# esq4/nind-denoise

Hardware: AMD Instinct MI355X
Metric: megapixels/sec denoised, UtNet cs=256 on 24 MP frames, 1/2/4/8 MI355X (higher is better)
Workload: dtype f32; 1 GPU; configs[1]: one 6000x4000 (24.0 MP) fp32 frame per step, f32 storage in the conv stack (fp32 accumulate), UtNet(funit=64,PReLU) random-init (seed 123), cs=264 (nearest valid to the named size; the reference rejects 256 / 512) ucs=200 ol=64 -> 1276 tiles/frame, tiles per conv-stack launch 256, crop->infer->stitch device resident (frame and canvas in HBM); every tile's input is the whole cs x cs cro; tiles_per_frame=1276, parallelism=single GPU

## Files before the change

include/nind_hip.h:

```cpp
#ifndef NIND_HIP_H
#define NIND_HIP_H

#include <stddef.h>
#include <stdint.h>

#ifdef __cplusplus
extern "C" {
#endif

typedef enum nd_status {
    ND_OK = 0,
    ND_EINVAL = -1,
    ND_ENOMEM = -2,
    ND_EHIP = -3
} nd_status;

typedef enum nd_act {
    ND_ACT_NONE = 0,
    ND_ACT_PRELU = 1,
    ND_ACT_ELU = 2,
    ND_ACT_HARDSWISH = 3
} nd_act;

typedef enum nd_layer_kind {
    ND_CONV3 = 0,
    ND_CONVT3 = 1,
    ND_CONVT2S2 = 2,
    ND_CONV1 = 3,
    ND_CONV2S2 = 4
} nd_layer_kind;

typedef enum nd_dtype {
    ND_F32 = 0,
    ND_BF16 = 1,
    ND_F16 = 2
} nd_dtype;

typedef enum nd_flags {
    ND_FLAG_NO_SPLITK = 1,
    ND_FLAG_DIRECT_CONV = 2,
    ND_FLAG_W1D_REGS = 4,
    ND_FLAG_UNFUSED_POOL = 16,
    ND_FLAG_TILE_ENCODER = 32,
    ND_FLAG_TILE_LEVEL2 = 64,
    ND_FLAG_FIND_NOISE = 128,
    ND_FLAG_TILE_SKIPS = 256,
    ND_FLAG_TILE_WINO = 512,
    ND_FLAG_FULL_TILES = 8
} nd_flags;

int nd_version(void);
const char *nd_last_error(void);

int nd_tile_grid(int width, int height, int cs, int ucs, int ol, int *cols, int *rows, int *pad);
int nd_tile_geom(int i, int width, int height, int cs, int ucs, int ol,
                 int *x0, int *y0, int usefuldim[4], int usefulstart[2]);

int nd_tile_gather(const float *img_chw, int width, int height, int cs, int ucs, int ol,
                   int tile_begin, int tile_count, float *tiles_nchw, void *stream);
int nd_stitch_add(float *canvas_chw, int width, int height, int cs, int ucs, int ol,
                  const float *tiles_nchw, int tile_begin, int tile_count, void *stream);

int nd_tile_source(int i, int width, int height, int cs, int ucs, int ol, int y, int x, int *Y, int *X);
int nd_stitch_weight(int i, int width, int height, int cs, int ucs, int ol, int y, int x, int *Y, int *X, float *w);
int nd_stitch_grad(const float *gcanvas_chw, int width, int height, int cs, int ucs, int ol, int tile_begin, int tile_count,
                   float *gtiles_nchw, void *stream);
int nd_tile_gather_grad(const float *gtiles_nchw, int width, int height, int cs, int ucs, int ol, int tile_begin, int tile_count,
                        float *gimg_chw, void *stream);

int nd_utnet_num_tensors(void);
const char *nd_utnet_tensor_name(int idx);
size_t nd_utnet_packed_bytes(int funit, int dtype);
int nd_utnet_pack_weights(int funit, int dtype, const float *const *tensors, int n_tensors,
                          void *packed_host, size_t packed_bytes);

int nd_utnet_pack_weights_device(int funit, int dtype, const float *const *dev_tensors, int n_tensors, void *packed_dev,
                                 size_t packed_bytes, void *stream);

size_t nd_utnet_workspace_bytes_hw(int funit, int h, int w, int batch, int dtype);
int nd_utnet_workspace_init_hw(void *workspace, size_t workspace_bytes, int funit, int h, int w, int batch, int dtype,
                               void *stream);
int nd_utnet_forward_hw(int funit, int act, int dtype, int flags, const void *packed_dev,
                        const float *x_nchw, float *y_nchw, int batch, int h, int w,
                        void *workspace, size_t workspace_bytes, void *stream);

int nd_utnet_denoise_tiles(int funit, int act, int dtype, int flags, const void *packed_dev,
                           const float *img_chw, float *canvas_chw, int width, int height,
                           int cs, int ucs, int ol, int tile_begin, int tile_count, int batch,
                           void *workspace, size_t workspace_bytes, void *stream);

typedef void (*nd_progress_fn)(void *ctx, int n, int tile_begin, int tile_count);
size_t nd_utnet_frame_workspace_bytes(int funit, int dtype, int flags, int width, int height, int cs, int ucs, int ol, int batch);
int nd_utnet_denoise_frame(int funit, int act, int dtype, int flags, const void *packed_dev,
                           const float *img_chw, float *canvas_chw, int width, int height,
                           int cs, int ucs, int ol, int tile_begin, int tile_count, int batch,
                           void *workspace, size_t workspace_bytes, void *frame_ws, size_t frame_ws_bytes, void *stream,
                           nd_progress_fn progress, void *progress_ctx);
int nd_utnet_denoise_frame_checked(int funit, int act, int dtype, int flags, const void *packed_dev,
                                   const float *img_chw, float *canvas_chw, int width, int height,
                                   int cs, int ucs, int ol, int tile_begin, int tile_count, int batch,
                                   void *workspace, size_t workspace_bytes, void *frame_ws, size_t frame_ws_bytes, void *stream,
                                   nd_progress_fn progress, void *progress_ctx, unsigned char *tile_ok);
int nd_utnet_frame_plan(int funit, int dtype, int flags, int width, int height, int cs, int ucs, int ol, int *out);
int nd_utnet_frame_levels(int funit, int dtype, int flags, int width, int height, int cs, int ucs, int ol, int *levels);
int nd_utnet_frame_folds(int funit, int dtype, int flags, int width, int height, int cs, int ucs, int ol, int *mask);

typedef struct nd_step_profile {
    float ms;
    float ms_xform_in;
    float ms_gemm;
    float ms_xform_out;
    int form;
    int kind;
    double flops;
    double mfma_flops;
    double bytes;
    double xform_bytes_in;
    double xform_bytes_out;
} nd_step_profile;
int nd_utnet_profile_stack(int funit, int act, int dtype, int flags, const void *packed_dev, int batch, int cs, int crop,
                           void *workspace, size_t workspace_bytes, void *stream, nd_step_profile *steps, int max_steps);
const char *nd_utnet_step_name(int i);
int nd_utnet_useful_region(int funit, int cs, int crop, int step, int *rect);

int nd_unet_num_tensors(void);
const char *nd_unet_tensor_name(int idx);
size_t nd_unet_packed_bytes(int dtype);
int nd_unet_pack_weights(int dtype, const float *const *tensors, int n_tensors, void *packed_host, size_t packed_bytes);
size_t nd_unet_workspace_bytes(int h, int w, int batch, int dtype);
int nd_unet_workspace_init(void *workspace, size_t workspace_bytes, int h, int w, int batch, int dtype, void *stream);
int nd_unet_forward(int dtype, const void *packed_dev, const float *x_nchw, float *y_nchw, int batch, int h, int w,
                    void *workspace, size_t workspace_bytes, void *stream);

int nd_unet_pack_weights_device(int dtype, const float *const *dev_tensors, int n_tensors, void *packed_dev, size_t packed_bytes,
                                void *stream);

int nd_unet_num_steps(void);
const char *nd_unet_step_name(int i);
int nd_unet_useful_region(int cs, int crop, int step, int *rect);

int nd_unet_denoise_frame(int dtype, int flags, const void *packed_dev, const float *img_chw, float *canvas_chw, int width,
                          int height, int cs, int ucs, int ol, int tile_begin, int tile_count, int batch, void *workspace,
                          size_t workspace_bytes, void *stream, nd_progress_fn progress, void *progress_ctx);

size_t nd_unet_param_count(void);
int nd_unet_param_range(int tensor_idx, size_t *offset, size_t *count);
size_t nd_unet_grad_blob_bytes(void);
size_t nd_unet_grad_workspace_bytes(int h, int w, int batch);
int nd_unet_grad_workspace_init(void *workspace, size_t workspace_bytes, int h, int w, int batch, void *stream);
int nd_unet_grad_forward(int flags, const float *params, void *blobs, const float *x_nchw, float *y_nchw, int batch, int h, int w,
                         void *workspace, size_t workspace_bytes, void *stream);
int nd_unet_grad_backward(int flags, const float *params, float *grads, void *blobs, const float *gy_nchw, float *dx_nchw, int batch,
                          int h, int w, void *workspace, size_t workspace_bytes, void *stream);

size_t nd_unet_train_blob_bytes(void);
size_t nd_unet_train_workspace_bytes(int h, int w, int batch);
int nd_unet_train_workspace_init(void *workspace, size_t workspace_bytes, int h, int w, int batch, void *stream);
int nd_unet_train_forward(int flags, float *params, void *blobs, const float *x_nchw, float *y_nchw, int batch, int h, int w,
                          float momentum, void *workspace, size_t workspace_bytes, void *stream);
int nd_unet_train_backward(int flags, const float *params, float *grads, void *blobs, const float *gy_nchw, float *dx_nchw, int batch,
                           int h, int w, void *workspace, size_t workspace_bytes, void *stream);

double nd_utnet_flops(int funit, int cs);

size_t nd_layer_packed_bytes(int kind, int cin, int cout, int dtype);
int nd_layer_pack(int kind, int cin, int cout, int dtype, const float *weight, const float *bias,
                  void *packed_host, size_t packed_bytes);
size_t nd_layer_workspace_bytes(int kind, int batch, int cin, int cout, int h, int w, int dtype);
int nd_layer_forward(int kind, int act, float slope, int dtype, const void *packed_dev,
                     const float *x_nchw, int batch, int cin, int h, int w, int cout, float *y_nchw,
                     void *workspace, size_t workspace_bytes, int variant, int flags, void *stream);
int nd_maxpool2_forward(const float *x_nchw, int batch, int c, int h, int w, float *y_nchw,
                        void *workspace, size_t workspace_bytes, void *stream);

size_t nd_layer_wgrad_workspace_bytes(int kind, int batch, int cin, int cout, int h, int w);
int nd_layer_wgrad(int kind, const float *x_nchw, const float *dy_nchw, int batch, int cin, int h, int w, int cout,
                   float *dw, float *db, void *workspace, size_t workspace_bytes, void *stream);

size_t nd_utnet_param_count(int funit);
int nd_utnet_param_range(int funit, int tensor_idx, size_t *offset, size_t *count);
size_t nd_utnet_train_blob_bytes(int funit);
size_t nd_utnet_train_workspace_bytes_hw(int funit, int h, int w, int batch);
int nd_utnet_train_workspace_init_hw(void *workspace, size_t workspace_bytes, int funit, int h, int w, int batch, void *stream);
int nd_utnet_train_step_act_hw(int funit, int act, int flags, const float *params, float *grads, void *blobs, const float *x_nchw,
                               const float *target_nchw, float *y_out_nchw, float w_l1, float w_mse, float w_ssim, float w_msssim,
                               float *loss_out, int batch, int h, int w, int loss_cs, void *workspace, size_t workspace_bytes,
                               void *stream, void *const *bucket_events, int n_events);
int nd_utnet_train_forward_hw(int funit, int act, int flags, const float *params, void *blobs, const float *x_nchw,
                              float *y_out_nchw, int batch, int h, int w, void *workspace, size_t workspace_bytes, void *stream);
int nd_utnet_train_backward_hw(int funit, int act, int flags, const float *params, float *grads, void *blobs, const float *gy_nchw,
                               float *dx_nchw, int batch, int h, int w, void *workspace, size_t workspace_bytes, void *stream,
                               void *const *bucket_events, int n_events);
int nd_utnet_grad_buckets(int funit, size_t *offsets, size_t *counts, int max);
int nd_adam_step(float *params, const float *grads, float *m, float *v, float *vmax, size_t n, float lr, float beta1,
                 float beta2, float eps, int step, int amsgrad, void *stream);
size_t nd_grad_guard_workspace_bytes(size_t n);
int nd_grad_guard(const float *grads, size_t n, float max_norm, int skip_nonfinite, double *state, void *workspace,
                  size_t workspace_bytes, void *stream);
int nd_adam_step_guarded(float *params, const float *grads, float *m, float *v, float *vmax, size_t n, float lr, float beta1,
                         float beta2, float eps, int step, int amsgrad, const double *state, void *stream);

size_t nd_ssim_workspace_bytes(int n, int c, int h, int w);
int nd_ssim(const float *x, const float *y, int n, int c, int h, int w, float *out, void *workspace, size_t workspace_bytes,
            void *stream);
int nd_ms_ssim(const float *x, const float *y, int n, int c, int h, int w, float *out, void *workspace,
               size_t workspace_bytes, void *stream);
int nd_mse(const float *x, const float *y, size_t count, float *out, void *workspace, size_t workspace_bytes, void *stream);

size_t nd_ssim_loss_workspace_bytes(int n, int c, int h, int w);
int nd_ssim_loss_grad(const float *x, const float *y, int n, int c, int h, int w, int multiscale, float weight,
                      float *loss_acc, float *gx, int accumulate, void *workspace, size_t workspace_bytes, void *stream);

size_t nd_criteria_workspace_bytes(int n, int h, int w, int loss_cs);
int nd_criteria(const float *y_nchw, const float *target_nchw, int n, int h, int w, int loss_cs, float w_l1, float w_mse,
                float w_ssim, float w_msssim, int also, float *out, void *workspace, size_t workspace_bytes, void *stream);
size_t nd_criteria_grad_workspace_bytes(int n, int h, int w, int loss_cs);
int nd_criteria_grad(const float *y_nchw, const float *target_nchw, int n, int h, int w, int loss_cs, float w_l1, float w_mse,
                     float w_ssim, float w_msssim, float *loss_out, float *gy_nchw, void *workspace, size_t workspace_bytes,
                     void *stream);

size_t nd_ssim_padded_workspace_bytes(int n, int c, int h, int w, int window);
int nd_ssim_padded(const float *x, const float *y, int n, int c, int h, int w, int window, float *out, void *workspace,
                   size_t workspace_bytes, void *stream);
int nd_ssim_padded_grad(const float *x, const float *y, int n, int c, int h, int w, int window, const float *gout, float *gx,
                        void *workspace, size_t workspace_bytes, void *stream);

typedef enum nd_sample_type { ND_SAMPLE_U8 = 0, ND_SAMPLE_U16 = 1, ND_SAMPLE_F32 = 2 } nd_sample_type;
int nd_crop_source(int cs, int nrot, int flips, int y, int x, int *a, int *b);
int nd_crop_batch(const void *pool, size_t pool_bytes, const int64_t *images, int n_images, const int32_t *draws, int batch, int cs,
                  float exp_mult_min, float exp_mult_max, const float *mult, float *xmax, float *mult_out, float *clean_nchw,
                  float *noisy_nchw, void *stream);
int nd_pool_fetch(const void *pool, size_t pool_bytes, const int64_t *images, int n_images, const int32_t *index, int n, int h, int w,
                  float *out_nchw, void *stream);
int nd_crop_batch_windows(const void *pool, size_t pool_bytes, const int64_t *windows, int n_windows, const int32_t *draws, int batch,
                          int cs, float exp_mult_min, float exp_mult_max, const float *mult, float *xmax, float *mult_out,
                          float *clean_nchw, float *noisy_nchw, void *stream);
int nd_pool_fetch_windows(const void *pool, size_t pool_bytes, const int64_t *windows, int n_windows, const int32_t *index, int n,
                          int h, int w, float *out_nchw, void *stream);

int nd_wino_mosaic(int p, int B, int *bx, int *by, long *tiles, long *tiles_per_image);

size_t nd_winograd_packed_bytes(int tile, int cin, int cout);
int nd_winograd_pack(int tile, int kind, int cin, int cout, const float *w, const float *bias, void *packed,
                     size_t packed_bytes);
size_t nd_layer_winograd_workspace_bytes(int tile, int kind, int batch, int cin, int cout, int h, int w);
int nd_layer_forward_winograd(int tile, int kind, int act, float slope, const void *packed, const float *x, int batch,
                              int cin, int h, int w, int cout, float *y, void *workspace, size_t workspace_bytes, int flags,
                              void *stream);

int nd_conv_bench(int kind, int dtype, int batch, int cin, int cout, int h, int w, int variant, int iters,
                  void *workspace, size_t workspace_bytes, void *stream, float *mean_ms);

int nd_winograd_bench(int tile, int kind, int batch, int cin, int cout, int h, int w, int iters, void *workspace,
                      size_t workspace_bytes, void *stream, float *mean_ms);
int nd_winograd_bench_flags(int tile, int kind, int batch, int cin, int cout, int h, int w, int iters, int flags, void *workspace,
                            size_t workspace_bytes, void *stream, float *mean_ms);

int nd_num_conv_variants(void);
const char *nd_conv_variant_name(int variant);

#ifdef __cplusplus
}
#endif
#endif
```

nind_denoise_amd/_lib.py:

```python
import ctypes
import os
from ctypes import POINTER, c_char_p, c_double, c_float, c_int, c_long, c_size_t, c_void_p

_HERE = os.path.dirname(os.path.abspath(__file__))
LIB_PATH = os.path.join(_HERE, "libnind_hip.so")

ND_F32, ND_BF16, ND_F16 = 0, 1, 2
DTYPE = {"f32": 0, "fp32": 0, "float32": 0, "bf16": 1, "bfloat16": 1, "f16": 2, "fp16": 2, "float16": 2}
ACT = {"none": 0, "PReLU": 1, "ELU": 2, "Hardswish": 3}
KIND = {"conv3": 0, "convT3": 1, "convT2s2": 2, "conv1": 3, "conv2s2": 4}
FLAG_NO_SPLITK, FLAG_DIRECT_CONV, FLAG_W1D_REGS, FLAG_FULL_TILES, FLAG_UNFUSED_POOL, FLAG_TILE_ENCODER, FLAG_TILE_LEVEL2 = 1, 2, 4, 8, 16, 32, 64
FLAG_FIND_NOISE = 128
FLAG_TILE_SKIPS = 256
FLAG_TILE_WINO = 512
PROGRESS_FN = ctypes.CFUNCTYPE(None, c_void_p, c_int, c_int, c_int)


class StepProfile(ctypes.Structure):
    _fields_ = [("ms", c_float), ("ms_xform_in", c_float), ("ms_gemm", c_float), ("ms_xform_out", c_float),
                ("form", c_int), ("kind", c_int), ("flops", c_double), ("mfma_flops", c_double), ("bytes", c_double),
                ("xform_bytes_in", c_double), ("xform_bytes_out", c_double)]


SAMPLE_U8, SAMPLE_U16, SAMPLE_F32 = 0, 1, 2

FORM_NAMES = {-1: "pool", 0: "direct", 1: "w1d_f43", 2: "w1d_f23", 3: "wino3p_f6x6"}


class NindHipError(RuntimeError):
    pass


class NindHipMissing(ImportError):
    pass


_lib = None

_SIGNATURES = {
    "nd_version": (c_int, []),
    "nd_last_error": (c_char_p, []),
    "nd_tile_grid": (c_int, [c_int] * 5 + [POINTER(c_int)] * 3),
    "nd_tile_geom": (c_int, [c_int] * 6 + [POINTER(c_int)] * 4),
    "nd_tile_gather": (c_int, [c_void_p] + [c_int] * 7 + [c_void_p, c_void_p]),
    "nd_stitch_add": (c_int, [c_void_p] + [c_int] * 5 + [c_void_p, c_int, c_int, c_void_p]),
    "nd_tile_source": (c_int, [c_int] * 8 + [POINTER(c_int)] * 2),
    "nd_stitch_weight": (c_int, [c_int] * 8 + [POINTER(c_int)] * 2 + [POINTER(c_float)]),
    "nd_stitch_grad": (c_int, [c_void_p] + [c_int] * 7 + [c_void_p, c_void_p]),
    "nd_tile_gather_grad": (c_int, [c_void_p] + [c_int] * 7 + [c_void_p, c_void_p]),
    "nd_utnet_num_tensors": (c_int, []),
    "nd_utnet_tensor_name": (c_char_p, [c_int]),
    "nd_utnet_packed_bytes": (c_size_t, [c_int, c_int]),
    "nd_utnet_pack_weights": (c_int, [c_int, c_int, POINTER(c_void_p), c_int, c_void_p, c_size_t]),
    "nd_utnet_pack_weights_device": (c_int, [c_int, c_int, POINTER(c_void_p), c_int, c_void_p, c_size_t, c_void_p]),
    "nd_utnet_workspace_bytes_hw": (c_size_t, [c_int] * 5),
    "nd_utnet_workspace_init_hw": (c_int, [c_void_p, c_size_t] + [c_int] * 5 + [c_void_p]),
    "nd_utnet_forward_hw": (c_int, [c_int] * 4 + [c_void_p] * 3 + [c_int, c_int, c_int, c_void_p, c_size_t, c_void_p]),
    "nd_utnet_denoise_tiles": (c_int, [c_int] * 4 + [c_void_p] * 3 + [c_int] * 8 + [c_void_p, c_size_t, c_void_p]),
    "nd_unet_num_tensors": (c_int, []),
    "nd_unet_tensor_name": (c_char_p, [c_int]),
    "nd_unet_packed_bytes": (c_size_t, [c_int]),
    "nd_unet_pack_weights": (c_int, [c_int, POINTER(c_void_p), c_int, c_void_p, c_size_t]),
    "nd_unet_workspace_bytes": (c_size_t, [c_int] * 4),
    "nd_unet_workspace_init": (c_int, [c_void_p, c_size_t] + [c_int] * 4 + [c_void_p]),
    "nd_unet_forward": (c_int, [c_int, c_void_p, c_void_p, c_void_p, c_int, c_int, c_int, c_void_p, c_size_t, c_void_p]),
    "nd_unet_pack_weights_device": (c_int, [c_int, POINTER(c_void_p), c_int, c_void_p, c_size_t, c_void_p]),
    "nd_unet_num_steps": (c_int, []),
    "nd_unet_step_name": (c_char_p, [c_int]),
    "nd_unet_useful_region": (c_int, [c_int, c_int, c_int, POINTER(c_int)]),
    "nd_unet_denoise_frame": (c_int, [c_int, c_int] + [c_void_p] * 3 + [c_int] * 8 + [c_void_p, c_size_t, c_void_p, PROGRESS_FN, c_void_p]),
    "nd_unet_param_count": (c_size_t, []),
    "nd_unet_param_range": (c_int, [c_int, POINTER(c_size_t), POINTER(c_size_t)]),
    "nd_unet_grad_blob_bytes": (c_size_t, []),
    "nd_unet_grad_workspace_bytes": (c_size_t, [c_int] * 3),
    "nd_unet_grad_workspace_init": (c_int, [c_void_p, c_size_t, c_int, c_int, c_int, c_void_p]),
    "nd_unet_grad_forward": (c_int, [c_int, c_void_p, c_void_p, c_void_p, c_void_p, c_int, c_int, c_int, c_void_p, c_size_t, c_void_p]),
    "nd_unet_train_blob_bytes": (c_size_t, []),
    "nd_unet_train_workspace_bytes": (c_size_t, [c_int] * 3),
    "nd_unet_train_workspace_init": (c_int, [c_void_p, c_size_t, c_int, c_int, c_int, c_void_p]),
    "nd_unet_train_forward": (c_int, [c_int, c_void_p, c_void_p, c_void_p, c_void_p, c_int, c_int, c_int, c_float, c_void_p, c_size_t,
                                      c_void_p]),
    "nd_unet_train_backward": (c_int, [c_int, c_void_p, c_void_p, c_void_p, c_void_p, c_void_p, c_int, c_int, c_int, c_void_p, c_size_t,
                                       c_void_p]),
    "nd_unet_grad_backward": (c_int, [c_int, c_void_p, c_void_p, c_void_p, c_void_p, c_void_p, c_int, c_int, c_int, c_void_p, c_size_t,
                                      c_void_p]),
    "nd_utnet_flops": (c_double, [c_int, c_int]),
    "nd_utnet_profile_stack": (c_int, [c_int] * 4 + [c_void_p, c_int, c_int, c_int, c_void_p, c_size_t, c_void_p, c_void_p, c_int]),
    "nd_utnet_step_name": (c_char_p, [c_int]),
    "nd_utnet_useful_region": (c_int, [c_int, c_int, c_int, c_int, POINTER(c_int)]),
    "nd_utnet_frame_workspace_bytes": (c_size_t, [c_int] * 9),
    "nd_utnet_frame_plan": (c_int, [c_int] * 8 + [POINTER(c_int)]),
    "nd_utnet_frame_levels": (c_int, [c_int] * 8 + [POINTER(c_int)]),
    "nd_utnet_frame_folds": (c_int, [c_int] * 8 + [POINTER(c_int)]),
    "nd_utnet_denoise_frame": (c_int, [c_int] * 4 + [c_void_p] * 3 + [c_int] * 8 + [c_void_p, c_size_t, c_void_p, c_size_t, c_void_p,
                                                                                    PROGRESS_FN, c_void_p]),
    "nd_utnet_denoise_frame_checked": (c_int, [c_int] * 4 + [c_void_p] * 3 + [c_int] * 8 + [c_void_p, c_size_t, c_void_p, c_size_t,
                                                                                            c_void_p, PROGRESS_FN, c_void_p, c_void_p]),
    "nd_layer_packed_bytes": (c_size_t, [c_int] * 4),
    "nd_layer_pack": (c_int, [c_int] * 4 + [c_void_p, c_void_p, c_void_p, c_size_t]),
    "nd_layer_workspace_bytes": (c_size_t, [c_int] * 7),
    "nd_layer_forward": (c_int, [c_int, c_int, c_float, c_int, c_void_p, c_void_p] + [c_int] * 5
                         + [c_void_p, c_void_p, c_size_t, c_int, c_int, c_void_p]),
    "nd_winograd_packed_bytes": (c_size_t, [c_int] * 3),
    "nd_winograd_pack": (c_int, [c_int] * 4 + [c_void_p, c_void_p, c_void_p, c_size_t]),
    "nd_layer_winograd_workspace_bytes": (c_size_t, [c_int] * 7),
    "nd_layer_forward_winograd": (c_int, [c_int, c_int, c_int, c_float, c_void_p, c_void_p] + [c_int] * 5
                                  + [c_void_p, c_void_p, c_size_t, c_int, c_void_p]),
    "nd_maxpool2_forward": (c_int, [c_void_p] + [c_int] * 4 + [c_void_p, c_void_p, c_size_t, c_void_p]),
    "nd_layer_wgrad_workspace_bytes": (c_size_t, [c_int] * 6),
    "nd_layer_wgrad": (c_int, [c_int, c_void_p, c_void_p] + [c_int] * 5 + [c_void_p, c_void_p, c_void_p, c_size_t, c_void_p]),
    "nd_utnet_param_count": (c_size_t, [c_int]),
    "nd_utnet_param_range": (c_int, [c_int, c_int, POINTER(c_size_t), POINTER(c_size_t)]),
    "nd_utnet_train_blob_bytes": (c_size_t, [c_int]),
    "nd_utnet_grad_buckets": (c_int, [c_int, POINTER(c_size_t), POINTER(c_size_t), c_int]),
    "nd_utnet_train_workspace_bytes_hw": (c_size_t, [c_int] * 4),
    "nd_utnet_train_workspace_init_hw": (c_int, [c_void_p, c_size_t, c_int, c_int, c_int, c_int, c_void_p]),
    "nd_utnet_train_forward_hw": (c_int, [c_int, c_int, c_int, c_void_p, c_void_p, c_void_p, c_void_p, c_int, c_int, c_int, c_void_p,
                                          c_size_t, c_void_p]),
    "nd_utnet_train_backward_hw": (c_int, [c_int, c_int, c_int, c_void_p, c_void_p, c_void_p, c_void_p, c_void_p, c_int, c_int, c_int,
                                           c_void_p, c_size_t, c_void_p, POINTER(c_void_p), c_int]),
    "nd_utnet_train_step_act_hw": (c_int, [c_int, c_int, c_int, c_void_p, c_void_p, c_void_p, c_void_p, c_void_p, c_void_p, c_float,
                                           c_float, c_float, c_float, c_void_p, c_int, c_int, c_int, c_int, c_void_p, c_size_t, c_void_p,
                                           POINTER(c_void_p), c_int]),
    "nd_adam_step": (c_int, [c_void_p] * 5 + [c_size_t, c_float, c_float, c_float, c_float, c_int, c_int, c_void_p]),
    "nd_grad_guard_workspace_bytes": (c_size_t, [c_size_t]),
    "nd_grad_guard": (c_int, [c_void_p, c_size_t, c_float, c_int, c_void_p, c_void_p, c_size_t, c_void_p]),
    "nd_adam_step_guarded": (c_int, [c_void_p] * 5 + [c_size_t, c_float, c_float, c_float, c_float, c_int, c_int, c_void_p, c_void_p]),
    "nd_ssim_workspace_bytes": (c_size_t, [c_int] * 4),
    "nd_ssim": (c_int, [c_void_p, c_void_p] + [c_int] * 4 + [c_void_p, c_void_p, c_size_t, c_void_p]),
    "nd_ms_ssim": (c_int, [c_void_p, c_void_p] + [c_int] * 4 + [c_void_p, c_void_p, c_size_t, c_void_p]),
    "nd_ssim_loss_workspace_bytes": (c_size_t, [c_int] * 4),
    "nd_ssim_loss_grad": (c_int, [c_void_p, c_void_p] + [c_int] * 5 + [c_float, c_void_p, c_void_p, c_int, c_void_p, c_size_t,
                                  c_void_p]),
    "nd_ssim_padded_workspace_bytes": (c_size_t, [c_int] * 5),
    "nd_ssim_padded": (c_int, [c_void_p, c_void_p] + [c_int] * 5 + [c_void_p, c_void_p, c_size_t, c_void_p]),
    "nd_ssim_padded_grad": (c_int, [c_void_p, c_void_p] + [c_int] * 5 + [c_void_p, c_void_p, c_void_p, c_size_t, c_void_p]),
    "nd_mse": (c_int, [c_void_p, c_void_p, c_size_t, c_void_p, c_void_p, c_size_t, c_void_p]),
    "nd_criteria_workspace_bytes": (c_size_t, [c_int] * 4),
    "nd_criteria": (c_int, [c_void_p, c_void_p] + [c_int] * 4 + [c_float] * 4 + [c_int, c_void_p, c_void_p, c_size_t, c_void_p]),
    "nd_criteria_grad_workspace_bytes": (c_size_t, [c_int] * 4),
    "nd_criteria_grad": (c_int, [c_void_p, c_void_p] + [c_int] * 4 + [c_float] * 4 + [c_void_p, c_void_p, c_void_p, c_size_t, c_void_p]),
    "nd_conv_bench": (c_int, [c_int] * 9 + [c_void_p, c_size_t, c_void_p, POINTER(c_float)]),
    "nd_winograd_bench": (c_int, [c_int] * 8 + [c_void_p, c_size_t, c_void_p, POINTER(c_float)]),
    "nd_winograd_bench_flags": (c_int, [c_int] * 9 + [c_void_p, c_size_t, c_void_p, POINTER(c_float)]),
    "nd_wino_mosaic": (c_int, [c_int, c_int, POINTER(c_int), POINTER(c_int), POINTER(c_long), POINTER(c_long)]),
    "nd_crop_source": (c_int, [c_int] * 5 + [POINTER(c_int)] * 2),
    "nd_crop_batch": (c_int, [c_void_p, c_size_t, c_void_p, c_int, c_void_p, c_int, c_int, c_float, c_float] + [c_void_p] * 6),
    "nd_pool_fetch": (c_int, [c_void_p, c_size_t, c_void_p, c_int, c_void_p, c_int, c_int, c_int, c_void_p, c_void_p]),
    "nd_crop_batch_windows": (c_int, [c_void_p, c_size_t, c_void_p, c_int, c_void_p, c_int, c_int, c_float, c_float] + [c_void_p] * 6),
    "nd_pool_fetch_windows": (c_int, [c_void_p, c_size_t, c_void_p, c_int, c_void_p, c_int, c_int, c_int, c_void_p, c_void_p]),
    "nd_num_conv_variants": (c_int, []),
    "nd_conv_variant_name": (c_char_p, [c_int]),
}

EXPORTS = tuple(_SIGNATURES)


def load():
    global _lib
    if _lib is not None:
        return _lib
    if not os.path.isfile(LIB_PATH):
        raise NindHipMissing(
            f"{LIB_PATH} not found: build it with `make -C nind_denoise_amd/csrc` (or __graft_entry__.build()). "
            "nind_denoise_amd has no CPU fallback for the denoise hot path.")
    import torch
    lib = ctypes.CDLL(LIB_PATH)
    for name, (res, args) in _SIGNATURES.items():
        fn = getattr(lib, name)
        fn.restype = res
        fn.argtypes = args
    _lib = lib
    return lib


def check(rc, what=""):
    if rc != 0:
        msg = load().nd_last_error().decode(errors="replace")
        exc = ValueError if rc == -1 else (MemoryError if rc == -2 else NindHipError)
        raise exc(f"{what}: {msg}" if what else msg)


def stream_ptr(device=None):
    import torch
    return c_void_p(torch.cuda.current_stream(device).cuda_stream)


def make_workspace(size_fn, init_fn, args, device, what, drop=None):
    import torch
    nbytes = size_fn(*args)
# ... 52 lines not shown
```

nind_denoise_amd/csrc/aux_kernels.hip:

```cpp
#include "nd_common.h"

typedef float f32x4 __attribute__((ext_vector_type(4)));
typedef __bf16 bf16x8 __attribute__((ext_vector_type(8)));
typedef _Float16 f16x8 __attribute__((ext_vector_type(8)));

template <int DT> struct Elem { typedef f32x4 vec; static constexpr int N = 4; typedef float scalar; };
template <> struct Elem<ND_BF16> { typedef bf16x8 vec; static constexpr int N = 8; typedef __bf16 scalar; };
template <> struct Elem<ND_F16> { typedef f16x8 vec; static constexpr int N = 8; typedef _Float16 scalar; };
#define ND_DISPATCH_DT(dt, CALL)                     \
    switch (dt) {                                    \
        case ND_F32: { constexpr int DT = ND_F32; CALL; break; }   \
        case ND_BF16: { constexpr int DT = ND_BF16; CALL; break; } \
        case ND_F16: { constexpr int DT = ND_F16; CALL; break; }   \
        default: ND_FAIL(ND_EINVAL, "unsupported storage type %d", dt); \
    }

static int make_geo(int W, int H, int cs, int ucs, int ol, TileGeo *g) {
    if (W <= 0 || H <= 0 || cs <= 0 || ucs <= 0 || ol < 0) ND_FAIL(ND_EINVAL, "tile grid: non-positive size");
    if (ucs - ol <= 0) ND_FAIL(ND_EINVAL, "tile grid: ucs (%d) must exceed the overlap (%d)", ucs, ol);
    if (cs < ucs) ND_FAIL(ND_EINVAL, "tile grid: cs (%d) < ucs (%d)", cs, ucs);
    g->W = W; g->H = H; g->cs = cs; g->ucs = ucs; g->ol = ol;
    g->stride = ucs - ol;
    g->pad = (cs - ucs) / 2;
    g->cols = ceil_div_py(W - ucs, g->stride) + 1;
// ... 649 lines not shown
    return ND_OK;
}

template <int DT>
__global__ void k_maxpool2(const typename Elem<DT>::vec *__restrict__ src, long snp, int sHb, int sWb, int spad, int splane0,
                           typename Elem<DT>::vec *__restrict__ dst, long dnp, int dHb, int dWb, int dpad, int Ho, int Wo, int B) {
    typedef typename Elem<DT>::vec V;
    const int xx = blockIdx.x * blockDim.x + threadIdx.x;
    const int yy = blockIdx.y;
    const int b = blockIdx.z % B, q = blockIdx.z / B;
    if (xx >= Wo) return;
    const V *s = src + (size_t)(splane0 + q) * snp + ((size_t)b * sHb + 2 * yy + spad) * sWb + 2 * xx + spad;
    const V a = s[0], c = s[1], d = s[sWb], e = s[sWb + 1];
    V o;
#pragma unroll
    for (int k = 0; k < Elem<DT>::N; ++k)
        o[k] = (typename Elem<DT>::scalar)fmaxf(fmaxf((float)a[k], (float)c[k]), fmaxf((float)d[k], (float)e[k]));
    dst[(size_t)q * dnp + ((size_t)b * dHb + yy + dpad) * dWb + xx + dpad] = o;
}

int nd_launch_maxpool2(const QpBuf &src, int src_plane0, int planes, const QpBuf &dst, hipStream_t s) {
    const int Hi = src.Hb - 2 * src.pad, Wi = src.Wb - 2 * src.pad;
    const int Ho = Hi / 2, Wo = Wi / 2;
    if (dst.Hb - 2 * dst.pad != Ho || dst.Wb - 2 * dst.pad != Wo || dst.B != src.B || dst.planes < planes || dst.dt != src.dt)
        ND_FAIL(ND_EINVAL, "maxpool2: destination does not fit %dx%d", Ho, Wo);
    dim3 grid((Wo + 127) / 128, Ho, src.B * planes);
    ND_DISPATCH_DT(src.dt, hipLaunchKernelGGL(k_maxpool2<DT>, grid, dim3(128), 0, s, (const typename Elem<DT>::vec *)src.base,
                                              src.np(), src.Hb, src.Wb, src.pad, src_plane0, (typename Elem<DT>::vec *)dst.base,
                                              dst.np(), dst.Hb, dst.Wb, dst.pad, Ho, Wo, src.B));
    ND_HIP(hipGetLastError());
    return ND_OK;
}

template <int DT>
__device__ __forceinline__ void dot3(const typename Elem<DT>::vec *__restrict__ s, long np, int planes,
                                     const float *__restrict__ w, int cin, float &o0, float &o1, float &o2) {
    constexpr int N = Elem<DT>::N;
    for (int q = 0; q < planes; ++q) {
        const typename Elem<DT>::vec v = s[(size_t)q * np];
#pragma unroll
        for (int e = 0; e < N; ++e) {
            const int c = N * q + e;
            if (c < cin) {
                const float f = (float)v[e];
                o0 = fmaf(f, w[c], o0);
                o1 = fmaf(f, w[cin + c], o1);
                o2 = fmaf(f, w[2 * cin + c], o2);
            }
        }
    }
}

template <int DT>
__global__ void k_final1x1(const typename Elem<DT>::vec *__restrict__ src, long np, int Hb, int Wb, int planes, int cin,
                           const float *__restrict__ w, const float *__restrict__ bias, int crop, float *__restrict__ y,
                           int H, int W, int sigmoid) {
    const int xx = blockIdx.x * blockDim.x + threadIdx.x;
    const int yy = blockIdx.y, b = blockIdx.z;
    if (xx >= W) return;
    float o0 = bias[0], o1 = bias[1], o2 = bias[2];
    dot3<DT>(src + ((size_t)b * Hb + yy + crop) * Wb + xx + crop, np, planes, w, cin, o0, o1, o2);
    if (sigmoid) {
        o0 = 1.f / (1.f + expf(-o0));
        o1 = 1.f / (1.f + expf(-o1));
        o2 = 1.f / (1.f + expf(-o2));
    }
    float *d = y + ((size_t)b * 3 * H + yy) * W + xx;
    d[0] = o0;
    d[(size_t)H * W] = o1;
    d[2 * (size_t)H * W] = o2;
}

int nd_launch_final1x1(const QpBuf &src, int cin, const float *w, const float *bias, int crop, float *y, int H, int W,
                       hipStream_t s, int sigmoid) {
    if (src.pad != 0 || src.Hb != H + 2 * crop || src.Wb != W + 2 * crop) ND_FAIL(ND_EINVAL, "final1x1: bad source geometry");
    dim3 grid((W + 255) / 256, H, src.B);
    const int n = nd_cpp(src.dt);
    ND_DISPATCH_DT(src.dt, hipLaunchKernelGGL(k_final1x1<DT>, grid, dim3(256), 0, s, (const typename Elem<DT>::vec *)src.base,
                                              src.np(), src.Hb, src.Wb, (cin + n - 1) / n, cin, w, bias, crop, y, H, W, sigmoid));
    ND_HIP(hipGetLastError());
    return ND_OK;
}

template <int DT, bool GUARD>
__device__ __forceinline__ void final1x1_stitch_pixel(const typename Elem<DT>::vec *__restrict__ src, long np, int Hb, int Wb, int planes,
                                                      int cin, const float *__restrict__ w, const float *__restrict__ bias, int crop,
                                                      float *__restrict__ canvas, const TileGeo &g, int tile_begin, int tile_count,
                                                      int y_first, int sigmoid, const float *__restrict__ noise_img,
                                                      const unsigned char *__restrict__ tile_ok) {
    const int X = blockIdx.x * blockDim.x + threadIdx.x;
    const int Y = y_first + blockIdx.y;
    if (X >= g.W || Y >= g.H) return;
    const size_t plane = (size_t)g.W * g.H;
    float *c = canvas + (size_t)Y * g.W + X;
    float v0 = c[0], v1 = c[plane], v2 = c[2 * plane];
    float n0 = 0.f, n1 = 0.f, n2 = 0.f;
    if (noise_img) {
        const float *n = noise_img + (size_t)Y * g.W + X;
        n0 = n[0]; n1 = n[plane]; n2 = n[2 * plane];
    }
    bool any = false;
    for_each_cover(g, X, Y, tile_begin, tile_count, [&](int t, int iy, int ix, float f) {
        if (GUARD && !tile_ok[tile_begin + t]) return;
        float o0 = bias[0], o1 = bias[1], o2 = bias[2];
        dot3<DT>(src + ((size_t)t * Hb + iy + crop) * Wb + ix + crop, np, planes, w, cin, o0, o1, o2);
        if (sigmoid) {
            o0 = 1.f / (1.f + expf(-o0));
            o1 = 1.f / (1.f + expf(-o1));
            o2 = 1.f / (1.f + expf(-o2));
        }
        if (noise_img) {
            o0 = n0 - o0;
            o1 = n1 - o1;
            o2 = n2 - o2;
        }
        v0 += o0 * f;
        v1 += o1 * f;
        v2 += o2 * f;
        any = true;
    });
    if (any) {
        c[0] = v0;
        c[plane] = v1;
        c[2 * plane] = v2;
    }
}

template <int DT>
__global__ void k_final1x1_stitch(const typename Elem<DT>::vec *__restrict__ src, long np, int Hb, int Wb, int planes, int cin,
                                  const float *__restrict__ w, const float *__restrict__ bias, int crop,
                                  float *__restrict__ canvas, TileGeo g, int tile_begin, int tile_count, int y_first, int sigmoid,
                                  const float *__restrict__ noise_img) {
    final1x1_stitch_pixel<DT, false>(src, np, Hb, Wb, planes, cin, w, bias, crop, canvas, g, tile_begin, tile_count, y_first, sigmoid,
                                     noise_img, nullptr);
}

template <int DT>
__global__ void k_final1x1_stitch_ok(const typename Elem<DT>::vec *__restrict__ src, long np, int Hb, int Wb, int planes, int cin,
                                     const float *__restrict__ w, const float *__restrict__ bias, int crop,
                                     float *__restrict__ canvas, TileGeo g, int tile_begin, int tile_count, int y_first,
                                     const unsigned char *__restrict__ tile_ok) {
    final1x1_stitch_pixel<DT, true>(src, np, Hb, Wb, planes, cin, w, bias, crop, canvas, g, tile_begin, tile_count, y_first, 0, nullptr,
                                    tile_ok);
}

template <int DT>
__global__ __launch_bounds__(256) void k_tile_verdict(const typename Elem<DT>::vec *__restrict__ src, long np, int Hb, int Wb,
                                                      int planes, int cin, const float *__restrict__ w,
                                                      const float *__restrict__ bias, int crop, TileGeo g, int tile_begin,
                                                      int tile_count, unsigned char *__restrict__ tile_ok) {
    const int t = blockIdx.y;
    if (t >= tile_count) return;
    const int i = tile_begin + t;
    const int yi = i / g.cols, xi = i - yi * g.cols;
    const int ax = xi * g.stride, ay = yi * g.stride;
    const int x1pad = max(0, ax - g.pad + g.cs - g.W), y1pad = max(0, ay - g.pad + g.cs - g.H);
    const int uw = min(g.cs - max(g.pad, x1pad) - g.pad, g.W - ax), uh = min(g.cs - max(g.pad, y1pad) - g.pad, g.H - ay);
    if (uw <= 0 || uh <= 0) return;
    const int p = blockIdx.x * blockDim.x + threadIdx.x;
    if (p >= uw * uh) return;
    const int dy = p / uw, dx = p - dy * uw;
    float o0 = bias[0], o1 = bias[1], o2 = bias[2];
    dot3<DT>(src + ((size_t)t * Hb + g.pad + dy + crop) * Wb + g.pad + dx + crop, np, planes, w, cin, o0, o1, o2);
    const unsigned e = 0x7f800000u;
    if ((__float_as_uint(o0) & e) == e || (__float_as_uint(o1) & e) == e || (__float_as_uint(o2) & e) == e) tile_ok[i] = 0;
}

static int stitch_launch_geo(const QpBuf &src, int crop, int W, int H, int cs, int ucs, int ol, int tile_begin, int tile_count, TileGeo *g,
                             int *yf, int *yr) {
    ND_TRY(make_geo(W, H, cs, ucs, ol, g));
    if (src.pad != 0 || src.Hb != cs + 2 * crop || src.Wb != cs + 2 * crop || tile_count > src.B)
        ND_FAIL(ND_EINVAL, "final1x1_stitch: bad source geometry");
    stitch_band(*g, tile_begin, tile_count, yf, yr);
    return ND_OK;
}

int nd_launch_final1x1_stitch(const QpBuf &src, int cin, const float *w, const float *bias, int crop, float *canvas,
                              int W, int H, int cs, int ucs, int ol, int tile_begin, int tile_count, hipStream_t s, int sigmoid,
                              const float *noise_img) {
    TileGeo g;
    int yf, yr;
    ND_TRY(stitch_launch_geo(src, crop, W, H, cs, ucs, ol, tile_begin, tile_count, &g, &yf, &yr));
    if (yr <= 0) return ND_OK;
    dim3 grid((W + 255) / 256, yr);
    const int n = nd_cpp(src.dt);
    ND_DISPATCH_DT(src.dt, hipLaunchKernelGGL(k_final1x1_stitch<DT>, grid, dim3(256), 0, s, (const typename Elem<DT>::vec *)src.base,
                                              src.np(), src.Hb, src.Wb, (cin + n - 1) / n, cin, w, bias, crop, canvas, g,
                                              tile_begin, tile_count, yf, sigmoid, noise_img));
    ND_HIP(hipGetLastError());
    return ND_OK;
}

int nd_launch_tile_verdict(const QpBuf &src, int cin, const float *w, const float *bias, int crop, int W, int H, int cs, int ucs, int ol,
                           int tile_begin, int tile_count, unsigned char *tile_ok, hipStream_t s) {
    TileGeo g;
    int yf, yr;
    ND_TRY(stitch_launch_geo(src, crop, W, H, cs, ucs, ol, tile_begin, tile_count, &g, &yf, &yr));
    if (!tile_ok || tile_begin < 0 || tile_count <= 0 || tile_count > 65535 || tile_begin + tile_count > g.cols * g.rows)
        ND_FAIL(ND_EINVAL, "tile_verdict: tiles [%d,+%d) outside the grid of %d (at most 65535 per launch), or no flags", tile_begin,
                tile_count, g.cols * g.rows);
    const int uwmax = g.cs - 2 * g.pad;
    if (uwmax <= 0) return ND_OK;
    dim3 grid((uwmax * uwmax + 255) / 256, tile_count);
    const int n = nd_cpp(src.dt);
    ND_DISPATCH_DT(src.dt, hipLaunchKernelGGL(k_tile_verdict<DT>, grid, dim3(256), 0, s, (const typename Elem<DT>::vec *)src.base,
                                              src.np(), src.Hb, src.Wb, (cin + n - 1) / n, cin, w, bias, crop, g, tile_begin, tile_count,
                                              tile_ok));
    ND_HIP(hipGetLastError());
    return ND_OK;
}

int nd_launch_final1x1_stitch_ok(const QpBuf &src, int cin, const float *w, const float *bias, int crop, float *canvas, int W, int H,
                                 int cs, int ucs, int ol, int tile_begin, int tile_count, const unsigned char *tile_ok, hipStream_t s) {
    TileGeo g;
    int yf, yr;
    ND_TRY(stitch_launch_geo(src, crop, W, H, cs, ucs, ol, tile_begin, tile_count, &g, &yf, &yr));
    if (!tile_ok) ND_FAIL(ND_EINVAL, "final1x1_stitch_ok: no flags");
    if (yr <= 0) return ND_OK;
    dim3 grid((W + 255) / 256, yr);
    const int n = nd_cpp(src.dt);
    ND_DISPATCH_DT(src.dt, hipLaunchKernelGGL(k_final1x1_stitch_ok<DT>, grid, dim3(256), 0, s, (const typename Elem<DT>::vec *)src.base,
                                              src.np(), src.Hb, src.Wb, (cin + n - 1) / n, cin, w, bias, crop, canvas, g,
                                              tile_begin, tile_count, yf, tile_ok));
    ND_HIP(hipGetLastError());
    return ND_OK;
}

__global__ __launch_bounds__(256) void k_sum(const float *__restrict__ partial, int n, float scale, float *__restrict__ out) {
    __shared__ float red[256];
    float acc = 0.f;
    for (int i = threadIdx.x; i < n; i += 256) acc += partial[i];
    acc = nd_block_sum(acc, red);
    if (threadIdx.x == 0) out[0] = acc * scale;
}
int nd_launch_sum(const float *partial, int n, float scale, float *out, hipStream_t s) {
    hipLaunchKernelGGL(k_sum, dim3(1), dim3(256), 0, s, partial, n, scale, out);
    ND_HIP(hipGetLastError());
    return ND_OK;
}
```

nind_denoise_amd/csrc/conv_qp.inc:

```
#pragma once
#include <stdlib.h>

#include <initializer_list>
#include <type_traits>

#include "nd_common.h"

typedef float f32x4 __attribute__((ext_vector_type(4)));
typedef float f32x8 __attribute__((ext_vector_type(8)));
typedef float f32x16 __attribute__((ext_vector_type(16)));
typedef __bf16 bf16x8 __attribute__((ext_vector_type(8)));
typedef __bf16 bf16x4 __attribute__((ext_vector_type(4)));
typedef _Float16 f16x8 __attribute__((ext_vector_type(8)));
typedef _Float16 f16x4 __attribute__((ext_vector_type(4)));

template <int DT> struct FragOf { typedef f32x4 type; };
template <> struct FragOf<ND_BF16> { typedef bf16x8 type; };
template <> struct FragOf<ND_F16> { typedef f16x8 type; };

struct FastDiv {
    unsigned m;
    int sh;
};
static inline FastDiv nd_fastdiv(int d) {
    FastDiv f;
    int s = 0;
    while ((1L << s) < (long)d) ++s;
    f.m = (unsigned)((((unsigned long long)1 << (31 + s)) + (unsigned long long)d - 1) / (unsigned long long)d);
    f.sh = 31 + s;
    return f;
}
__device__ __forceinline__ unsigned fdiv(unsigned n, const FastDiv &f) { return (unsigned)(((unsigned long long)n * f.m) >> f.sh); }

struct ConvParams {
    const f32x4 *in;
    const float *wpk;
    const float *bias;
    f32x4 *out;
    long in_plane;
    long out_plane;
    int nimg;
    int P, Wb;
    int Hv, Wv, PV;
    int tpi;
    int G;
    int stride;
    int ioff;
    f32x4 *pre;
    long pre_plane;
    int KB;
    int M;
    int cout;
    int Po, Wo, opad;
    int out_plane0;
    int act;
    float slope;
    const float *slope_dev;
    int n_tiles_n;
    int n_tiles_m;
    int split_first, S, cps, nitems;
    f32x4 *part;
    int wpx;
    int tiles_per_problem;
    long in_bs, out_bs;
    long w_bs;
    int dbg;
    int linear;
    FastDiv fd_PV, fd_Wv, fd_ntm, fd_tpp, fd_upq, fd_tpi;
    f32x4 *pool;
    long pool_plane;
    int pool_P, pool_W, pool_pad;
    int band2;
    FastDiv fd_2Wv;
    const f32x4 *in2;
    long in2_plane;
    const int *origin2;
    int kb2, Wb2;
    int KBw;
    const f32x4 *add;
    long add_plane;
    const int *origin_add;
    int W_add;
};

static inline void nd_conv_fastdivs(ConvParams &p) {
    p.fd_PV = nd_fastdiv(p.PV > 0 ? p.PV : 1);
    p.fd_Wv = nd_fastdiv(p.Wv > 0 ? p.Wv : 1);
    p.fd_2Wv = nd_fastdiv(p.Wv > 0 ? 2 * p.Wv : 1);
    p.fd_ntm = nd_fastdiv(p.n_tiles_m > 0 ? p.n_tiles_m : 1);
    p.fd_tpp = nd_fastdiv(p.tiles_per_problem > 0 ? p.tiles_per_problem : 1);
    p.fd_upq = nd_fastdiv(p.cout / 4 > 0 ? p.cout / 4 : 1);
    p.fd_tpi = nd_fastdiv(p.tpi > 0 ? p.tpi : 1);
}

ConvParams nd_conv_params(const ConvDesc &d, int KB, int M);
int nd_conv_pool(const char *who, const ConvDesc &d, int Hv, int Wv, ConvParams &p);
void nd_conv_tiles(ConvParams &p, bool cross, int nblk, int mblk);
long nd_conv_schedule(ConvParams &p, long ntiles, int nchunks, long slots, long cap);
double nd_conv_schedule_time(long ntiles, int nchunks, long slots, long cap);
int nd_launch_split_finish(const ConvParams &p, int n_split_tiles, int mblk, int nblk, int up, int dt, hipStream_t s);
#ifdef ND_QP_STAMPS
int nd_stamped_launch(void (*fn)(ConvParams), int threads, size_t lds, ConvParams p, long ntiles, int nchunks, long slots, hipStream_t s,
                      bool print, const char *header, const char *wave_prefix, const char *const *names, int nphases, std::initializer_list<int> waves);
#endif

__device__ __forceinline__ void glds16(const void *g, void *l) {
    __builtin_amdgcn_global_load_lds((const __attribute__((address_space(1))) void *)g,
                                     (__attribute__((address_space(3))) void *)l, 16, 0, 0);
}

__device__ __forceinline__ f32x8 sload8(const float *p) {
    const unsigned long long a = (unsigned long long)p;
    const unsigned lo = __builtin_amdgcn_readfirstlane((unsigned)a);
    const unsigned hi = __builtin_amdgcn_readfirstlane((unsigned)(a >> 32));
    const float *sp = (const float *)(((unsigned long long)hi << 32) | lo);
    f32x8 v;
    asm volatile("s_load_dwordx8 %0, %1, 0x0\n\ts_waitcnt lgkmcnt(0)" : "=s"(v) : "s"(sp) : "memory");
    return v;
}
__device__ __forceinline__ f32x4 sload_bias4(const float *p, int h) {
    const unsigned long long a = (unsigned long long)p;
    const unsigned lo = __builtin_amdgcn_readfirstlane((unsigned)a);
    const unsigned hi = __builtin_amdgcn_readfirstlane((unsigned)(a >> 32));
    const float *sp = (const float *)(((unsigned long long)hi << 32) | lo);
    f32x4 b0, b1;
    asm volatile("s_load_dwordx4 %0, %2, 0x0\n\ts_load_dwordx4 %1, %2, 0x10\n\ts_waitcnt lgkmcnt(0)" : "=&s"(b0), "=&s"(b1) : "s"(sp) : "memory");
    f32x4 r;
#pragma unroll
    for (int e = 0; e < 4; ++e) r[e] = h ? b1[e] : b0[e];
    return r;
}

#ifdef ND_QP_STAMPS
__device__ __forceinline__ unsigned long long qp_stamp() {
    unsigned long long t;
    __builtin_amdgcn_sched_barrier(0);
    asm volatile("s_memtime %0\n\ts_waitcnt lgkmcnt(0)" : "=s"(t)::"memory");
    __builtin_amdgcn_sched_barrier(0);
    return t;
}
#define QP_STAMP(k) do { if (stamps) { t1 = qp_stamp(); tph[k] += t1 - t0; t0 = t1; } } while (0)
#else
#define QP_STAMP(k) do { } while (0)
#endif

__device__ __forceinline__ float quad_max(float v) {
    int a = __builtin_bit_cast(int, v);
    v = fmaxf(v, __builtin_bit_cast(float, __builtin_amdgcn_update_dpp(a, a, 0xB1, 0xF, 0xF, false)));
    a = __builtin_bit_cast(int, v);
    return fmaxf(v, __builtin_bit_cast(float, __builtin_amdgcn_update_dpp(a, a, 0x4E, 0xF, 0xF, false)));
}

__device__ __forceinline__ float apply_act(float v, int act, float slope) {
    switch (act) {
        case ND_ACT_PRELU: return v > 0.f ? v : v * slope;
        case ND_ACT_ELU: return v > 0.f ? v : expm1f(v);
        case ND_ACT_HARDSWISH: return v * fminf(fmaxf(v + 3.f, 0.f), 6.f) / 6.f;
        default: return v;
    }
}

template <int DT, int MR, int NR, int WM, int WN, int TAPS, int KBC, bool UP, int NSTAGE>
__global__ __launch_bounds__(64 * WM * WN) void conv_qp(ConvParams p) {
    typedef typename FragOf<DT>::type Frag;
    extern __shared__ __attribute__((aligned(16))) char smem[];
// ... 531 lines not shown
```

nind_denoise_amd/csrc/conv_w2d.hip:

```cpp
#include "conv_qp.inc"

namespace {

typedef float f32x2 __attribute__((ext_vector_type(2)));

constexpr int kR = 8;
constexpr int kS = 16;
constexpr int kRI = kR + 2;
constexpr int kVPlane = kRI * kS * 16;
constexpr int kVPos = 2 * kVPlane;
constexpr int kVBytes = 6 * kVPos;
constexpr int kTaps = 18;
constexpr int kMTB = 2;
constexpr int kWBytes = kMTB * kTaps * 1024;
constexpr int kStage = kWBytes + kVBytes;
constexpr int kStages = 2;
constexpr int kScratch = 2048;
constexpr int kLds = kStages * kStage + 8 * kScratch;
constexpr int kDmaAt = 4;
constexpr int kXfAt = 12;
constexpr int kSlots = 4 * 32 * 4;

template <int OFF> __device__ __forceinline__ void glds16o(const void *g, void *l) {
    __builtin_amdgcn_global_load_lds((const __attribute__((address_space(1))) void *)g, (__attribute__((address_space(3))) void *)l, 16, OFF, 0);
}

__device__ __forceinline__ int vslot(int r, int s) { return r * kS + (s ^ ((r & 3) << 2)); }

__device__ __forceinline__ void w4_in(const f32x4 *d, f32x4 *v) {
    const f32x4 s34 = d[3] + d[4], d43 = d[4] - d[3], s12 = d[1] + d[2], d12 = d[1] - d[2], d42 = d[4] - d[2], d31 = d[3] - d[1];
    v[0] = 4.f * d[0] - 5.f * d[2] + d[4];
    v[1] = s34 - 4.f * s12;
    v[2] = d43 + 4.f * d12;
    v[3] = d42 + 2.f * d31;
    v[4] = d42 - 2.f * d31;
    v[5] = 4.f * d[1] - 5.f * d[3] + d[5];
}
__device__ __forceinline__ void w4_out(const float *m, float *y) {
    const float a = m[1] + m[2], b = m[1] - m[2], c = m[3] + m[4], e = m[3] - m[4];
    y[0] = m[0] + a + c;
    y[1] = b + 2.f * e;
    y[2] = a + 4.f * c;
    y[3] = b + 8.f * e + m[5];
}

__device__ __forceinline__ unsigned long long stamp() {
    unsigned long long t;
    __builtin_amdgcn_sched_barrier(0);
    asm volatile("s_memtime %0\n\ts_waitcnt lgkmcnt(0)" : "=s"(t)::"memory");
    __builtin_amdgcn_sched_barrier(0);
    return t;
}

#ifdef ND_QP_STAMPS
const char *const kStampNames[6] = {"issue loads + DMA", "MFMA loop", "wait vmcnt", "transform+publish (inside the loop)", "epilogue", "barrier"};
#endif
struct Strip { int img, y0, x0; bool ok; };

template <int DBG, bool SRC2 = false, bool ADD = false>
__global__ __launch_bounds__(512) void conv_w2d(ConvParams p) {
    extern __shared__ __attribute__((aligned(16))) char smem[];
    const int lane = threadIdx.x & 63;
    const int wave = __builtin_amdgcn_readfirstlane(threadIdx.x >> 6);
    const int wm = wave >> 2, wn = wave & 3;
    const int j = lane & 31, h = lane >> 5;
    const int nwg = gridDim.x;
    const int bid = blockIdx.x;
    const int vb = (nwg % 8 == 0) ? (bid % 8) * (nwg / 8) + bid / 8 : bid;

    const int nchunks = p.KB;
    const int nitems = p.nitems;
    const int my_items = vb < nitems ? (nitems - vb + nwg - 1) / nwg : 0;
    struct Item { int tile, c0, c1, slice; };
    auto decode = [&](int w) -> Item {
        Item it;
        if (w < p.split_first) {
            it.tile = w; it.c0 = 0; it.c1 = nchunks; it.slice = -1;
        } else {
            const int u = w - p.split_first;
            const int t = u / p.S, ks = u - t * p.S;
            it.tile = p.split_first + t;
            it.c0 = ks * p.cps;
            it.c1 = it.c0 + p.cps < nchunks ? it.c0 + p.cps : nchunks;
            it.slice = u;
        }
        return it;
    };
    int nsteps = 0;
    if (p.split_first >= nitems)
        nsteps = my_items * nchunks;
    else
        for (int i = 0; i < my_items; ++i) {
            const Item it = decode(vb + i * nwg);
            nsteps += it.c1 - it.c0;
        }
    if (nsteps == 0) return;

    const unsigned tot = (unsigned)p.nimg * (unsigned)p.PV;
    auto strip_of = [&](int nb, int s) -> Strip {
        Strip r;
        const unsigned u = (unsigned)nb * kS + s;
        r.ok = u < tot;
        const unsigned uc = r.ok ? u : tot - 1;
        r.img = (int)fdiv(uc, p.fd_PV);
        const int rem = (int)(uc - (unsigned)r.img * p.PV);
        const int band = (int)fdiv((unsigned)rem, p.fd_Wv);
        r.y0 = band * kR;
        r.x0 = 4 * (rem - band * p.Wv);
        return r;
    };

    int f_id = vb, f_c = 0, f_end = 0, f_stage = 0, issued = 0;
    int f_nb = 0;
    const float *f_w;
    const unsigned lane16 = (unsigned)lane * 16u;
    const int kXfHalf = 1;
    const bool xfA = (wave >> 2) == kXfHalf, xfB = wave == 4 * (1 - kXfHalf);
    const int dw = wave - 4 * (1 - kXfHalf);
    int vwOff[2];
    int x_h[2], x_i[2], x_s[2];
#pragma unroll
    for (int ps = 0; ps < 2; ++ps) {
        const int xt = ps == 0 ? (wave & 3) * 64 + lane : 256 + lane;
        x_h[ps] = xt / (kS * kRI);
        x_i[ps] = (xt / kS) % kRI;
        x_s[ps] = xt % kS;
        vwOff[ps] = kWBytes + x_h[ps] * kVPlane + vslot(x_i[ps], x_s[ps]) * 16;
    }
    unsigned x_off[2] = {0, 0};
    int x_keep[2] = {6, 6};
    auto set_fill_tile = [&](int w) {
        const Item it = decode(w);
        f_c = it.c0;
        f_end = it.c1;
        const int nb = (int)fdiv((unsigned)it.tile, p.fd_ntm), mb = it.tile - nb * p.n_tiles_m;
        f_w = p.wpk + (size_t)mb * kMTB * p.KBw * kTaps * 256;
        if constexpr (SRC2) f_nb = nb;
#pragma unroll
        for (int ps = 0; ps < 2; ++ps)
            if (ps == 0 ? xfA : xfB) {
                const Strip st = strip_of(nb, x_s[ps]);
                x_off[ps] = 16u * ((unsigned)x_h[ps] * (unsigned)p.in_plane + (unsigned)st.img * (unsigned)p.P + (unsigned)(st.y0 + x_i[ps]) * p.Wb + st.x0);
                const int left = p.wpx - st.x0;
                x_keep[ps] = left + 2 < 6 ? left + 2 : 6;
            }
    };
    auto set_fill_src2 = [&]() {
        const int nb = f_nb;
#pragma unroll
        for (int ps = 0; ps < 2; ++ps)
            if (ps == 0 ? xfA : xfB) {
                const Strip st = strip_of(nb, x_s[ps]);
                x_off[ps] = 16u * ((unsigned)x_h[ps] * (unsigned)p.in2_plane + (unsigned)p.origin2[st.img] + (unsigned)(st.y0 + x_i[ps]) * p.Wb2 + st.x0);
            }
    };
    set_fill_tile(f_id);
    if constexpr (SRC2) if (f_c >= p.kb2) set_fill_src2();
    f32x4 dn[2][6];
#pragma unroll
    for (int ps = 0; ps < 2; ++ps)
#pragma unroll
        for (int k = 0; k < 6; ++k) dn[ps][k] = f32x4{0.f, 0.f, 0.f, 0.f};
    auto fill_loads = [&]() {
        if (issued >= nsteps || (DBG & 8)) return;
        const bool s2 = SRC2 && f_c >= p.kb2;
        const char *kbase = s2 ? (const char *)(p.in2 + (size_t)(2 * (f_c - p.kb2)) * p.in2_plane)
                               : (const char *)(p.in + (size_t)(2 * f_c) * p.in_plane);
        if (xfA) {
#pragma unroll
            for (int k = 0; k < 6; ++k) dn[0][k] = *(const f32x4 *)(kbase + x_off[0] + 16 * k);
        }
        if (xfB) {
#pragma unroll
            for (int k = 0; k < 6; ++k) dn[1][k] = *(const f32x4 *)(kbase + x_off[1] + 16 * k);
        }
    };
    auto fill_xform = [&]() {
        if (issued >= nsteps || (DBG & 16)) return;
#pragma unroll
// ... 32 lines not shown
    auto fill_advance = [&]() {
        if (issued >= nsteps) return;
        ++issued;
        f_stage ^= 1;
        if (++f_c == f_end) {
            f_id += nwg;
            if (f_id < nitems) {
                set_fill_tile(f_id);
                if constexpr (SRC2) if (f_c >= p.kb2) set_fill_src2();
            }
        } else if constexpr (SRC2) {
            if (f_c == p.kb2) set_fill_src2();
        }
    };

    const int sl = 4 * wn + (j >> 3), rr = j & 7;
    const int aOff = (wm * kTaps) * 1024 + lane * 16;
    int bOffK[3];
#pragma unroll
    for (int ky = 0; ky < 3; ++ky) bOffK[ky] = kWBytes + h * kVPlane + vslot(rr + ky, sl) * 16;

    f32x16 acc[6];
#pragma unroll
    for (int x = 0; x < 6; ++x)
#pragma unroll
        for (int r = 0; r < 16; ++r) acc[x][r] = 0.f;

    const float slope = p.act == ND_ACT_NONE ? 1.f : (p.slope_dev ? *p.slope_dev : p.slope);
    const bool slope01 = p.act <= ND_ACT_PRELU && slope >= 0.f && slope <= 1.f;

    auto combine = [&](int g, f32x4 *y) {
#pragma unroll
        for (int e = 0; e < 4; ++e) {
            float m[6], o[4];
#pragma unroll
            for (int x = 0; x < 6; ++x) {
                m[x] = acc[x][4 * g + e];
                acc[x][4 * g + e] = 0.f;
            }
            w4_out(m, o);
#pragma unroll
            for (int i = 0; i < 4; ++i) y[i][e] = o[i];
        }
    };

    char *const scratch = smem + kStages * kStage + wave * kScratch;
    const int e_row = lane >> 4, e_px = lane & 15;
    f32x4 biasq[4];
    auto load_bias = [&](int id) {
        if constexpr (ADD) return;
        const int mb = id - (int)fdiv((unsigned)id, p.fd_ntm) * p.n_tiles_m;
#pragma unroll
        for (int g = 0; g < 4; ++g) biasq[g] = *(const f32x4 *)(p.bias + (mb * kMTB + wm) * 32 + 8 * g + 4 * h);
    };
    load_bias(decode(vb).tile);
    auto epilogue = [&](int id, auto fast) {
        const int nb = (int)fdiv((unsigned)id, p.fd_ntm), mb = id - nb * p.n_tiles_m;
        const Strip st = strip_of(nb, 4 * wn + (e_px >> 2));
        const int ex = st.x0 + (e_px & 3);
        const unsigned offA = (unsigned)((st.img * p.Po + (st.y0 + e_row + p.opad) * p.Wo + ex + p.opad) * 16);
        const unsigned offB = offA + (unsigned)(4 * p.Wo * 16);
        const bool okx = st.ok && ex < p.wpx;
        const bool okA = okx && st.y0 + e_row < p.Hv, okB = okx && st.y0 + e_row + 4 < p.Hv;
        const int q0 = (mb * kMTB + wm) * 8;
        const f32x2 slope2 = {slope, slope};
        const int pp_i = (e_px & ~3) + 2 * (e_px & 1);
        const int pxp = (st.x0 >> 1) + (e_px & 1), pyp = (st.y0 >> 1) + e_row;
        unsigned offQA = 0, offQB = 0;
        f32x4 qa[8], qb[8];
        auto add_loads = [&](int k) {
            const int qq = (q0 + k) * 4 < p.M ? q0 + k : 0;
            const char *pq = (const char *)(p.add + (size_t)qq * p.add_plane);
            qa[k] = *(const f32x4 *)(pq + offQA);
            qb[k] = *(const f32x4 *)(pq + offQB);
        };
        if constexpr (ADD) {
            const unsigned oq = 16u * ((unsigned)p.origin_add[st.img] + (unsigned)(st.y0 + e_row) * (unsigned)p.W_add + (unsigned)ex);
            offQA = okA ? oq : 0u;
            offQB = okB ? oq + 64u * (unsigned)p.W_add : 0u;
            add_loads(0);
            add_loads(1);
            __builtin_amdgcn_sched_barrier(0);
        }
        const bool okP = !SRC2 && !ADD && p.pool && !(lane & 2) && st.ok && 2 * pxp + 1 < p.wpx && 2 * pyp + 1 < p.Hv;
        const unsigned offP = (unsigned)((st.img * p.pool_P + (pyp + p.pool_pad) * p.pool_W + pxp + p.pool_pad) * 16);
#pragma unroll
        for (int g = 0; g < 4; ++g) {
            f32x4 yy[4], ypre[4];
#pragma unroll
            for (int pr = 0; pr < 2; ++pr) {
                f32x2 m[6];
#pragma unroll
                for (int x = 0; x < 6; ++x) {
                    m[x] = f32x2{acc[x][4 * g + 2 * pr], acc[x][4 * g + 2 * pr + 1]};
                    acc[x][4 * g + 2 * pr] = 0.f;
                    acc[x][4 * g + 2 * pr + 1] = 0.f;
                }
                f32x2 a = m[1] + m[2], b = m[1] - m[2];
                const f32x2 c = m[3] + m[4], e = m[3] - m[4];
                if constexpr (!ADD) {
                    const f32x2 bq = {biasq[g][2 * pr], biasq[g][2 * pr + 1]};
                    a += bq;
                    b += bq;
                }
                f32x2 y[4];
                y[0] = m[0] + a + c;
                y[1] = b + 2.f * e;
                y[2] = a + 4.f * c;
                y[3] = b + 8.f * e + m[5];
#pragma unroll
                for (int i = 0; i < 4; ++i) {
                    ypre[i][2 * pr] = y[i][0];
                    ypre[i][2 * pr + 1] = y[i][1];
                    if constexpr (ADD) {
                    } else if constexpr (decltype(fast)::value) {
                        const f32x2 t = y[i] * slope2;
                        y[i] = f32x2{fmaxf(y[i][0], t[0]), fmaxf(y[i][1], t[1])};
                    } else {
                        y[i] = f32x2{apply_act(y[i][0], p.act, slope), apply_act(y[i][1], p.act, slope)};
                    }
                    yy[i][2 * pr] = y[i][0];
                    yy[i][2 * pr + 1] = y[i][1];
                }
            }
            if (!SRC2 && !ADD && p.pre) {
                const Strip so = strip_of(nb, sl);
                const int yo = so.y0 + rr, m4 = (q0 + 2 * g + h) * 4, left = p.wpx - so.x0;
                if (so.ok && yo < p.Hv && m4 < p.M) {
                    f32x4 *dst = p.pre + (long)(m4 >> 2) * p.pre_plane + ((long)so.img * p.Hv + yo) * p.wpx + so.x0;
#pragma unroll
                    for (int i = 0; i < 4; ++i)
                        if (i < left) dst[i] = ypre[i];
                }
            }
            if (DBG & 256) {
                const Strip so = strip_of(nb, sl);
                const int yo = so.y0 + rr, m4 = (q0 + 2 * g + h) * 4, left = p.wpx - so.x0;
                if (so.ok && yo < p.Hv && m4 < p.M) {
                    f32x4 *dst = p.out + (long)(p.out_plane0 + (m4 >> 2)) * p.out_plane + (long)so.img * p.Po + (long)(yo + p.opad) * p.Wo + so.x0 + p.opad;
#pragma unroll
                    for (int i = 0; i < 4; ++i)
                        if (i < left) dst[i] = yy[i];
                }
                continue;
            }
#pragma unroll
            for (int hq = 0; hq < 2; ++hq) {
                if (h == hq) {
                    f32x4 *w = (f32x4 *)scratch + rr * 16 + (j >> 3) * 4;
#pragma unroll
                    for (int i = 0; i < 4; ++i) w[i] = yy[i];
                }
                __builtin_amdgcn_fence(__ATOMIC_RELEASE, "wavefront");
                __builtin_amdgcn_wave_barrier();
                __builtin_amdgcn_fence(__ATOMIC_ACQUIRE, "wavefront");
                f32x4 va = *((const f32x4 *)scratch + e_row * 16 + e_px);
                f32x4 vb2 = *((const f32x4 *)scratch + (e_row + 4) * 16 + e_px);
                if constexpr (ADD) {
                    const int k = 2 * g + hq;
                    va += qa[k];
                    vb2 += qb[k];
                    if (k + 2 < 8) {
                        add_loads(k + 2);
                        __builtin_amdgcn_sched_barrier(0);
                    }
#pragma unroll
                    for (int e = 0; e < 4; ++e) {
                        if constexpr (decltype(fast)::value) {
                            va[e] = fmaxf(va[e], va[e] * slope);
                            vb2[e] = fmaxf(vb2[e], vb2[e] * slope);
                        } else {
                            va[e] = apply_act(va[e], p.act, slope);
                            vb2[e] = apply_act(vb2[e], p.act, slope);
                        }
                    }
                }
                f32x4 vp = va;
                if (!SRC2 && !ADD && p.pool) {
                    const f32x4 *blk = (const f32x4 *)scratch + (2 * e_row) * 16 + pp_i;
                    const f32x4 p00 = blk[0], p01 = blk[1], p10 = blk[16], p11 = blk[17];
#pragma unroll
                    for (int e = 0; e < 4; ++e) vp[e] = fmaxf(fmaxf(p00[e], p01[e]), fmaxf(p10[e], p11[e]));
                }
                __builtin_amdgcn_fence(__ATOMIC_RELEASE, "wavefront");
                __builtin_amdgcn_wave_barrier();
                __builtin_amdgcn_fence(__ATOMIC_ACQUIRE, "wavefront");
                const int quad = q0 + 2 * g + hq;
                if (quad * 4 < p.M && !(DBG & 1)) {
                    char *pb = (char *)(p.out + (size_t)(p.out_plane0 + quad) * p.out_plane);
                    if (okA) *(f32x4 *)(pb + offA) = va;
                    if (okB) *(f32x4 *)(pb + offB) = vb2;
                    if (okP) *(f32x4 *)((char *)(p.pool + (size_t)quad * p.pool_plane) + offP) = vp;
                }
            }
        }
    };
    auto epilogue_partial = [&](int slice) {
        f32x4 *dst = p.part + (size_t)slice * (kMTB * 8) * kSlots;
#pragma unroll
        for (int g = 0; g < 4; ++g) {
            f32x4 yy[4];
            combine(g, yy);
            f32x4 *d2 = dst + (size_t)(wm * 8 + 2 * g + h) * kSlots + 4 * (wn * 32 + j);
#pragma unroll
            for (int i = 0; i < 4; ++i) d2[i] = yy[i];
        }
    };

    fill_loads();
    fill_xform();
    fill_dma();
    fill_advance();
    asm volatile("s_waitcnt vmcnt(0) lgkmcnt(0)" ::: "memory");
    __builtin_amdgcn_s_barrier();

    int c_id = vb, c_stage = 0;
    Item c_it = decode(vb);
    int c_c = c_it.c0;
    unsigned long long tph[6] = {0, 0, 0, 0, 0, 0}, t0 = 0, t1 = 0;
    for (int s = 0; s < nsteps; ++s) {
        if (DBG & 128) t0 = stamp();
        fill_loads();
        __builtin_amdgcn_sched_barrier(0);
        if (DBG & 128) { t1 = stamp(); tph[0] += t1 - t0; t0 = t1; }
        const char *wa = smem + c_stage * kStage + aOff;
        const char *vq = smem + c_stage * kStage;
        f32x4 a[2], b[2];
        a[0] = *(const f32x4 *)wa;
        b[0] = *(const f32x4 *)(vq + bOffK[0]);
#pragma unroll
        for (int st = 0; st < kTaps; ++st) {
            if (st + 1 < kTaps) {
                const int ky = (st + 1) / 6, x = (st + 1) % 6;
                a[(st + 1) & 1] = *(const f32x4 *)(wa + (st + 1) * 1024);
                b[(st + 1) & 1] = *(const f32x4 *)(vq + bOffK[ky] + x * kVPos);
            }
            __builtin_amdgcn_sched_barrier(0);
            const int x = st % 6;
            if (!(DBG & 32)) {
#pragma unroll
                for (int q = 0; q < 4; ++q) acc[x] = __builtin_amdgcn_mfma_f32_32x32x2f32(a[st & 1][q], b[st & 1][q], acc[x], 0, 0, 0);
            } else {
#pragma unroll
                for (int q = 0; q < 4; ++q) acc[x][q] += a[st & 1][q] * b[st & 1][q];
            }
            if (st + 1 == kDmaAt) {
                __builtin_amdgcn_sched_barrier(0);
                fill_dma();
                __builtin_amdgcn_sched_barrier(0);
            }
            if (st + 1 == kXfAt) {
                __builtin_amdgcn_sched_barrier(0);
                if (DBG & 128) { t1 = stamp(); tph[1] += t1 - t0; t0 = t1; }
                fill_xform();
                fill_advance();
                if (DBG & 128) { t1 = stamp(); tph[3] += t1 - t0; t0 = t1; }
                __builtin_amdgcn_sched_barrier(0);
            }
        }
        __builtin_amdgcn_sched_barrier(0);
        if (DBG & 128) { t1 = stamp(); tph[1] += t1 - t0; t0 = t1; }
        asm volatile("s_waitcnt vmcnt(0) lgkmcnt(0)" ::: "memory");
        if (DBG & 128) { t1 = stamp(); tph[2] += t1 - t0; t0 = t1; }
        c_stage ^= 1;
        if (++c_c == c_it.c1) {
            if (DBG & 2) {
            } else if (c_it.slice >= 0)
                epilogue_partial(c_it.slice);
            else if (slope01)
                epilogue(c_it.tile, std::true_type{});
            else
                epilogue(c_it.tile, std::false_type{});
            c_id += nwg;
            if (c_id < nitems) {
                c_it = decode(c_id);
                if (p.n_tiles_m > 1) load_bias(c_it.tile);
            }
            c_c = c_it.c0;
        }
        if (DBG & 128) { t1 = stamp(); tph[4] += t1 - t0; t0 = t1; }
        if (!(DBG & 64)) __builtin_amdgcn_s_barrier();
        if (DBG & 128) { t1 = stamp(); tph[5] += t1 - t0; }
    }
    if ((DBG & 128) && lane == 0 && p.part) {
        unsigned long long *o = (unsigned long long *)p.part + ((size_t)blockIdx.x * 8 + wave) * 8;
        for (int k = 0; k < 6; ++k) o[k] = tph[k];
        o[6] = (unsigned long long)nsteps;
    }
}

__global__ __launch_bounds__(256) void k_w2d_split_finish(ConvParams p) {
    const int t = blockIdx.x, quad = blockIdx.y;
    const int gid = p.split_first + t;
    const int nb = gid / p.n_tiles_m, mb = gid - nb * p.n_tiles_m;
    const int m4 = mb * (kMTB * 32) + quad * 4;
    if (m4 >= p.M) return;
    const float slope = p.act == ND_ACT_NONE ? 1.f : (p.slope_dev ? *p.slope_dev : p.slope);
    const f32x4 bv = p.add ? f32x4{0.f, 0.f, 0.f, 0.f} : *(const f32x4 *)(p.bias + m4);
    const unsigned tot = (unsigned)p.nimg * (unsigned)p.PV;
    for (int l = threadIdx.x; l < kSlots; l += 256) {
        const int i = l & 3, jj = l >> 2, wn = jj >> 5, j = jj & 31;
        const int s = 4 * wn + (j >> 3), rr = j & 7;
        const unsigned u = (unsigned)nb * kS + s;
        if (u >= tot) continue;
        const int img = (int)(u / (unsigned)p.PV);
        const int rem = (int)(u - (unsigned)img * p.PV);
        const int band = rem / p.Wv;
        const int y = band * kR + rr, x = 4 * (rem - band * p.Wv) + i;
        if (y >= p.Hv || x >= p.wpx) continue;
        f32x4 acc = {0.f, 0.f, 0.f, 0.f};
        for (int ks = 0; ks < p.S; ++ks) acc += p.part[((size_t)(t * p.S + ks) * (kMTB * 8) + quad) * kSlots + l];
        if (p.add)
            acc += p.add[(long)(m4 >> 2) * p.add_plane + (long)p.origin_add[img] + (long)y * p.W_add + x];
        else
            acc += bv;
        f32x4 v;
#pragma unroll
        for (int e = 0; e < 4; ++e) v[e] = p.act <= ND_ACT_PRELU ? (acc[e] > 0.f ? acc[e] : acc[e] * slope) : apply_act(acc[e], p.act, slope);
        p.out[(long)(p.out_plane0 + (m4 >> 2)) * p.out_plane + (long)img * p.Po + (long)(y + p.opad) * p.Wo + x + p.opad] = v;
    }
}

}

bool nd_w2d_ok(const QpBuf &in) { return in.dt == ND_F32 && in.Hb >= 3 && in.Wb >= 3; }
long nd_w2d_tiles(const QpBuf &in, int cout) {
    const long strips = (long)in.B * ((in.Hb - 2 + kR - 1) / kR) * ((in.Wb - 2 + 3) / 4);
    return ((strips + kS - 1) / kS) * ((cout + kMTB * 32 - 1) / (kMTB * 32));
}

int nd_launch_conv_w2d(const ConvDesc &d, hipStream_t stream) {
    if ((d.kind != ND_CONV3 && d.kind != ND_CONVT3) || d.in.dt != ND_F32 || d.out.dt != ND_F32) ND_FAIL(ND_EINVAL, "w2d: fp32 3x3 layers only");
    const int KB = nd_kblocks(d.cin);
    const int Hfull = d.in.Hb - 2, Wfull = d.in.Wb - 2;
    if (Hfull < 1 || Wfull < 1) ND_FAIL(ND_EINVAL, "w2d: input smaller than the kernel");
    ND_TRY(nd_check_roi("w2d", d, Hfull, Wfull, d.pool != nullptr, "a pooled layer"));
    const bool roi = d.roi_rows > 0;
    const int Hv = roi ? d.roi_rows : Hfull, Wpx = roi ? d.roi_cols : Wfull, Wg = (Wpx + 3) / 4, NB = (Hv + kR - 1) / kR;
    if (d.pre && (roi || d.pool)) ND_FAIL(ND_EINVAL, "w2d: a pre-activation copy goes with whole, unpooled layers only");
    if (d.cout % 4) ND_FAIL(ND_EINVAL, "w2d: cout must be a multiple of 4");
    ND_TRY(nd_check_in_planes("w2d", d, KB, true, true));
    const bool src2 = d.in2.base != nullptr, add = d.add.base != nullptr;
    if (add && (d.pool || d.pre || src2))
        ND_FAIL(ND_EINVAL, "w2d: a layer with an addend source is neither pooled nor keeps a pre-activation copy nor has a second input source");
    if (add) ND_TRY(nd_check_add("w2d", d, (long)(d.roi_r0 + Hv - 1 + d.add.pad) * d.add.Wb + d.roi_c0 + Wpx - 1 + d.add.pad + 1));
    if (src2 && (d.pool || d.pre)) ND_FAIL(ND_EINVAL, "w2d: a layer with a second input source is neither pooled nor keeps a pre-activation copy");
    if (src2) ND_TRY(nd_check_in2("w2d", d, KB, (long)(d.roi_r0 + (NB - 1) * kR + kRI - 1) * d.in2.Wb + d.roi_c0 + 4 * (Wg - 1) + 6));
    ND_TRY(nd_check_out("w2d", d, Hfull, Wfull, false));
    ND_TRY(nd_check_int32("w2d", d.in));
    if (2 * d.in.np() * 16 + 65536 >= (1L << 32)) ND_FAIL(ND_EINVAL, "w2d: input too large for 32-bit byte offsets");

    int dev = 0, ncus = 0;
    ND_TRY(nd_device(&dev, &ncus));
    void (*fn)(ConvParams) = add ? conv_w2d<0, false, true> : src2 ? conv_w2d<0, true> : conv_w2d<0>;
#ifdef ND_QP_STAMPS
    static const int dbg_all = getenv("ND_W2D_DBG") ? atoi(getenv("ND_W2D_DBG")) : 0;
    const int dbg_env = src2 ? 0 : add ? (dbg_all == 128 ? 128 : 0) : dbg_all;
    switch (dbg_env) {
        case 1: fn = conv_w2d<1>; break;
        case 2: fn = conv_w2d<2>; break;
        case 4: fn = conv_w2d<4>; break;
        case 8: fn = conv_w2d<8>; break;
        case 16: fn = conv_w2d<16>; break;
        case 24: fn = conv_w2d<24>; break;
        case 28: fn = conv_w2d<28>; break;
        case 30: fn = conv_w2d<30>; break;
        case 32: fn = conv_w2d<32>; break;
        case 62: fn = conv_w2d<62>; break;
        case 128: fn = add ? conv_w2d<128, false, true> : conv_w2d<128>; break;
        case 256: fn = conv_w2d<256>; break;
        default: break;
    }
#endif
    ND_TRY(nd_raise_lds(dev, (const void *)fn, kLds));

    ConvParams p = nd_conv_params(d, KB, d.cout);
    if (roi) {
        p.in += (long)d.roi_r0 * d.in.Wb + d.roi_c0;
        p.out += (long)d.roi_r0 * d.out.Wb + d.roi_c0;
    }
    if (src2) {
        p.in2 = (const f32x4 *)d.in2.base + (long)d.in2_plane0 * d.in2.np() + (roi ? (long)d.roi_r0 * d.in2.Wb + d.roi_c0 : 0);
        p.in2_plane = d.in2.np();
        p.origin2 = d.in2_origin;
        p.kb2 = d.in2_from / 2;
        p.Wb2 = d.in2.Wb;
    }
    if (d.w_kb) {
        p.KBw = d.w_kb;
        p.wpk += (size_t)d.w_kb0 * kTaps * 256;
    }
    if (add) {
        p.add = (const f32x4 *)d.add.base + (long)d.add_plane0 * d.add.np() + (long)((roi ? d.roi_r0 : 0) + d.add.pad) * d.add.Wb +
                (roi ? d.roi_c0 : 0) + d.add.pad;
        p.add_plane = d.add.np();
        p.origin_add = d.add_origin;
        p.W_add = d.add.Wb;
    }
    p.Hv = Hv;
    p.Wv = Wg;
    p.PV = NB * Wg;
    p.wpx = Wpx;
    if (d.pool) {
        ND_TRY(nd_conv_pool("w2d", d, Hv, Wpx, p));
        if (d.pool->used() * 16 >= (1L << 32)) ND_FAIL(ND_EINVAL, "w2d: pooled destination too large for 32-bit byte offsets");
    }
    nd_conv_tiles(p, true, kS, kMTB * 32);
    nd_conv_fastdivs(p);
    const long ntiles = p.tiles_per_problem;
    const long cap = d.part && !d.nosplit && !d.pool && !d.pre ? (long)(d.part_bytes / ((size_t)kMTB * 32 * kSlots * 4)) : 0;
    const long grid = nd_conv_schedule(p, ntiles, KB, ncus, cap);
    p.part = (f32x4 *)d.part;
#ifdef ND_QP_STAMPS
    if (dbg_env == 128) {
        static const int only_kb = getenv("ND_W2D_STAMP_KB") ? atoi(getenv("ND_W2D_STAMP_KB")) : 0;
        static int printed = 0, printed_kb[2] = {0, 0};
        char header[160];
        snprintf(header, sizeof(header), "[w2d stamps] kind %d cin %d cout %d KB %d tiles %ld%s", d.kind, d.cin, d.cout, KB, ntiles,
                 add ? " ADDEND" : "");
        if (only_kb)
            return nd_stamped_launch(fn, 512, kLds, p, ntiles, KB, ncus, stream, KB == only_kb && ntiles >= 4 * ncus && printed_kb[add]++ < 4,
                                     header, "[w2d stamps] wave", kStampNames, 6, {0, 1, 4});
        return nd_stamped_launch(fn, 512, kLds, p, ntiles, KB, ncus, stream, printed++ < 2, nullptr, "[w2d stamps] wave", kStampNames, 6, {0, 1, 4});
    }
#endif
    hipLaunchKernelGGL(fn, dim3((unsigned)grid), dim3(512), kLds, stream, p);
    if (p.split_first < ntiles) hipLaunchKernelGGL(k_w2d_split_finish, dim3((unsigned)(ntiles - p.split_first), kMTB * 8), dim3(256), 0, stream, p);
    ND_HIP(hipGetLastError());
    return ND_OK;
}

bool nd_f43_w2d(const QpBuf &in, int cout, bool pre, int flags) {
    return !(flags & ND_FLAG_W1D_REGS) && nd_w2d_ok(in) && (!pre || nd_w2d_tiles(in, cout) >= 512);
}
int nd_launch_conv_f43(const ConvDesc &d, int flags, hipStream_t stream) {
    return nd_f43_w2d(d.in, d.cout, d.pre != nullptr, flags) ? nd_launch_conv_w2d(d, stream) : nd_launch_conv_w1d(4, d, stream);
}
```

nind_denoise_amd/csrc/nd_common.h:

```cpp
#pragma once
#include <hip/hip_runtime.h>

#include <stdarg.h>
#include <stdint.h>
#include <stdio.h>

#include "nind_hip.h"

void nd_set_error(const char *fmt, ...);
#define ND_FAIL(code, ...)        \
    do {                          \
        nd_set_error(__VA_ARGS__); \
        return (code);            \
    } while (0)
#define ND_HIP(call)                                                                         \
    do {                                                                                     \
        hipError_t e_ = (call);                                                              \
        if (e_ != hipSuccess) ND_FAIL(ND_EHIP, "%s failed: %s", #call, hipGetErrorString(e_)); \
    } while (0)
#define ND_TRY(call)        \
    do {                    \
        int r_ = (call);    \
        if (r_ != 0) return r_; \
    } while (0)
// ... 13 lines not shown
    *Y = mirror_sym(yi * g.stride - g.pad + y, g.H);
}
__host__ __device__ static inline float nd_stitch_weight_map(const TileGeo &g, int i, int y, int x, int *Y, int *X) {
    const int yi = i / g.cols, xi = i - yi * g.cols;
    const int ax = xi * g.stride, ay = yi * g.stride;
    const int x1pad = ax - g.pad + g.cs - g.W > 0 ? ax - g.pad + g.cs - g.W : 0;
    const int y1pad = ay - g.pad + g.cs - g.H > 0 ? ay - g.pad + g.cs - g.H : 0;
    const int uw = g.cs - (g.pad > x1pad ? g.pad : x1pad) - g.pad;
    const int uh = g.cs - (g.pad > y1pad ? g.pad : y1pad) - g.pad;
    const int dx = x - g.pad, dy = y - g.pad;
    *X = ax + dx;
    *Y = ay + dy;
    if (dx < 0 || dx >= uw || dy < 0 || dy >= uh) return 0.f;
    float f = 1.f;
    if (ax != 0 && dx < g.ol) f *= 0.5f;
    if (ay != 0 && dy < g.ol) f *= 0.5f;
    if (ax + g.ucs < g.W && g.ol && dx >= uw - g.ol) f *= 0.5f;
    if (ay + g.ucs < g.H && g.ol && dy >= uh - g.ol) f *= 0.5f;
    return f;
}

template <typename T>
__device__ inline T nd_block_sum(T v, T *red) {
    red[threadIdx.x] = v;
    __syncthreads();
    for (int k = 128; k > 0; k >>= 1) {
        if ((int)threadIdx.x < k) red[threadIdx.x] += red[threadIdx.x + k];
        __syncthreads();
    }
    return red[0];
}
int nd_launch_sum(const float *partial, int n, float scale, float *out, hipStream_t s);

struct LossWindow {
    int Lh, Lw, oy, ox;
};
int nd_loss_window(const char *who, int n, int h, int w, int loss_cs, bool ssim, bool msssim, LossWindow *win);

static inline int nd_cpp(int dt) { return dt == ND_F32 ? 4 : 8; }
struct QpBuf {
    float *base;
    int planes;
    int B, Hb, Wb;
    int pad;
    long pstride;
    int dt = ND_F32;
    long np() const { return pstride; }
    long used() const { return (long)B * Hb * Wb; }
};

struct ConvDesc {
    int kind = ND_CONV3;
    int act = ND_ACT_NONE;
    float slope = 1.f;
    const float *slope_dev = nullptr;
    const float *wpk = nullptr;
    const float *bias = nullptr;
    int cin = 0, cout = 0;
    QpBuf in = {};
    QpBuf out = {};
    int out_plane0 = 0;
    int variant = -1;
    int in_plane0 = 0;
    float *pre = nullptr;
    long pre_plane = 0;
    float *part = nullptr;
    size_t part_bytes = 0;
    bool nosplit = false;
    bool tile_wino = false;
    int nbatch = 1;
    long in_bs = 0, out_bs = 0;
    size_t w_bs = 0;
    const QpBuf *pool = nullptr;
    int roi_r0 = 0, roi_c0 = 0, roi_rows = 0, roi_cols = 0;
    QpBuf in2 = {};
    int in2_plane0 = 0, in2_from = 0;
    const int *in2_origin = nullptr;
    long in2_origin_max = 0;
    int w_kb = 0, w_kb0 = 0;
    QpBuf add = {};
    int add_plane0 = 0;
    const int *add_origin = nullptr;
    long add_origin_max = 0;
};
int nd_check_in2(const char *who, const ConvDesc &d, int KB, long reach);
int nd_check_add(const char *who, const ConvDesc &d, long reach);
static const size_t kSplitScratchBytes = (size_t)512 * 64 * 1024 * 4;
int nd_launch_conv(const ConvDesc &d, hipStream_t stream);
bool nd_conv_pool_fits(const ConvDesc &d);
bool nd_conv_roi_fits(const ConvDesc &d);
int nd_conv_variant_count();
int nd_conv_variant_gemm(int cin, int cout);
size_t nd_wino_packed_floats(int T, int cin, int cout);
int nd_wino_pack(int T, int kind, int cin, int cout, const float *w, const float *bias, float *packed);
size_t nd_wino_scratch_bytes(int T, const QpBuf &in, int cin, int cout);
int nd_launch_conv_wino(int T, const ConvDesc &d, void *scratch, size_t scratch_bytes, hipStream_t s, hipEvent_t *ev2 = nullptr);
long nd_wino_launch_tiles(int T, const ConvDesc &d);
void nd_wino_xform_bytes(int T, const QpBuf &in, int cin, int cout, long tiles, double *bytes_in, double *bytes_out);
size_t nd_w1d_packed_floats(int T, int cin, int cout);
int nd_w1d_pack(int T, int kind, int cin, int cout, const float *w, const float *bias, float *packed);
bool nd_w1d_fits(int T, const QpBuf &in);
int nd_launch_conv_w1d(int T, const ConvDesc &d, hipStream_t stream);
bool nd_w2d_ok(const QpBuf &in);
long nd_w2d_tiles(const QpBuf &in, int cout);
int nd_launch_conv_w2d(const ConvDesc &d, hipStream_t stream);
bool nd_f43_w2d(const QpBuf &in, int cout, bool pre, int flags);
int nd_launch_conv_f43(const ConvDesc &d, int flags, hipStream_t stream);
static inline size_t nd_buf_slack(int Wb) { return (size_t)10 * Wb + 8 + 2048; }
int nd_device(int *dev, int *ncus = nullptr);
int nd_raise_lds(int dev, const void *fn, size_t bytes);
int nd_once_per_device(int dev, int (*init)());
int nd_check_in_planes(const char *who, const ConvDesc &d, int KB, bool takes_in2 = false, bool takes_add = false);
int nd_check_out(const char *who, const ConvDesc &d, int oh, int ow, bool at_least);
int nd_check_int32(const char *who, const QpBuf &in);
int nd_check_roi(const char *who, const ConvDesc &d, int Hv, int Wv, bool refused, const char *why);
static inline int nd_check_flags(int flags, bool frame_loop = false, bool unet_frame = false) {
    const int known = ND_FLAG_NO_SPLITK | ND_FLAG_DIRECT_CONV | ND_FLAG_W1D_REGS | ND_FLAG_FULL_TILES | ND_FLAG_UNFUSED_POOL |
                      ND_FLAG_TILE_ENCODER | ND_FLAG_TILE_WINO | (frame_loop ? ND_FLAG_TILE_LEVEL2 | ND_FLAG_TILE_SKIPS : 0) | (unet_frame ? ND_FLAG_FIND_NOISE : 0);
    if (flags & ~known) ND_FAIL(ND_EINVAL, "unknown flag bits 0x%x", flags);
    return ND_OK;
}
const char *nd_conv_variant_label(int v);

static inline int nd_mtiles(int kind, int cout) {
    return kind == ND_CONVT2S2 ? (4 * cout + 255) / 256 * 8 : (cout + 127) / 128 * 4;
}
struct NdUpRow { int a, b, co; };
__host__ __device__ static inline NdUpRow nd_up_row(int m, int cout, int dt) {
    NdUpRow r;
    const int cpp = dt == ND_F32 ? 4 : 8, q = cout / cpp;
    const int G = m / (2 * cpp), e = m % cpp;
    r.b = (m / cpp) & 1;
    r.a = G / q;
    r.co = cpp * (G % q) + e;
    return r;
}
static inline int nd_taps(int kind) { return (kind == ND_CONV3 || kind == ND_CONVT3) ? 9 : (kind == ND_CONV2S2 ? 4 : 1); }
static inline int nd_kblocks(int cin, int dt = ND_F32) { return (cin + 2 * nd_cpp(dt) - 1) / (2 * nd_cpp(dt)); }
static inline size_t nd_bias_offset(int kind, int cin, int cout, int dt = ND_F32, int w1d_T = 0) {
    return (size_t)nd_mtiles(kind, cout) * nd_kblocks(cin, dt) * (w1d_T ? 3 * (w1d_T + 2) : nd_taps(kind)) * 256;
}
static inline size_t nd_packed_floats(int kind, int cin, int cout, int dt = ND_F32) {
    return nd_bias_offset(kind, cin, cout, dt) + (size_t)nd_mtiles(kind, cout) * 32;
}
void nd_pack_layer(int kind, int cin, int cout, int dt, const float *w, const float *bias, float *packed);

int nd_pack_layer_device(int kind, int cin, int cout, int dt, const float *w, const float *bias, float *packed, hipStream_t s,
                         const float *scale = nullptr);
int nd_launch_bn_fold(int cout, const float *b, const float *g, const float *be, const float *rm, const float *rv, float *scale,
                      float *fbias, hipStream_t s);
int nd_pack_w1d_device(int T, int kind, int cin, int cout, const float *w, const float *bias, float *packed, hipStream_t s);
int nd_pack_wino_device(int T, int kind, int cin, int cout, const float *w, const float *bias, float *packed, hipStream_t s);

int nd_launch_nchw_to_qp(const float *x, int C, const QpBuf &dst, int plane0, hipStream_t s);
int nd_launch_qp_to_nchw(const QpBuf &src, int plane0, float *y, int C, hipStream_t s);
int nd_launch_reflect_pack(const float *x_nchw, int B, int H, int W, const QpBuf &dst, hipStream_t s);
int nd_launch_maxpool2(const QpBuf &src, int src_plane0, int planes, const QpBuf &dst, hipStream_t s);
int nd_launch_final1x1(const QpBuf &src, int cin, const float *w, const float *bias, int crop, float *y_nchw, int H,
                       int W, hipStream_t s, int sigmoid = 0);
int nd_launch_final1x1_stitch(const QpBuf &src, int cin, const float *w, const float *bias, int crop, float *canvas,
                              int width, int height, int cs, int ucs, int ol, int tile_begin, int tile_count,
                              hipStream_t s, int sigmoid = 0, const float *noise_img = nullptr);
int nd_launch_tile_verdict(const QpBuf &src, int cin, const float *w, const float *bias, int crop, int width, int height, int cs, int ucs,
                           int ol, int tile_begin, int tile_count, unsigned char *tile_ok, hipStream_t s);
int nd_launch_final1x1_stitch_ok(const QpBuf &src, int cin, const float *w, const float *bias, int crop, float *canvas, int width,
                                 int height, int cs, int ucs, int ol, int tile_begin, int tile_count, const unsigned char *tile_ok,
                                 hipStream_t s);
static inline int nd_launch_utnet_stitch(const QpBuf &src, int cin, const float *w, const float *bias, float *canvas, int width, int height,
                                         int cs, int ucs, int ol, int tile_begin, int tile_count, unsigned char *tile_ok, hipStream_t s) {
    if (!tile_ok) return nd_launch_final1x1_stitch(src, cin, w, bias, 2, canvas, width, height, cs, ucs, ol, tile_begin, tile_count, s);
    ND_TRY(nd_launch_tile_verdict(src, cin, w, bias, 2, width, height, cs, ucs, ol, tile_begin, tile_count, tile_ok, s));
    return nd_launch_final1x1_stitch_ok(src, cin, w, bias, 2, canvas, width, height, cs, ucs, ol, tile_begin, tile_count, tile_ok, s);
}
int nd_utnet_denoise_tiles_ok(int funit, int act, int dtype, int flags, const void *packed, const float *img, float *canvas, int width,
                              int height, int cs, int ucs, int ol, int tile_begin, int tile_count, int batch, void *ws, size_t ws_bytes,
                              void *stream, unsigned char *tile_ok);
int nd_launch_gather_pack(const float *img, int width, int height, int cs, int ucs, int ol, int tile_begin,
                          int tile_count, const QpBuf &dst, hipStream_t s, int border = 2, bool reflect = true);
int nd_launch_gather_band(const float *img, int width, int height, int cs, int ucs, int ol, int band_row0, const QpBuf &dst,
                          hipStream_t s);
enum nd_edge_set { ND_EDGE_ROWS = 0, ND_EDGE_COLS = 1, ND_EDGE_CORNERS = 2 };
int nd_launch_gather_edges(const float *img, int width, int height, int cs, int ucs, int ol, int set, int first, int count,
                           const QpBuf &dst, hipStream_t s);
int nd_launch_skip_origins(const QpBuf &src, int dst_pad, int tile_begin, int tile_count, int cols, int band_rows, int step, long slot_elems,
                           int *table, long *origin_max, hipStream_t s);
struct SpliceMap {
    int step_y = 0, step_x = 0, img_t = 0, img_y = 0, img_x = 0, img_add = 0, oy = 0, ox = 0;
};
int nd_launch_splice(const QpBuf &src, int src_p0, const QpBuf &dst, int dst_p0, int planes, int tile_begin, int tile_count, int cols,
                     int row0, const SpliceMap &m, int r0, int r1, int c0, int c1, hipStream_t s, int band_rows = 0,
                     long slot_elems = 0, int dst_img0 = 0);
struct SpliceJob {
    QpBuf src, dst;
    int src_p0, dst_p0, planes, tile_begin, tile_count, cols, row0;
    SpliceMap m;
    int r0, r1, c0, c1, band_rows;
    long slot_elems;
    int dst_img0;
};
constexpr int kSpliceJobs = 16;
static inline SpliceJob nd_splice_job(const QpBuf &src, int src_p0, const QpBuf &dst, int dst_p0, int planes, int tile_begin, int tile_count,
                                      int cols, int row0, const SpliceMap &m, int r0, int r1, int c0, int c1, int band_rows = 0,
                                      long slot_elems = 0, int dst_img0 = 0) {
    return SpliceJob{src, dst, src_p0, dst_p0, planes, tile_begin, tile_count, cols, row0, m, r0, r1, c0, c1, band_rows, slot_elems, dst_img0};
}
int nd_launch_splices(const SpliceJob *jobs, int n, hipStream_t s);

int nd_launch_repitch(const QpBuf &src, int src_plane0, int planes, int ss, int sy, int sx, const QpBuf &dst, int oy, int ox, int h, int w,
                      hipStream_t s);
size_t nd_wgrad_partial_floats(int taps, int M, int N, long K, int *ksplit_out, int *cps_out);
int nd_launch_wgrad(const QpBuf &A, int a_plane0, int M, const QpBuf &Bq, int b_plane0, int N, int taps, int taps_total, int tap0,
                    float *partial, size_t partial_floats, float *dw, hipStream_t s);
int nd_launch_channel_sum(const QpBuf &src, int plane0, int C, float *out, float *scratch, hipStream_t s);
int nd_launch_maxpool_bwd_add(const QpBuf &gpool, const QpBuf &fwd, int fwd_plane0, const QpBuf &gfine, int g_plane0, int planes,
                              hipStream_t s);
int nd_launch_final_wgrad(const float *gy, int H, int W, const QpBuf &act, int cin, int crop, float *red, float *dw, float *db,
                          hipStream_t s);
int nd_launch_final_bwd_data(const float *gy, int H, int W, const float *w, int cin, int crop, const QpBuf &g, hipStream_t s);

int nd_launch_bn_train_fwd(const QpBuf &z, const QpBuf &a, int plane0, int cout, float momentum, const float *gamma, const float *beta,
                           float *rm, float *rv, float *stat, float *red, long red_floats, hipStream_t s);
int nd_launch_bn_train_bwd(const QpBuf &g, const QpBuf &a, int plane0, const QpBuf &z, int cout, const float *gamma, const float *stat,
                           float *coef, float *dgamma, float *dbeta, float *red, long red_floats, hipStream_t s);
```

nind_denoise_amd/csrc/pack.hip:

```cpp
#include <string.h>

#include "nd_common.h"

static thread_local char g_err[512] = "";

void nd_set_error(const char *fmt, ...) {
    va_list ap;
    va_start(ap, fmt);
    vsnprintf(g_err, sizeof(g_err), fmt, ap);
    va_end(ap);
}

extern "C" const char *nd_last_error(void) { return g_err; }
extern "C" int nd_version(void) { return 119; }

static inline uint16_t f32_to_bf16_rne(float f) {
    uint32_t u;
    memcpy(&u, &f, 4);
    if ((u & 0x7fffffffu) > 0x7f800000u) return (uint16_t)((u >> 16) | 0x40);
    return (uint16_t)((u + 0x7fffu + ((u >> 16) & 1u)) >> 16);
}
static inline uint16_t f32_to_f16_rne(float f) {
    const _Float16 h = (_Float16)f;
    uint16_t u;
    memcpy(&u, &h, 2);
    return u;
}

void nd_pack_layer(int kind, int cin, int cout, int dt, const float *w, const float *bias, float *packed) {
    const int taps = nd_taps(kind);
    const int KB = nd_kblocks(cin, dt);
    const int MT = nd_mtiles(kind, cout);
    const int M = kind == ND_CONVT2S2 ? 4 * cout : cout;
    const int cpp = nd_cpp(dt);
    float *bp = packed + nd_bias_offset(kind, cin, cout, dt);
    auto weff = [&](int m, int ci, int t) -> float {
        if (m >= M || ci >= cin) return 0.f;
        switch (kind) {
            case ND_CONV3: return w[((size_t)m * cin + ci) * 9 + t];
            case ND_CONVT3: return w[((size_t)ci * cout + m) * 9 + (8 - t)];
            case ND_CONVT2S2: {
                const NdUpRow r = nd_up_row(m, cout, dt);
                return w[((size_t)ci * cout + r.co) * 4 + 2 * r.a + r.b];
            }
            case ND_CONV2S2: return w[((size_t)m * cin + ci) * 4 + t];
            default: return w[(size_t)m * cin + ci];
        }
    };
    for (int mt = 0; mt < MT; ++mt)
        for (int kb = 0; kb < KB; ++kb)
            for (int t = 0; t < taps; ++t) {
                float *dst = packed + (((size_t)mt * KB + kb) * taps + t) * 256;
                uint16_t *dst16 = (uint16_t *)dst;
                for (int lane = 0; lane < 64; ++lane) {
                    const int i = lane & 31, h = lane >> 5;
                    const int m = 32 * mt + i;
                    for (int s = 0; s < cpp; ++s) {
                        const float v = weff(m, 2 * cpp * kb + cpp * h + s, t);
                        if (dt == ND_F32)
                            dst[lane * 4 + s] = v;
                        else
                            dst16[lane * 8 + s] = dt == ND_BF16 ? f32_to_bf16_rne(v) : f32_to_f16_rne(v);
                    }
                }
            }
    for (int m = 0; m < MT * 32; ++m) {
        float v = 0.f;
        if (m < M && bias) v = bias[kind == ND_CONVT2S2 ? nd_up_row(m, cout, dt).co : m];
        bp[m] = v;
    }
}

extern "C" size_t nd_layer_packed_bytes(int kind, int cin, int cout, int dtype) {
    if (dtype < ND_F32 || dtype > ND_F16 || kind < 0 || kind > 4 || cin <= 0 || cout <= 0) return 0;
    return nd_packed_floats(kind, cin, cout, dtype) * sizeof(float);
}

extern "C" int nd_layer_pack(int kind, int cin, int cout, int dtype, const float *weight, const float *bias,
                             void *packed_host, size_t packed_bytes) {
    if (dtype < ND_F32 || dtype > ND_F16) ND_FAIL(ND_EINVAL, "nd_layer_pack: unsupported dtype %d", dtype);
    if (kind < 0 || kind > 4 || cin <= 0 || cout <= 0 || !weight || !packed_host)
        ND_FAIL(ND_EINVAL, "nd_layer_pack: bad arguments");
    if (packed_bytes < nd_layer_packed_bytes(kind, cin, cout, dtype))
        ND_FAIL(ND_ENOMEM, "nd_layer_pack: packed buffer too small");
    nd_pack_layer(kind, cin, cout, dtype, weight, bias, (float *)packed_host);
    return ND_OK;
}
```

nind_denoise_amd/csrc/utnet.hip:

```cpp
#include <string.h>

#include <string>
#include <vector>

#include "nd_common.h"

#include "utnet_net.h"

extern "C" int nd_utnet_num_tensors(void) { return (int)tensor_names().size(); }
extern "C" const char *nd_utnet_tensor_name(int idx) {
    const auto &n = tensor_names();
    return (idx >= 0 && idx < (int)n.size()) ? n[idx].c_str() : nullptr;
}

extern "C" size_t nd_utnet_packed_bytes(int funit, int dtype) {
    if (check_funit(funit, dtype) != ND_OK) return 0;
    return blob_layout(funit, dtype).total * sizeof(float);
}

extern "C" int nd_utnet_pack_weights(int funit, int dtype, const float *const *tensors, int n_tensors, void *packed_host,
                                     size_t packed_bytes) {
    ND_TRY(check_funit(funit, dtype));
    if (n_tensors != nd_utnet_num_tensors()) ND_FAIL(ND_EINVAL, "nd_utnet_pack_weights: expected %d tensors, got %d", nd_utnet_num_tensors(), n_tensors);
    const BlobLayout bl = blob_layout(funit, dtype);
    if (packed_bytes < bl.total * sizeof(float)) ND_FAIL(ND_ENOMEM, "nd_utnet_pack_weights: packed buffer too small");
    float *blob = (float *)packed_host;
    memset(blob, 0, bl.total * sizeof(float));
    for (int i = 0; i < kNumLayers; ++i) {
        const LayerSpec &l = kLayers[i];
        const int wi = tensor_index(std::string(l.key) + ".weight"), bi = tensor_index(std::string(l.key) + ".bias");
        if (wi < 0 || bi < 0 || !tensors[wi] || !tensors[bi]) ND_FAIL(ND_EINVAL, "nd_utnet_pack_weights: missing tensor %s.{weight,bias}", l.key);
        const int ci = lcin(l, funit), co = lcout(l, funit);
        if (i == kNumLayers - 1) {
            memcpy(blob + bl.off[i], tensors[wi], sizeof(float) * 3 * ci);
            memcpy(blob + bl.off[i] + 3 * ci, tensors[bi], sizeof(float) * 3);
        } else {
            nd_pack_layer(l.kind, ci, co, dtype, tensors[wi], tensors[bi], blob + bl.off[i]);
            if (bl.woff[i]) ND_TRY(nd_wino_pack(kWinoTile, l.kind, ci, co, tensors[wi], tensors[bi], blob + bl.woff[i]));
            if (bl.w1off[i]) ND_TRY(nd_w1d_pack(kW1dTile, l.kind, ci, co, tensors[wi], tensors[bi], blob + bl.w1off[i]));
            if (bl.w1off2[i]) ND_TRY(nd_w1d_pack(2, l.kind, ci, co, tensors[wi], tensors[bi], blob + bl.w1off2[i]));
        }
        if (l.prelu >= 0) {
            std::string k(l.key);
            const size_t dot = k.rfind('.');
            const std::string an = k.substr(0, dot + 1) + std::to_string(atoi(k.c_str() + dot + 1) + 1) + ".weight";
            const int ai = tensor_index(an);
            blob[l.prelu] = (ai >= 0 && tensors[ai]) ? tensors[ai][0] : 0.25f;
        }
    }
    return ND_OK;
}

extern "C" int nd_utnet_pack_weights_device(int funit, int dtype, const float *const *tensors, int n_tensors, void *packed_dev,
                                            size_t packed_bytes, void *stream) {
    ND_TRY(check_funit(funit, dtype));
    if (n_tensors != nd_utnet_num_tensors()) ND_FAIL(ND_EINVAL, "nd_utnet_pack_weights_device: expected %d tensors, got %d", nd_utnet_num_tensors(), n_tensors);
    const BlobLayout bl = blob_layout(funit, dtype);
    if (!packed_dev || packed_bytes < bl.total * sizeof(float)) ND_FAIL(ND_ENOMEM, "nd_utnet_pack_weights_device: packed buffer too small");
    hipStream_t s = (hipStream_t)stream;
    float *blob = (float *)packed_dev;
    ND_HIP(hipMemsetAsync(blob, 0, bl.total * sizeof(float), s));
    for (int i = 0; i < kNumLayers; ++i) {
        const LayerSpec &l = kLayers[i];
        const int wi = tensor_index(std::string(l.key) + ".weight"), bi = tensor_index(std::string(l.key) + ".bias");
        if (wi < 0 || bi < 0 || !tensors[wi] || !tensors[bi]) ND_FAIL(ND_EINVAL, "nd_utnet_pack_weights_device: missing tensor %s.{weight,bias}", l.key);
        const int ci = lcin(l, funit), co = lcout(l, funit);
        if (i == kNumLayers - 1) {
            ND_HIP(hipMemcpyAsync(blob + bl.off[i], tensors[wi], sizeof(float) * 3 * ci, hipMemcpyDeviceToDevice, s));
            ND_HIP(hipMemcpyAsync(blob + bl.off[i] + 3 * ci, tensors[bi], sizeof(float) * 3, hipMemcpyDeviceToDevice, s));
        } else {
            ND_TRY(nd_pack_layer_device(l.kind, ci, co, dtype, tensors[wi], tensors[bi], blob + bl.off[i], s));
            if (bl.woff[i]) ND_TRY(nd_pack_wino_device(kWinoTile, l.kind, ci, co, tensors[wi], tensors[bi], blob + bl.woff[i], s));
            if (bl.w1off[i]) ND_TRY(nd_pack_w1d_device(kW1dTile, l.kind, ci, co, tensors[wi], tensors[bi], blob + bl.w1off[i], s));
            if (bl.w1off2[i]) ND_TRY(nd_pack_w1d_device(2, l.kind, ci, co, tensors[wi], tensors[bi], blob + bl.w1off2[i], s));
        }
        if (l.prelu >= 0) {
            std::string k(l.key);
            const size_t dot = k.rfind('.');
            const std::string an = k.substr(0, dot + 1) + std::to_string(atoi(k.c_str() + dot + 1) + 1) + ".weight";
            const int ai = tensor_index(an);
            if (ai >= 0 && tensors[ai]) {
                ND_HIP(hipMemcpyAsync(blob + l.prelu, tensors[ai], sizeof(float), hipMemcpyDeviceToDevice, s));
            } else {
                const float dflt = 0.25f;
                ND_HIP(hipMemcpyAsync(blob + l.prelu, &dflt, sizeof(float), hipMemcpyHostToDevice, s));
                ND_HIP(hipStreamSynchronize(s));
            }
        }
    }
    return ND_OK;
}

extern "C" size_t nd_utnet_workspace_bytes_hw(int funit, int h, int w, int batch, int dtype) {
    if (check_net(funit, h, w, batch, dtype) != ND_OK) return 0;
    return make_plan(funit, h, w, batch, batch, nullptr, dtype).bytes;
}

extern "C" int nd_utnet_workspace_init_hw(void *ws, size_t ws_bytes, int funit, int h, int w, int batch, int dtype,
                                          void *stream) {
    ND_TRY(check_net(funit, h, w, batch, dtype));
    const size_t need = make_plan(funit, h, w, batch, batch, nullptr, dtype).bytes;
    if (!ws || ws_bytes < need) ND_FAIL(ND_ENOMEM, "UtNet workspace: %zu B given, %zu B needed", ws_bytes, need);
    ND_HIP(hipMemsetAsync(ws, 0, need, (hipStream_t)stream));
    return ND_OK;
}

extern "C" int nd_utnet_forward_hw(int funit, int act, int dtype, int flags, const void *packed, const float *x, float *y,
                                   int batch, int h, int w, void *ws, size_t ws_bytes, void *stream) {
    ND_TRY(nd_check_flags(flags));
    Plan pl;
    ND_TRY(forward_common(funit, act, dtype, packed, batch, batch, h, w, ws, ws_bytes, &pl));
    if (!x || !y) ND_FAIL(ND_EINVAL, "UtNet: null tensor");
    hipStream_t s = (hipStream_t)stream;
    const float *blob = (const float *)packed;
    ND_TRY(nd_launch_reflect_pack(x, batch, h, w, pl.buf[X0], s));
    StackOpts o;
    o.flags = flags;
    ND_TRY(run_stack(funit, act, dtype, blob, pl, s, o));
    const BlobLayout bl = blob_layout(funit, dtype);
    const float *fw = blob + bl.off[kNumLayers - 1];
    ND_TRY(nd_launch_final1x1(pl.buf[T4B], funit, fw, fw + 3 * funit, 2, y, h, w, s));
    return ND_OK;
}

extern "C" int nd_utnet_denoise_tiles(int funit, int act, int dtype, int flags, const void *packed, const float *img,
                                      float *canvas, int width, int height, int cs, int ucs, int ol, int tile_begin,
                                      int tile_count, int batch, void *ws, size_t ws_bytes, void *stream) {
    return nd_utnet_denoise_tiles_ok(funit, act, dtype, flags, packed, img, canvas, width, height, cs, ucs, ol, tile_begin, tile_count, batch,
                                     ws, ws_bytes, stream, nullptr);
}

int nd_utnet_denoise_tiles_ok(int funit, int act, int dtype, int flags, const void *packed, const float *img, float *canvas, int width,
                              int height, int cs, int ucs, int ol, int tile_begin, int tile_count, int batch, void *ws, size_t ws_bytes,
                              void *stream, unsigned char *tile_ok) {
    ND_TRY(nd_check_flags(flags));
    Plan pl;
    ND_TRY(forward_common(funit, act, dtype, packed, batch, tile_count, cs, cs, ws, ws_bytes, &pl));
    if (!img || !canvas) ND_FAIL(ND_EINVAL, "UtNet: null image");
    hipStream_t s = (hipStream_t)stream;
    const float *blob = (const float *)packed;
    ND_TRY(nd_launch_gather_pack(img, width, height, cs, ucs, ol, tile_begin, tile_count, pl.buf[X0], s));
    const BlobLayout bl = blob_layout(funit, dtype);
    Roi rois[kNumSteps];
    StackOpts o;
    o.flags = flags;
    const int crop = (cs - ucs) / 2;
    if (!(flags & ND_FLAG_FULL_TILES) && plan_rois(pl, crop, crop, rois) && rois_supported(funit, dtype, flags, pl, bl, rois)) o.rois = rois;
    ND_TRY(run_stack(funit, act, dtype, blob, pl, s, o));
    const float *fw = blob + bl.off[kNumLayers - 1];
    return nd_launch_utnet_stitch(pl.buf[T4B], funit, fw, fw + 3 * funit, canvas, width, height, cs, ucs, ol, tile_begin, tile_count,
                                  tile_ok, s);
}

namespace {
template <int N>
struct Events {
    hipEvent_t ev[N];
    int n = 0;
    int create() {
        for (; n < N; ++n) ND_HIP(hipEventCreate(&ev[n]));
        return ND_OK;
    }
    ~Events() { for (int i = 0; i < n; ++i) (void)hipEventDestroy(ev[i]); }
};
}

extern "C" int nd_utnet_profile_stack(int funit, int act, int dtype, int flags, const void *packed, int batch, int cs, int crop,
                                      void *ws, size_t ws_bytes, void *stream, nd_step_profile *steps, int max_steps) {
    ND_TRY(nd_check_flags(flags));
    Plan pl;
    ND_TRY(forward_common(funit, act, dtype, packed, batch, batch, cs, cs, ws, ws_bytes, &pl));
    if (max_steps < kNumSteps || !steps) ND_FAIL(ND_EINVAL, "nd_utnet_profile_stack: need room for %d steps", kNumSteps);
    if (crop < 0 || 2 * crop >= cs) ND_FAIL(ND_EINVAL, "nd_utnet_profile_stack: crop %d", crop);
    hipStream_t s = (hipStream_t)stream;
    Events<kNumSteps + 1 + 2 * kNumSteps> evs;
    ND_TRY(evs.create());
    hipEvent_t *const ev = evs.ev, *const evx = evs.ev + kNumSteps + 1;
    const BlobLayout bl = blob_layout(funit, dtype);
    Roi rois[kNumSteps];
    StackOpts opts;
    opts.flags = flags;
    opts.ev = ev;
    opts.ev_x = evx;
    long tiles_run[kNumSteps] = {};
    opts.wino_tiles = tiles_run;
    if (!(flags & ND_FLAG_FULL_TILES) && plan_rois(pl, crop, crop, rois) && rois_supported(funit, dtype, flags, pl, bl, rois)) opts.rois = rois;
    int rc = run_stack(funit, act, dtype, (const float *)packed, pl, s, opts);
    if (rc == ND_OK) {
        hipError_t e = hipStreamSynchronize(s);
        if (e != hipSuccess) {
            nd_set_error("hipStreamSynchronize failed: %s", hipGetErrorString(e));
            rc = ND_EHIP;
        }
    }
    for (int i = 0; i < kNumSteps && rc == ND_OK; ++i) {
        nd_step_profile &o = steps[i];
        memset(&o, 0, sizeof(o));
        if (hipEventElapsedTime(&o.ms, ev[i], ev[i + 1]) != hipSuccess) {
            nd_set_error("hipEventElapsedTime failed");
            rc = ND_EHIP;
            break;
        }
        const Step &st = kSteps[i];
        const Form form = step_form(st, funit, dtype, flags, pl, bl);
        o.form = (int)form;
        o.kind = st.layer >= 0 ? kLayers[st.layer].kind : -1;
        const QpBuf &in = pl.buf[st.src], &out = pl.buf[st.dst];
        const double B = batch, esz = 16.0 / nd_cpp(dtype);
        double hin = in.Hb - 2 * in.pad, win = in.Wb - 2 * in.pad;
        if (opts.rois && opts.rois[i].rows > 0) {
            const bool t3 = kLayers[st.layer].kind == ND_CONVT3;
            hin = opts.rois[i].rows - (t3 ? 2 : 0);
            win = opts.rois[i].cols - (t3 ? 2 : 0);
        }
        if (st.layer < 0) {
            const double c = st.dst_plane0_mul * funit;
            o.bytes = B * c * esz * (hin * win + (hin / 2) * (win / 2));
            continue;
        }
        const LayerSpec &l = kLayers[st.layer];
        const double ci = lcin(l, funit), co = lcout(l, funit);
        const double cip = nd_kblocks((int)ci, dtype) * 2.0 * nd_cpp(dtype);
        double hout, wout;
        switch (l.kind) {
            case ND_CONV3: hout = hin - 2; wout = win - 2; o.flops = 2.0 * hout * wout * ci * co * 9; break;
            case ND_CONVT3: hout = hin + 2; wout = win + 2; o.flops = 2.0 * hin * win * ci * co * 9; break;
            case ND_CONVT2S2: hout = 2 * hin; wout = 2 * win; o.flops = 2.0 * hin * win * ci * co * 4; break;
            default: hout = hin; wout = win; o.flops = 2.0 * hin * win * ci * co; break;
        }
        o.flops *= B;
        o.bytes = B * esz * (ci * hin * win + co * hout * wout) + 4.0 * ci * co * nd_taps(l.kind);
        auto cdiv = [](double a, double b) { return (double)(long)((a + b - 1) / b); };
// ... 143 lines not shown
    d.in = pl.in;
    d.out = pl.out;
    d.part = pl.split;
    d.part_bytes = kSplitScratchBytes;
    return d;
}
int launch_form(const LayerForm &fm, const ConvDesc &d, void *scratch, size_t scratch_bytes, hipStream_t s) {
    switch (fm.fam) {
        case LF_W1D: return nd_launch_conv_w1d(fm.T, d, s);
        case LF_W2D: return nd_launch_conv_w2d(d, s);
        case LF_WINO3P: return nd_launch_conv_wino(fm.T, d, scratch, scratch_bytes, s);
        default: return nd_launch_conv(d, s);
    }
}

int layer_forward(const LayerForm &fm, int kind, int act, float slope, int dt, const void *packed, const float *x, int batch,
                  int cin, int h, int w, int cout, float *y, void *ws, size_t ws_bytes, int variant, int flags, hipStream_t s) {
    const LayerPlan pl = layer_plan(kind, batch, cin, cout, h, w, (char *)ws, dt);
    ND_HIP(hipMemsetAsync(ws, 0, pl.bytes, s));
    ND_TRY(nd_launch_nchw_to_qp(x, cin, pl.in, 0, s));
    ConvDesc d = layer_desc(fm, kind, cin, cout, dt, (const float *)packed, pl);
    d.act = act;
    d.slope = slope;
    d.variant = variant;
    d.nosplit = (flags & ND_FLAG_NO_SPLITK) != 0;
    d.tile_wino = (flags & ND_FLAG_TILE_WINO) != 0;
    ND_TRY(launch_form(fm, d, (char *)ws + pl.bytes, ws_bytes - pl.bytes, s));
    return nd_launch_qp_to_nchw(pl.out, 0, y, cout, s);
}
}

extern "C" size_t nd_layer_workspace_bytes(int kind, int batch, int cin, int cout, int h, int w, int dtype) {
    if (dtype < ND_F32 || dtype > ND_F16 || kind < 0 || kind > 4 || batch <= 0 || cin <= 0 || cout <= 0 || h <= 0 || w <= 0) return 0;
    if (kind == ND_CONV3 && (h < 3 || w < 3)) return 0;
    return layer_plan(kind, batch, cin, cout, h, w, nullptr, dtype).bytes;
}

extern "C" int nd_layer_forward(int kind, int act, float slope, int dtype, const void *packed, const float *x, int batch,
                                int cin, int h, int w, int cout, float *y, void *ws, size_t ws_bytes, int variant, int flags,
                                void *stream) {
    ND_TRY(nd_check_flags(flags));
    if (dtype < ND_F32 || dtype > ND_F16) ND_FAIL(ND_EINVAL, "nd_layer_forward: unsupported dtype %d", dtype);
    const size_t need = nd_layer_workspace_bytes(kind, batch, cin, cout, h, w, dtype);
    if (!need) ND_FAIL(ND_EINVAL, "nd_layer_forward: bad shape");
    if (!ws || ws_bytes < need) ND_FAIL(ND_ENOMEM, "nd_layer_forward: workspace %zu B given, %zu B needed", ws_bytes, need);
    if (cout % nd_cpp(dtype)) ND_FAIL(ND_EINVAL, "nd_layer_forward: cout must be a multiple of %d", nd_cpp(dtype));
    return layer_forward(kDirect, kind, act, slope, dtype, packed, x, batch, cin, h, w, cout, y, ws, ws_bytes, variant, flags,
                         (hipStream_t)stream);
}

extern "C" size_t nd_winograd_packed_bytes(int tile, int cin, int cout) {
    const LayerForm fm = wino_form(tile);
    if (fm.fam == LF_NONE || cin <= 0 || cout <= 0) return 0;
    return wino_packed_floats(fm, cin, cout) * sizeof(float);
}
extern "C" int nd_winograd_pack(int tile, int kind, int cin, int cout, const float *w, const float *bias, void *packed,
                                size_t packed_bytes) {
    const size_t need = nd_winograd_packed_bytes(tile, cin, cout);
    if (!need) ND_FAIL(ND_EINVAL, "nd_winograd_pack: bad shape");
    if (!packed || packed_bytes < need) ND_FAIL(ND_ENOMEM, "nd_winograd_pack: %zu B given, %zu B needed", packed_bytes, need);
    const LayerForm fm = wino_form(tile);
    if (fm.fam == LF_WINO3P) return nd_wino_pack(fm.T, kind, cin, cout, w, bias, (float *)packed);
    return nd_w1d_pack(fm.T, kind, cin, cout, w, bias, (float *)packed);
}
extern "C" size_t nd_layer_winograd_workspace_bytes(int tile, int kind, int batch, int cin, int cout, int h, int w) {
    const LayerForm fm = wino_form(tile);
    if (fm.fam == LF_NONE || (kind != ND_CONV3 && kind != ND_CONVT3)) return 0;
    const size_t base = nd_layer_workspace_bytes(kind, batch, cin, cout, h, w, ND_F32);
    if (!base || fm.fam != LF_WINO3P) return base;
    const LayerPlan pl = layer_plan(kind, batch, cin, cout, h, w, nullptr, ND_F32);
    return base + nd_wino_scratch_bytes(fm.T, pl.in, cin, cout);
}
extern "C" int nd_layer_forward_winograd(int tile, int kind, int act, float slope, const void *packed, const float *x, int batch,
                                         int cin, int h, int w, int cout, float *y, void *ws, size_t ws_bytes, int flags,
                                         void *stream) {
    ND_TRY(nd_check_flags(flags));
    const size_t need = nd_layer_winograd_workspace_bytes(tile, kind, batch, cin, cout, h, w);
    if (!need) ND_FAIL(ND_EINVAL, "nd_layer_forward_winograd: bad shape / kind / tile");
    if (!ws || ws_bytes < need) ND_FAIL(ND_ENOMEM, "nd_layer_forward_winograd: workspace %zu B given, %zu B needed", ws_bytes, need);
    return layer_forward(wino_form(tile), kind, act, slope, ND_F32, packed, x, batch, cin, h, w, cout, y, ws, ws_bytes, -1, flags,
                         (hipStream_t)stream);
}

extern "C" int nd_maxpool2_forward(const float *x, int batch, int c, int h, int w, float *y, void *ws, size_t ws_bytes,
                                   void *stream) {
    if (batch <= 0 || c <= 0 || h < 2 || w < 2) ND_FAIL(ND_EINVAL, "nd_maxpool2_forward: bad shape");
    QpBuf in, out;
    in.planes = out.planes = (c + 3) / 4;
    in.B = out.B = batch;
    in.Hb = h; in.Wb = w; in.pad = 0; in.pstride = (long)batch * h * w;
    out.Hb = h / 2; out.Wb = w / 2; out.pad = 0; out.pstride = (long)batch * (h / 2) * (w / 2);
    const size_t ib = ((size_t)in.planes * in.pstride * 16 + 255) & ~(size_t)255;
    const size_t need = ib + (size_t)out.planes * out.pstride * 16;
    if (!ws || ws_bytes < need) ND_FAIL(ND_ENOMEM, "nd_maxpool2_forward: workspace %zu B given, %zu B needed", ws_bytes, need);
    in.base = (float *)ws;
    out.base = (float *)((char *)ws + ib);
    hipStream_t s = (hipStream_t)stream;
    ND_TRY(nd_launch_nchw_to_qp(x, c, in, 0, s));
    ND_TRY(nd_launch_maxpool2(in, 0, in.planes, out, s));
    ND_TRY(nd_launch_qp_to_nchw(out, 0, y, c, s));
    return ND_OK;
}

__global__ void k_fill_random(float *p, size_t n, unsigned seed) {
    size_t i = (size_t)blockIdx.x * blockDim.x + threadIdx.x;
    const size_t stride = (size_t)gridDim.x * blockDim.x;
    for (; i < n; i += stride) {
        unsigned h = (unsigned)i * 2654435761u ^ seed;
        h ^= h >> 15; h *= 2246822519u; h ^= h >> 13;
        p[i] = ((h & 0xFFFF) - 32768.f) * (1.f / 65536.f);
    }
}

__global__ void k_fill_random16(unsigned short *p, size_t n, unsigned seed, int dt) {
    size_t i = (size_t)blockIdx.x * blockDim.x + threadIdx.x;
    const size_t stride = (size_t)gridDim.x * blockDim.x;
    for (; i < n; i += stride) {
        unsigned h = (unsigned)i * 2654435761u ^ seed;
        h ^= h >> 15; h *= 2246822519u; h ^= h >> 13;
        const float f = ((h & 0xFFFF) - 32768.f) * (1.f / 65536.f);
        if (dt == ND_BF16) {
            const __bf16 v = (__bf16)f;
            p[i] = *(const unsigned short *)&v;
        } else {
            const _Float16 v = (_Float16)f;
            p[i] = *(const unsigned short *)&v;
        }
    }
}

namespace {
void fill_random(void *ws, size_t bytes, float *wpk, size_t wfloats, int dt, int kind, int cin, int cout, hipStream_t s) {
    if (dt == ND_F32) {
        hipLaunchKernelGGL(k_fill_random, dim3(2048), dim3(256), 0, s, (float *)ws, bytes / 4, 12345u);
        hipLaunchKernelGGL(k_fill_random, dim3(1024), dim3(256), 0, s, wpk, wfloats, 777u);
        return;
    }
    hipLaunchKernelGGL(k_fill_random16, dim3(2048), dim3(256), 0, s, (unsigned short *)ws, bytes / 2, 12345u, dt);
    hipLaunchKernelGGL(k_fill_random16, dim3(1024), dim3(256), 0, s, (unsigned short *)wpk, wfloats * 2, 777u, dt);
    hipLaunchKernelGGL(k_fill_random, dim3(64), dim3(256), 0, s, wpk + nd_bias_offset(kind, cin, cout, dt), (size_t)nd_mtiles(kind, cout) * 32, 99u);
}

int time_form(const char *what, const LayerForm &fm, const ConvDesc &d, void *scratch, size_t scratch_bytes, int iters,
              hipStream_t s, float *mean_ms) {
    ND_TRY(launch_form(fm, d, scratch, scratch_bytes, s));
    Events<2> ev;
    ND_TRY(ev.create());
    ND_HIP(hipEventRecord(ev.ev[0], s));
    int rc = ND_OK;
    for (int i = 0; i < iters && rc == ND_OK; ++i) rc = launch_form(fm, d, scratch, scratch_bytes, s);
    (void)hipEventRecord(ev.ev[1], s);
    if (hipStreamSynchronize(s) != hipSuccess && rc == ND_OK) {
        nd_set_error("%s: stream failed", what);
        rc = ND_EHIP;
    }
    float ms = 0;
    (void)hipEventElapsedTime(&ms, ev.ev[0], ev.ev[1]);
    if (mean_ms) *mean_ms = ms / (iters > 0 ? iters : 1);
    return rc;
}
}

extern "C" int nd_conv_bench(int kind, int dtype, int batch, int cin, int cout, int h, int w, int variant, int iters, void *ws,
                             size_t ws_bytes, void *stream, float *mean_ms) {
    const size_t need = nd_layer_workspace_bytes(kind, batch, cin, cout, h, w, dtype);
    if (!need) ND_FAIL(ND_EINVAL, "nd_conv_bench: bad shape");
// ... 42 lines not shown
```

nind_denoise_amd/csrc/utnet_frame.hip:

```cpp
#include <string.h>

#include "nd_common.h"

#include "utnet_net.h"

namespace {

constexpr int kSharedSteps = 6, kLevel2End = 9;
constexpr int kStrip = 16, kStrip2 = 6;
constexpr double kBandBytes = 8.0 * (1 << 30);

struct Level {
    int begin, end;
    Buf in, out;
    int strip;
    int out_shift;
    bool three_pass;
    bool by_side;
};
const Level kLevels[2] = {{0, kSharedSteps, X0, P2, kStrip, 2, false, false}, {kSharedSteps, kLevel2End, P2, P3, kStrip2, 3, true, true}};
struct SkipSpec { Buf cat; int level, edge; };
const SkipSpec kSkips[3] = {{CAT4, 0, 2}, {CAT3, 0, 1}, {CAT2, 1, 1}};
inline int skip_step(Buf cat) {
    for (int i = 0; i < kNumSteps; ++i)
// ... 392 lines not shown
int assemble_output(const Frame &c, int l, const Plan &tp, const Plan &cp, int t0, int cnt) {
    const FramePlan &fp = c.fp;
    const Level &lv = kLevels[l];
    const QpBuf &dst = tp.buf[lv.out], &bt = c.full[l].buf[lv.out];
    const int n = c.tile[lv.out], step = fp.S >> lv.out_shift, per_band = fp.R * fp.cols;
    SpliceList jobs = {c.s};
    SpliceMap whole;
    whole.step_y = whole.step_x = step;
    const int strip = l + 1 < c.nlev ? kLevels[l + 1].strip : 0;
    if (strip > 0 && n >= 2 * strip) {
        for (int k = 0; k < 4; ++k) {
            const int r0 = (k >> 1) ? n - strip : 1, c0 = (k & 1) ? n - strip : 1;
            ND_TRY(jobs.add(nd_splice_job(bt, 0, dst, 0, dst.planes, t0, cnt, fp.cols, 0, whole, r0, r0 + strip - 1, c0, c0 + strip - 1, fp.R,
                                          slot_elems(bt, fp.slots))));
        }
    } else {
        ND_TRY(jobs.add(nd_splice_job(bt, 0, dst, 0, dst.planes, t0, cnt, fp.cols, 0, whole, 1, n - 1, 1, n - 1, fp.R, slot_elems(bt, fp.slots))));
    }
    for (int b = t0 / per_band; b <= (t0 + cnt - 1) / per_band; ++b) {
        const int lo = t0 > b * per_band ? t0 : b * per_band, hi = t0 + cnt < (b + 1) * per_band ? t0 + cnt : (b + 1) * per_band;
        const int row0 = b * fp.R, nrows = c.tile_rows(b);
        const QpBuf rl = row_plan(fp, l, c.f, c.dt, nrows, c.ws.rows[l], b & 1).buf[lv.out];
        const QpBuf cl = col_plan(fp, l, c.f, c.dt, nrows, c.cs, c.ws.cols[l], b & 1).buf[lv.out];
        for (int side = 0; side < 2; ++side) {
            const int at = side * (n - 1);
            SpliceMap mr, mc;
            mr.step_x = mc.step_y = step;
            line_image(lv, side, nrows, &mr.img_y, &mr.img_add);
            line_image(lv, side, fp.cols, &mc.img_x, &mc.img_add);
            mr.oy = mc.ox = -at;
            ND_TRY(jobs.add(nd_splice_job(rl, 0, dst, 0, dst.planes, lo, hi - lo, fp.cols, row0, mr, at, at + 1, 1, n - 1, 0, 0, lo - t0)));
            ND_TRY(jobs.add(nd_splice_job(cl, 0, dst, 0, dst.planes, lo, hi - lo, fp.cols, row0, mc, 1, n - 1, at, at + 1, 0, 0, lo - t0)));
        }
    }
    for (int k = 0; k < 4; ++k) {
        const int r = (k >> 1) * (n - 1), col = (k & 1) * (n - 1);
        SpliceMap m;
        m.img_t = lv.by_side ? 1 : 4;
        m.img_add = lv.by_side ? k * cnt : k;
        m.oy = -r;
        m.ox = -col;
        ND_TRY(jobs.add(nd_splice_job(cp.buf[lv.out], 0, dst, 0, dst.planes, t0, cnt, fp.cols, 0, m, r, r + 1, col, col + 1)));
    }
    return jobs.flush();
}

}

extern "C" size_t nd_utnet_frame_workspace_bytes(int funit, int dtype, int flags, int width, int height, int cs, int ucs, int ol,
                                                 int batch) {
    FramePlan fp;
    if (nd_check_flags(flags, true) != ND_OK || frame_plan(funit, dtype, flags, width, height, cs, ucs, ol, batch, &fp) != ND_OK) return 0;
    return fp.bytes;
}

extern "C" int nd_utnet_frame_plan(int funit, int dtype, int flags, int width, int height, int cs, int ucs, int ol, int *out) {
    ND_TRY(nd_check_flags(flags, true));
    if (!out) ND_FAIL(ND_EINVAL, "nd_utnet_frame_plan: null output");
    FramePlan fp;
    ND_TRY(frame_plan(funit, dtype, flags, width, height, cs, ucs, ol, 1, &fp));
    const int v[8] = {fp.D, fp.aligned, fp.R, fp.nbands, fp.S, fp.cols, fp.rows, fp.in_h[0]};
    memcpy(out, v, sizeof(v));
    return ND_OK;
}

extern "C" int nd_utnet_frame_levels(int funit, int dtype, int flags, int width, int height, int cs, int ucs, int ol, int *levels) {
    ND_TRY(nd_check_flags(flags, true));
    if (!levels) ND_FAIL(ND_EINVAL, "nd_utnet_frame_levels: null output");
    FramePlan fp;
    ND_TRY(frame_plan(funit, dtype, flags, width, height, cs, ucs, ol, 1, &fp));
    *levels = fp.levels;
    return ND_OK;
}

extern "C" int nd_utnet_frame_folds(int funit, int dtype, int flags, int width, int height, int cs, int ucs, int ol, int *mask) {
    ND_TRY(nd_check_flags(flags, true));
    if (!mask) ND_FAIL(ND_EINVAL, "nd_utnet_frame_folds: null output");
    FramePlan fp;
    ND_TRY(frame_plan(funit, dtype, flags, width, height, cs, ucs, ol, 1, &fp));
    *mask = fp.folds;
    return ND_OK;
}

static int denoise_frame(int funit, int act, int dtype, int flags, const void *packed, const float *img, float *canvas, int width,
                         int height, int cs, int ucs, int ol, int tile_begin, int tile_count, int batch, void *ws, size_t ws_bytes, void *fws,
                         size_t fws_bytes, void *stream, nd_progress_fn progress, void *progress_ctx, unsigned char *tile_ok) {
    ND_TRY(nd_check_flags(flags, true));
    Frame c = {funit, act, dtype, flags, (const float *)packed, img, canvas, width, height, cs, ucs, ol, batch, (hipStream_t)stream};
    FramePlan &fp = c.fp;
    ND_TRY(frame_plan(funit, dtype, flags, width, height, cs, ucs, ol, batch, &fp));
    if (tile_begin < 0 || tile_count < 0 || tile_begin + tile_count > fp.cols * fp.rows)
        ND_FAIL(ND_EINVAL, "nd_utnet_denoise_frame: tiles [%d,+%d) outside the grid of %d", tile_begin, tile_count, fp.cols * fp.rows);
    const int end = tile_begin + tile_count;
    ND_TRY(forward_common(funit, act, dtype, packed, batch, batch, cs, cs, ws, ws_bytes, &c.pl));
    c.bl = blob_layout(funit, dtype);
    const int crop = (cs - ucs) / 2;
    if (fp.D && !(plan_rois(c.pl, crop, crop, c.rois) && rois_supported(funit, dtype, flags, c.pl, c.bl, c.rois))) fp.D = 0;
    if (fp.D == 0) {
        int n = 0;
        for (int t0 = tile_begin; t0 < end; t0 += batch, ++n) {
            const int cnt = end - t0 < batch ? end - t0 : batch;
            if (progress) progress(progress_ctx, n, t0, cnt);
            ND_TRY(nd_utnet_denoise_tiles_ok(funit, act, dtype, flags & ~(ND_FLAG_TILE_LEVEL2 | ND_FLAG_TILE_SKIPS), packed, img, canvas, width, height, cs, ucs, ol, t0, cnt, batch, ws,
                                             ws_bytes, stream, tile_ok));
        }
        return ND_OK;
    }
    if (!img || !canvas) ND_FAIL(ND_EINVAL, "UtNet: null image");
    if (!fws || fws_bytes < fp.bytes || ((uintptr_t)fws & 255))
        ND_FAIL(ND_ENOMEM, "nd_utnet_denoise_frame: frame workspace %zu B given, %zu B needed (256-byte aligned)", fws_bytes, fp.bytes);
    c.ws = frame_ws(fp, (char *)fws);
    c.nlev = shared_levels(fp);
    c.tile = extents_from(X0, cs + 4);
    for (int l = 0; l < c.nlev; ++l) c.full[l] = band_plan(fp, l, funit, dtype, fp.R, cs, c.ws.band[l]);
    for (int k = 0; k < 3; ++k) {
        if (kSkips[k].level >= c.nlev) continue;
        Frame::Skip &sk = c.skips[k];
        sk.step = skip_step(kSkips[k].cat);
        sk.form = step_form(kSteps[sk.step], funit, dtype, flags, c.pl, c.bl);
        sk.in_place = form_takes_src2(kSteps[sk.step], sk.form, funit, flags, c.pl);
        sk.fold = ((fp.folds >> k) & 1) && sk.in_place;
    }
    const float *fw = c.blob + c.bl.off[kNumLayers - 1];
    StepSrc2 src2[3];
    StackOpts dec;
    dec.flags = flags;
    dec.step_begin = kLevels[c.nlev - 1].end;
    dec.rois = c.rois;
    dec.src2 = src2;
    const int per_band = fp.R * fp.cols;
    int band_done = tile_begin / per_band - 1;
    for (int t0 = tile_begin, n = 0; t0 < end; ++n) {
        const int b0 = t0 / per_band;
        int cnt = end - t0 < batch ? end - t0 : batch;
        if (t0 + cnt > (b0 + 2) * per_band) cnt = (b0 + 2) * per_band - t0;
        for (; band_done < (t0 + cnt - 1) / per_band; ++band_done) ND_TRY(build_band(c, band_done + 1));
        if (progress) progress(progress_ctx, n, t0, cnt);
        const Plan tp = make_plan(funit, cs, cs, batch, cnt, (char *)ws, dtype);
        Plan cp;
        ND_TRY(corner_patches(c, 0, tp, t0, cnt, &cp));
        ND_TRY(bind_skips(c, tp, t0, cnt, src2, &dec.nsrc2));
        ND_TRY(assemble_output(c, 0, tp, cp, t0, cnt));
        for (int l = 1; l < c.nlev; ++l) {
            ND_TRY(corner_patches(c, l, tp, t0, cnt, &cp));
            ND_TRY(assemble_output(c, l, tp, cp, t0, cnt));
        }
        ND_TRY(run_stack(funit, act, dtype, c.blob, tp, c.s, dec));
        ND_TRY(nd_launch_utnet_stitch(tp.buf[T4B], funit, fw, fw + 3 * funit, canvas, width, height, cs, ucs, ol, t0, cnt, tile_ok, c.s));
        t0 += cnt;
    }
    return ND_OK;
}

extern "C" int nd_utnet_denoise_frame(int funit, int act, int dtype, int flags, const void *packed, const float *img, float *canvas,
                                      int width, int height, int cs, int ucs, int ol, int tile_begin, int tile_count, int batch,
                                      void *ws, size_t ws_bytes, void *fws, size_t fws_bytes, void *stream, nd_progress_fn progress,
                                      void *progress_ctx) {
    return denoise_frame(funit, act, dtype, flags, packed, img, canvas, width, height, cs, ucs, ol, tile_begin, tile_count, batch, ws, ws_bytes,
                         fws, fws_bytes, stream, progress, progress_ctx, nullptr);
}

extern "C" int nd_utnet_denoise_frame_checked(int funit, int act, int dtype, int flags, const void *packed, const float *img, float *canvas,
                                              int width, int height, int cs, int ucs, int ol, int tile_begin, int tile_count, int batch,
                                              void *ws, size_t ws_bytes, void *fws, size_t fws_bytes, void *stream,
                                              nd_progress_fn progress, void *progress_ctx, unsigned char *tile_ok) {
    if (!tile_ok) ND_FAIL(ND_EINVAL, "nd_utnet_denoise_frame_checked: null tile_ok");
    return denoise_frame(funit, act, dtype, flags, packed, img, canvas, width, height, cs, ucs, ol, tile_begin, tile_count, batch, ws, ws_bytes,
                         fws, fws_bytes, stream, progress, progress_ctx, tile_ok);
}
```

nind_denoise_amd/csrc/utnet_net.h:

```cpp
#pragma once
#include <string.h>

#include <string>
#include <vector>

#include "nd_common.h"

namespace {

struct LayerSpec {
    const char *key;
    int kind;
    int cin_mul, cout_mul;
    int prelu;
};

const LayerSpec kLayers[] = {
    {"convs1.0", ND_CONV3, 0, 1, 0},    {"convs1.2", ND_CONV3, 1, 1, 1},    {"convs2.0", ND_CONV3, 1, 2, 2},
    {"convs2.2", ND_CONV3, 2, 2, 3},    {"convs3.0", ND_CONV3, 2, 4, 4},    {"convs3.2", ND_CONV3, 4, 4, 5},
    {"convs4.0", ND_CONV3, 4, 8, 6},    {"convs4.2", ND_CONV3, 8, 8, 7},    {"bottom.0", ND_CONV3, 8, 16, 8},
    {"bottom.2", ND_CONVT3, 16, 16, 9}, {"up1", ND_CONVT2S2, 16, 8, -1},    {"tconvs1.0", ND_CONVT3, 16, 8, 10},
    {"tconvs1.2", ND_CONVT3, 8, 8, 11}, {"up2", ND_CONVT2S2, 8, 4, -1},     {"tconvs2.0", ND_CONVT3, 8, 4, 12},
    {"tconvs2.2", ND_CONVT3, 4, 4, 13}, {"up3", ND_CONVT2S2, 4, 2, -1},     {"tconvs3.0", ND_CONVT3, 4, 2, 14},
    {"tconvs3.2", ND_CONVT3, 2, 2, 15}, {"up4", ND_CONVT2S2, 2, 1, -1},     {"tconvs4.0", ND_CONVT3, 2, 1, 16},
// ... 241 lines not shown
            const int kind = kLayers[st.layer].kind;
            if (kind != ND_CONVT3 && kind != ND_CONVT2S2) continue;
            if (hi[dim][st.dst] < 0) continue;
            const QpBuf &src = pl.buf[st.src];
            const int si = (dim ? src.Wb : src.Hb) - 2 * src.pad;
            int a = lo[dim][st.dst], b = hi[dim][st.dst];
            if (kind == ND_CONVT3) {
                a = a - 2 < 0 ? 0 : a - 2;
                b = b > si ? si : b;
            } else {
                a = a >> 1;
                b = (b + 1) >> 1;
                b = b > si ? si : b;
            }
            if (a < lo[dim][st.src]) lo[dim][st.src] = a;
            if (b > hi[dim][st.src]) hi[dim][st.src] = b;
        }
    }
    for (int i = 0; i < kNumSteps; ++i) {
        const Step &st = kSteps[i];
        if (st.layer < 0) continue;
        const int kind = kLayers[st.layer].kind;
        if (kind != ND_CONVT3 && kind != ND_CONVT2S2) continue;
        const Buf b = kind == ND_CONVT3 ? st.dst : st.src;
        const QpBuf &q = pl.buf[b];
        const int H = q.Hb - 2 * q.pad, W = q.Wb - 2 * q.pad;
        int r0 = 0, r1 = H, c0 = 0, c1 = W;
        if (kind == ND_CONVT3) {
            if (hi[0][b] >= 0) { r0 = lo[0][b]; r1 = hi[0][b]; }
            if (hi[1][b] >= 0) { c0 = lo[1][b]; c1 = hi[1][b]; }
        } else {
            if (hi[0][st.dst] >= 0) { r0 = lo[0][st.dst] >> 1; r1 = (hi[0][st.dst] + 1) >> 1; }
            if (hi[1][st.dst] >= 0) { c0 = lo[1][st.dst] >> 1; c1 = (hi[1][st.dst] + 1) >> 1; }
        }
        r0 = r0 < 0 ? 0 : r0; c0 = c0 < 0 ? 0 : c0;
        r1 = r1 > H ? H : r1; c1 = c1 > W ? W : c1;
        if (r0 == 0 && c0 == 0 && r1 == H && c1 == W) continue;
        if (r1 <= r0 || c1 <= c0) continue;
        roi[i] = Roi{r0, c0, r1 - r0, c1 - c0};
        any = true;
    }
    return any;
}

inline bool rois_supported(int f, int dt, int flags, const Plan &pl, const BlobLayout &bl, const Roi *rois) {
    for (int i = 0; i < kNumSteps; ++i) {
        if (rois[i].rows <= 0) continue;
        const Form form = step_form(kSteps[i], f, dt, flags, pl, bl);
        if (form == FORM_DIRECT) {
            const LayerSpec &l = kLayers[kSteps[i].layer];
            ConvDesc d;
            d.kind = l.kind;
            d.cin = lcin(l, f);
            d.cout = lcout(l, f);
            d.in = pl.buf[kSteps[i].src];
            d.out = pl.buf[kSteps[i].dst];
            d.roi_r0 = rois[i].r0;
            d.roi_c0 = rois[i].c0;
            d.roi_rows = rois[i].rows;
            d.roi_cols = rois[i].cols;
            if (!nd_conv_roi_fits(d)) return false;
            continue;
        }
        if (form == FORM_WINO3P) continue;
        if (form == FORM_W1D4 && !(flags & ND_FLAG_W1D_REGS)) continue;
        return false;
    }
    return true;
}

struct StepSrc2 {
    int step = -1;
    QpBuf buf = {};
    int plane0 = 0, from = 0;
    const int *origin = nullptr;
    long origin_max = 0;
    bool addend = false;
};
inline bool form_takes_src2(const Step &st, Form form, int f, int flags, const Plan &pl) {
    if (form == FORM_WINO3P) return kWinoTile == 6;
    return form == FORM_W1D4 && nd_f43_w2d(pl.buf[st.src], lcout(kLayers[st.layer], f), false, flags);
}

struct StackOpts {
    int flags = 0;
    const Roi *rois = nullptr;
    int step_begin = 0, step_end = kNumSteps;
    const StepSrc2 *src2 = nullptr;
    int nsrc2 = 0;
    hipEvent_t *ev = nullptr;
    hipEvent_t *ev_x = nullptr;
    long *wino_tiles = nullptr;
    const QpBuf *pre = nullptr;
    const unsigned char *train_w1 = nullptr;
};
int run_stack(int f, int act, int dt, const float *blob, const Plan &pl, hipStream_t s, const StackOpts &o) {
    const QpBuf *const pre = o.pre;
    const int flags = o.flags, step_begin = o.step_begin, step_end = o.step_end;
    const BlobLayout bl = blob_layout(f, dt, pre != nullptr);
    const int cpp = nd_cpp(dt);
    int si = step_begin;
    bool pool_done = false;
    QpBuf pool_view;
    for (int k = step_begin; k < step_end; ++k) {
        const Step &st = kSteps[k];
        if (o.ev) ND_HIP(hipEventRecord(o.ev[si], s));
        const int this_step = si++;
        if (st.layer < 0) {
            if (pool_done) {
                pool_done = false;
                continue;
            }
            ND_TRY(nd_launch_maxpool2(pl.buf[st.src], st.dst_plane0_mul * f / cpp, st.dst_plane0_mul * f / cpp, pl.buf[st.dst], s));
            continue;
        }
        const LayerSpec &l = kLayers[st.layer];
        ConvDesc d;
        d.kind = l.kind;
        d.act = l.prelu >= 0 ? act : ND_ACT_NONE;
        d.slope = 0.25f;
        d.slope_dev = (l.prelu >= 0 && act == ND_ACT_PRELU) ? blob + l.prelu : nullptr;
        if (pre && l.prelu >= 0) {
            d.pre = pre[l.prelu].base;
            d.pre_plane = pre[l.prelu].np();
        }
        const int cin = lcin(l, f);
        d.cin = cin;
        d.cout = lcout(l, f);
        d.wpk = blob + bl.off[st.layer];
        d.bias = d.wpk + nd_bias_offset(l.kind, d.cin, d.cout, dt);
        d.in = pl.buf[st.src];
        d.out = pl.buf[st.dst];
        d.out_plane0 = st.dst_plane0_mul * f / cpp;
        d.part = pl.split;
        d.part_bytes = kSplitScratchBytes;
        d.nosplit = (flags & ND_FLAG_NO_SPLITK) != 0;
        d.tile_wino = (flags & ND_FLAG_TILE_WINO) != 0;
        const Form form = step_form(st, f, dt, flags, pl, bl, o.train_w1);
        if (o.rois && o.rois[this_step].rows > 0) {
            d.roi_r0 = o.rois[this_step].r0;
            d.roi_c0 = o.rois[this_step].c0;
            d.roi_rows = o.rois[this_step].rows;
            d.roi_cols = o.rois[this_step].cols;
        }
        for (int i = 0; i < o.nsrc2; ++i)
            if (o.src2[i].step == k && o.src2[i].addend) {
                d.add = o.src2[i].buf;
                d.add_plane0 = o.src2[i].plane0;
                d.add_origin = o.src2[i].origin;
                d.add_origin_max = o.src2[i].origin_max;
                d.w_kb = nd_kblocks(cin, dt);
                d.cin = o.src2[i].from * cpp;
            } else if (o.src2[i].step == k) {
                d.in2 = o.src2[i].buf;
                d.in2_plane0 = o.src2[i].plane0;
                d.in2_from = o.src2[i].from;
                d.in2_origin = o.src2[i].origin;
                d.in2_origin_max = o.src2[i].origin_max;
            }
        const bool next_is_pool = this_step + 1 < step_end && kSteps[this_step + 1].layer < 0;
        const bool w2d = form == FORM_W1D4 && nd_f43_w2d(d.in, d.cout, pre != nullptr, flags);
        if (next_is_pool && !pre && !(flags & ND_FLAG_UNFUSED_POOL)) {
            pool_view = pl.buf[kSteps[this_step + 1].dst];
            d.pool = &pool_view;
            pool_done = w2d || form == FORM_WINO3P || (form == FORM_DIRECT && dt != ND_F32 && nd_conv_pool_fits(d));
            if (!pool_done) d.pool = nullptr;
        }
        if (form == FORM_W1D4 || form == FORM_W1D2) {
            const int T = form == FORM_W1D4 ? kW1dTile : 2;
            if (!pre) d.wpk = blob + (T == kW1dTile ? bl.w1off[st.layer] : bl.w1off2[st.layer]);
            d.bias = d.wpk + nd_bias_offset(d.kind, cin, d.cout, ND_F32, T);
            ND_TRY(form == FORM_W1D4 ? nd_launch_conv_f43(d, flags, s) : nd_launch_conv_w1d(T, d, s));
            continue;
        }
        if (form == FORM_WINO3P) {
            d.wpk = blob + bl.woff[st.layer];
            d.bias = nullptr;
            const int nimg = d.in.B;
            for (int b0 = 0; b0 < nimg; b0 += kWinoChunk) {
                ConvDesc c = d;
                c.in.B = c.out.B = nimg - b0 < kWinoChunk ? nimg - b0 : kWinoChunk;
                c.in.base = d.in.base + (size_t)b0 * d.in.Hb * d.in.Wb * 4;
                c.out.base = d.out.base + (size_t)b0 * d.out.Hb * d.out.Wb * 4;
                QpBuf pv;
                if (d.pool) {
                    pv = *d.pool;
                    pv.B = c.in.B;
                    pv.base = d.pool->base + (size_t)b0 * pv.Hb * pv.Wb * 4;
                    c.pool = &pv;
                }
                if (d.in2_origin) c.in2_origin = d.in2_origin + b0;
                if (d.add_origin) c.add_origin = d.add_origin + b0;
                ND_TRY(nd_launch_conv_wino(kWinoTile, c, pl.wino, pl.wino_bytes, s, (o.ev_x && nimg <= kWinoChunk) ? o.ev_x + 2 * this_step : nullptr));
                if (o.wino_tiles) o.wino_tiles[this_step] += nd_wino_launch_tiles(kWinoTile, c);
            }
            continue;
        }
        ND_TRY(nd_launch_conv(d, s));
    }
    if (o.ev) ND_HIP(hipEventRecord(o.ev[si], s));
    return ND_OK;
}

}
```

nind_denoise_amd/networks/UtNet.py:

```python
import ctypes

import torch
from torch import nn

from .. import _lib
from ._autograd import FlatState, NetFunction
from ..synth import utnet_layer_table, utnet_prelu_keys

_ACTIVATIONS = {"PReLU": nn.PReLU, "ELU": nn.ELU, "Hardswish": nn.Hardswish}
_SHORT_DTYPE = {_lib.ND_F32: "f32", _lib.ND_BF16: "bf16", _lib.ND_F16: "f16"}


def canonical_compute_dtype(name):
    if name not in _lib.DTYPE:
        raise ValueError(f"unknown compute dtype {name!r}; choose one of {', '.join(_lib.DTYPE)}")
    return _SHORT_DTYPE[_lib.DTYPE[name]]


FALLBACK_DTYPES = {"f16": ("bf16", "f32"), "bf16": ("f32",)}


def canonical_fallback_dtype(name):
    if name is None or (isinstance(name, str) and name.strip().lower() in ("", "none")):
        return None
    return canonical_compute_dtype(name)


def check_fallback_pair(compute_dtype, fallback_dtype):
    if fallback_dtype is None or fallback_dtype in FALLBACK_DTYPES.get(compute_dtype, ()):
        return fallback_dtype
    pairs = ", ".join(f"{c} -> {' | '.join(f)}" for c, f in FALLBACK_DTYPES.items())
    raise ValueError(f"fallback_dtype={fallback_dtype!r} cannot serve compute_dtype={compute_dtype!r}; choose one of: {pairs} "
                     "(or none)")


def valid_cs(cs):
    return cs >= 104 and (cs - 56) % 16 == 0


def nearest_valid_cs(cs):
    k = (cs - 56 + 8) // 16
    return max(104, 16 * k + 56)


class UtNet(nn.Module):
    split_k = True
    mosaic_wino = True
    winograd = True
    w1d_regs = False
    useful_only = True
    fused_pool = True
    share_encoder = True
    share_level2 = True
    fold_skips = True

    def __init__(self, funit=64, activation='PReLU', compute_dtype='f32', fallback_dtype=None):
        super().__init__()
        funit = int(funit)
        compute_dtype = canonical_compute_dtype(compute_dtype)
        fallback_dtype = check_fallback_pair(compute_dtype, canonical_fallback_dtype(fallback_dtype))
        if activation not in _ACTIVATIONS:
            exit(f'UtNet: unknown activation function: {activation}')
        self.funit, self.activation = funit, activation
        groups = {}
        for key, kind, cin, cout, k in utnet_layer_table(funit):
            if kind == "conv":
                layer = nn.Conv2d(cin, cout, k)
            elif kind == "convT":
                layer = nn.ConvTranspose2d(cin, cout, k)
            else:
                layer = nn.ConvTranspose2d(cin, cout, k, stride=2)
            if "." in key:
                seq, idx = key.split(".")
                groups.setdefault(seq, {})[int(idx)] = layer
            else:
                groups[key] = layer
        for key in utnet_prelu_keys():
            seq, idx = key.split(".")
            groups[seq][int(idx)] = _ACTIVATIONS[activation]()
        order = ["convs1", "convs2", "convs3", "convs4", "bottom"]
        for n in range(1, 5):
            order += [f"up{n}", f"tconvs{n}"]
        for name in order:
            g = groups[name]
            self.add_module(name, nn.Sequential(*[g[i] for i in sorted(g)]) if isinstance(g, dict) else g)
        self._packed = {}
        self.pack_on_device = True
        self._workspaces = {}
        self.max_cached_workspaces = 2
        self._fallback_workspaces = {}
        self.compute_dtype = compute_dtype
        self.fallback_dtype = fallback_dtype
        self.weights_generation = 0

    def set_compute_dtype(self, name):
        self.compute_dtype = canonical_compute_dtype(name)
        return self

    def set_fallback_dtype(self, name):
        self.fallback_dtype = check_fallback_pair(self.compute_dtype, canonical_fallback_dtype(name))
        return self

    def checked_fallback_dtype(self):
        return check_fallback_pair(self.compute_dtype, self.fallback_dtype)

    @property
    def _dt(self):
        return _lib.DTYPE[self.compute_dtype]

    @property
    def flags(self):
        return ((0 if self.split_k else _lib.FLAG_NO_SPLITK) | (0 if self.winograd else _lib.FLAG_DIRECT_CONV) |
                (_lib.FLAG_W1D_REGS if self.w1d_regs else 0) | (0 if self.useful_only else _lib.FLAG_FULL_TILES) |
                (0 if self.fused_pool else _lib.FLAG_UNFUSED_POOL) | (0 if self.share_encoder else _lib.FLAG_TILE_ENCODER) |
                (0 if self.mosaic_wino else _lib.FLAG_TILE_WINO))

    @property
    def frame_flags(self):
        return self.flags | (0 if self.share_level2 else _lib.FLAG_TILE_LEVEL2) | (0 if self.fold_skips else _lib.FLAG_TILE_SKIPS)

    def _weights_key(self, device):
        return (str(device), self.weights_generation) + tuple((p.data_ptr(), p._version) for p in self.parameters())

    def packed_weights(self, device, dtype=None):
        dtype = self.compute_dtype if dtype is None else canonical_compute_dtype(dtype)
        dt = _lib.DTYPE[dtype]
        key = self._weights_key(device)
        hit = self._packed.get(dtype)
        if hit is not None and hit[0] == key:
            return hit[1]
        lib = _lib.load()
        sd = self.state_dict()
        names = _lib.utnet_tensor_names()
        nbytes = lib.nd_utnet_packed_bytes(self.funit, dt)
        if nbytes == 0:
            raise ValueError(f"UtNet: funit={self.funit} is not supported by the HIP path for {dtype} "
                             "(multiple of 8 for f32, of 16 for bf16 / f16)")
        on_device = self.pack_on_device
        where = device if on_device else "cpu"
        keep = []
        ptrs = (ctypes.c_void_p * len(names))()
        for i, n in enumerate(names):
            if n in sd:
                t = sd[n].detach().to(device=where, dtype=torch.float32).contiguous()
                keep.append(t)
                ptrs[i] = t.data_ptr()
            else:
                ptrs[i] = None
        if on_device:
            dev_blob = torch.empty(nbytes // 4, dtype=torch.float32, device=device)
            with torch.cuda.device(device):
                _lib.check(lib.nd_utnet_pack_weights_device(self.funit, dt, ptrs, len(names), dev_blob.data_ptr(), nbytes,
                                                            _lib.stream_ptr(device)), "nd_utnet_pack_weights_device")
                torch.cuda.current_stream(device).synchronize()
        else:
            blob = torch.empty(nbytes // 4, dtype=torch.float32)
            _lib.check(lib.nd_utnet_pack_weights(self.funit, dt, ptrs, len(names), blob.data_ptr(), nbytes),
                       "nd_utnet_pack_weights")
            dev_blob = blob.to(device)
        self._packed[dtype] = (key, dev_blob)
        return dev_blob

    def workspace(self, cs, batch, device, width=None, dtype=None):
        h, w = int(cs), int(cs if width is None else width)
        other = dtype is not None and canonical_compute_dtype(dtype) != self.compute_dtype
        dtype = canonical_compute_dtype(dtype) if other else self.compute_dtype
        cache = self._fallback_workspaces if other else self._workspaces
        key = (str(device), h, w, int(batch), dtype)
        ws = cache.get(key)
        if ws is None:
            lib = _lib.load()

            def drop():
                while len(cache) >= (1 if other else self.max_cached_workspaces):
                    cache.pop(next(iter(cache)))
            ws = _lib.make_workspace(lib.nd_utnet_workspace_bytes_hw, lib.nd_utnet_workspace_init_hw,
                                     (self.funit, h, w, batch, _lib.DTYPE[dtype]), device, "UtNet", drop=drop)
            cache[key] = ws
        return ws

    def frame_workspace(self, width, height, cs, ucs, ol, batch, device):
        lib = _lib.load()
        nbytes = lib.nd_utnet_frame_workspace_bytes(self.funit, self._dt, self.frame_flags, width, height, cs, ucs, ol, batch)
        if nbytes == 0:
            return None
        key = (str(device), "frame", nbytes)
        ws = self._workspaces.get(key)
        if ws is None:
            for k in [k for k in self._workspaces if k[1] == "frame"]:
                del self._workspaces[k]
            ws = torch.zeros(nbytes, dtype=torch.uint8, device=device)
            self._workspaces[key] = ws
        return ws

    def forward(self, l):
        if l.device.type != "cuda":
            raise RuntimeError("nind_denoise_amd.UtNet runs on the MI355X HIP path only (no CPU fallback); "
                               "move the module and its input to the GPU")
        if l.dim() != 4 or l.size(1) != 3:
            raise ValueError(f"UtNet expects [B,3,H,W], got {tuple(l.shape)}")
        batch, h, w = l.size(0), l.size(2), l.size(3)
        for cs in (h, w):
# ... 52 lines not shown
```

Measured before the change: 90.46 MP/s.

## Fuse final 1x1 head conv into last transposed-conv w2d kernel epilogue

Folds the final 1x1 (funit->3) output convolution into the epilogue of the last conv_w2d layer. Each wave accumulates the 3-channel head dot products from registers, and two half-waves combine through LDS. Only 3 channels are written instead of the full 64-channel activation, and the stitch kernel then just reads and accumulates them. This removes a large HBM write and read of the last feature map and the per-pixel dot3 in the stitch. The cost is extra LDS, a workgroup barrier and more register pressure in the last layer.

```diff
diff --git a/include/nind_hip.h b/include/nind_hip.h
--- a/include/nind_hip.h
+++ b/include/nind_hip.h
@@ -46,6 +46,7 @@
     ND_FLAG_FIND_NOISE = 128,
     ND_FLAG_TILE_SKIPS = 256,
     ND_FLAG_TILE_WINO = 512,
+    ND_FLAG_TILE_HEAD = 1024,
     ND_FLAG_FULL_TILES = 8
 } nd_flags;
 
@@ -104,6 +105,8 @@
 int nd_utnet_frame_plan(int funit, int dtype, int flags, int width, int height, int cs, int ucs, int ol, int *out);
 int nd_utnet_frame_levels(int funit, int dtype, int flags, int width, int height, int cs, int ucs, int ol, int *levels);
 int nd_utnet_frame_folds(int funit, int dtype, int flags, int width, int height, int cs, int ucs, int ol, int *mask);
+int nd_utnet_last_buffer(int funit, int cs, int batch, int dtype, size_t *offset, size_t *plane_bytes, int *planes, int *side);
+int nd_utnet_frame_head(int funit, int dtype, int flags, int width, int height, int cs, int ucs, int ol, int *fused);
 
 typedef struct nd_step_profile {
     float ms;
@@ -247,6 +250,9 @@
 int nd_layer_forward_winograd(int tile, int kind, int act, float slope, const void *packed, const float *x, int batch,
                               int cin, int h, int w, int cout, float *y, void *workspace, size_t workspace_bytes, int flags,
                               void *stream);
+int nd_layer_head_forward(int fused, int act, float slope, const void *packed_dev, const float *head_dev, const float *x, int batch,
+                          int cin, int h, int w, int cout, const int *roi, float *raw_dev, float *y3_dev, void *workspace,
+                          size_t workspace_bytes, void *stream);
 
 int nd_conv_bench(int kind, int dtype, int batch, int cin, int cout, int h, int w, int variant, int iters,
                   void *workspace, size_t workspace_bytes, void *stream, float *mean_ms);
diff --git a/nind_denoise_amd/_lib.py b/nind_denoise_amd/_lib.py
--- a/nind_denoise_amd/_lib.py
+++ b/nind_denoise_amd/_lib.py
@@ -12,6 +12,7 @@
 FLAG_NO_SPLITK, FLAG_DIRECT_CONV, FLAG_W1D_REGS, FLAG_FULL_TILES, FLAG_UNFUSED_POOL, FLAG_TILE_ENCODER, FLAG_TILE_LEVEL2 = 1, 2, 4, 8, 16, 32, 64
 FLAG_FIND_NOISE = 128
 FLAG_TILE_SKIPS = 256
+FLAG_TILE_HEAD = 1024
 FLAG_TILE_WINO = 512
 PROGRESS_FN = ctypes.CFUNCTYPE(None, c_void_p, c_int, c_int, c_int)
 
@@ -92,6 +93,8 @@
     "nd_utnet_frame_plan": (c_int, [c_int] * 8 + [POINTER(c_int)]),
     "nd_utnet_frame_levels": (c_int, [c_int] * 8 + [POINTER(c_int)]),
     "nd_utnet_frame_folds": (c_int, [c_int] * 8 + [POINTER(c_int)]),
+    "nd_utnet_last_buffer": (c_int, [c_int] * 4 + [POINTER(c_size_t)] * 2 + [POINTER(c_int)] * 2),
+    "nd_utnet_frame_head": (c_int, [c_int] * 8 + [POINTER(c_int)]),
     "nd_utnet_denoise_frame": (c_int, [c_int] * 4 + [c_void_p] * 3 + [c_int] * 8 + [c_void_p, c_size_t, c_void_p, c_size_t, c_void_p,
                                                                                     PROGRESS_FN, c_void_p]),
     "nd_utnet_denoise_frame_checked": (c_int, [c_int] * 4 + [c_void_p] * 3 + [c_int] * 8 + [c_void_p, c_size_t, c_void_p, c_size_t,
@@ -106,6 +109,8 @@
     "nd_layer_winograd_workspace_bytes": (c_size_t, [c_int] * 7),
     "nd_layer_forward_winograd": (c_int, [c_int, c_int, c_int, c_float, c_void_p, c_void_p] + [c_int] * 5
                                   + [c_void_p, c_void_p, c_size_t, c_int, c_void_p]),
+    "nd_layer_head_forward": (c_int, [c_int, c_int, c_float, c_void_p, c_void_p, c_void_p] + [c_int] * 5
+                              + [POINTER(c_int), c_void_p, c_void_p, c_void_p, c_size_t, c_void_p]),
     "nd_maxpool2_forward": (c_int, [c_void_p] + [c_int] * 4 + [c_void_p, c_void_p, c_size_t, c_void_p]),
     "nd_layer_wgrad_workspace_bytes": (c_size_t, [c_int] * 6),
     "nd_layer_wgrad": (c_int, [c_int, c_void_p, c_void_p] + [c_int] * 5 + [c_void_p, c_void_p, c_void_p, c_size_t, c_void_p]),
diff --git a/nind_denoise_amd/csrc/aux_kernels.hip b/nind_denoise_amd/csrc/aux_kernels.hip
--- a/nind_denoise_amd/csrc/aux_kernels.hip
+++ b/nind_denoise_amd/csrc/aux_kernels.hip
@@ -755,7 +755,7 @@
     return ND_OK;
 }
 
-template <int DT, bool GUARD>
+template <int DT, bool GUARD, bool HEAD = false>
 __device__ __forceinline__ void final1x1_stitch_pixel(const typename Elem<DT>::vec *__restrict__ src, long np, int Hb, int Wb, int planes,
                                                       int cin, const float *__restrict__ w, const float *__restrict__ bias, int crop,
                                                       float *__restrict__ canvas, const TileGeo &g, int tile_begin, int tile_count,
@@ -775,8 +775,18 @@
     bool any = false;
     for_each_cover(g, X, Y, tile_begin, tile_count, [&](int t, int iy, int ix, float f) {
         if (GUARD && !tile_ok[tile_begin + t]) return;
-        float o0 = bias[0], o1 = bias[1], o2 = bias[2];
-        dot3<DT>(src + ((size_t)t * Hb + iy + crop) * Wb + ix + crop, np, planes, w, cin, o0, o1, o2);
+        float o0, o1, o2;
+        if constexpr (HEAD) {
+            const typename Elem<DT>::vec v = src[((size_t)t * Hb + iy + crop) * Wb + ix + crop];
+            o0 = (float)v[0];
+            o1 = (float)v[1];
+            o2 = (float)v[2];
+        } else {
+            o0 = bias[0];
+            o1 = bias[1];
+            o2 = bias[2];
+            dot3<DT>(src + ((size_t)t * Hb + iy + crop) * Wb + ix + crop, np, planes, w, cin, o0, o1, o2);
+        }
         if (sigmoid) {
             o0 = 1.f / (1.f + expf(-o0));
             o1 = 1.f / (1.f + expf(-o1));
@@ -817,7 +827,14 @@
                                     tile_ok);
 }
 
-template <int DT>
+template <bool GUARD>
+__global__ void k_head_stitch(const f32x4 *__restrict__ src, int Hb, int Wb, int crop, float *__restrict__ canvas, TileGeo g, int tile_begin,
+                              int tile_count, int y_first, const unsigned char *__restrict__ tile_ok) {
+    final1x1_stitch_pixel<ND_F32, GUARD, true>(src, 0, Hb, Wb, 0, 0, nullptr, nullptr, crop, canvas, g, tile_begin, tile_count, y_first, 0, nullptr,
+                                               tile_ok);
+}
+
+template <int DT, bool HEAD = false>
 __global__ __launch_bounds__(256) void k_tile_verdict(const typename Elem<DT>::vec *__restrict__ src, long np, int Hb, int Wb,
                                                       int planes, int cin, const float *__restrict__ w,
                                                       const float *__restrict__ bias, int crop, TileGeo g, int tile_begin,
@@ -833,8 +850,18 @@
     const int p = blockIdx.x * blockDim.x + threadIdx.x;
     if (p >= uw * uh) return;
     const int dy = p / uw, dx = p - dy * uw;
-    float o0 = bias[0], o1 = bias[1], o2 = bias[2];
-    dot3<DT>(src + ((size_t)t * Hb + g.pad + dy + crop) * Wb + g.pad + dx + crop, np, planes, w, cin, o0, o1, o2);
+    float o0, o1, o2;
+    if constexpr (HEAD) {
+        const typename Elem<DT>::vec v = src[((size_t)t * Hb + g.pad + dy + crop) * Wb + g.pad + dx + crop];
+        o0 = (float)v[0];
+        o1 = (float)v[1];
+        o2 = (float)v[2];
+    } else {
+        o0 = bias[0];
+        o1 = bias[1];
+        o2 = bias[2];
+        dot3<DT>(src + ((size_t)t * Hb + g.pad + dy + crop) * Wb + g.pad + dx + crop, np, planes, w, cin, o0, o1, o2);
+    }
     const unsigned e = 0x7f800000u;
     if ((__float_as_uint(o0) & e) == e || (__float_as_uint(o1) & e) == e || (__float_as_uint(o2) & e) == e) tile_ok[i] = 0;
 }
@@ -860,6 +887,33 @@
     ND_DISPATCH_DT(src.dt, hipLaunchKernelGGL(k_final1x1_stitch<DT>, grid, dim3(256), 0, s, (const typename Elem<DT>::vec *)src.base,
                                               src.np(), src.Hb, src.Wb, (cin + n - 1) / n, cin, w, bias, crop, canvas, g,
                                               tile_begin, tile_count, yf, sigmoid, noise_img));
+    ND_HIP(hipGetLastError());
+    return ND_OK;
+}
+
+int nd_launch_head_stitch(const QpBuf &src, int crop, float *canvas, int W, int H, int cs, int ucs, int ol, int tile_begin, int tile_count,
+                          unsigned char *tile_ok, hipStream_t s) {
+    TileGeo g;
+    int yf, yr;
+    if (src.dt != ND_F32) ND_FAIL(ND_EINVAL, "head_stitch: fp32 only");
+    ND_TRY(stitch_launch_geo(src, crop, W, H, cs, ucs, ol, tile_begin, tile_count, &g, &yf, &yr));
+    const f32x4 *p0 = (const f32x4 *)src.base;
+    if (tile_ok) {
+        if (tile_begin < 0 || tile_count <= 0 || tile_count > 65535 || tile_begin + tile_count > g.cols * g.rows)
+            ND_FAIL(ND_EINVAL, "head_stitch: tiles [%d,+%d) outside the grid of %d (at most 65535 per launch)", tile_begin, tile_count,
+                    g.cols * g.rows);
+        const int uwmax = g.cs - 2 * g.pad;
+        if (uwmax > 0)
+            hipLaunchKernelGGL((k_tile_verdict<ND_F32, true>), dim3((uwmax * uwmax + 255) / 256, tile_count), dim3(256), 0, s, p0, 0L, src.Hb,
+                               src.Wb, 0, 0, nullptr, nullptr, crop, g, tile_begin, tile_count, tile_ok);
+    }
+    if (yr > 0) {
+        dim3 grid((W + 255) / 256, yr);
+        if (tile_ok)
+            hipLaunchKernelGGL(k_head_stitch<true>, grid, dim3(256), 0, s, p0, src.Hb, src.Wb, crop, canvas, g, tile_begin, tile_count, yf, tile_ok);
+        else
+            hipLaunchKernelGGL(k_head_stitch<false>, grid, dim3(256), 0, s, p0, src.Hb, src.Wb, crop, canvas, g, tile_begin, tile_count, yf, nullptr);
+    }
     ND_HIP(hipGetLastError());
     return ND_OK;
 }
diff --git a/nind_denoise_amd/csrc/conv_qp.inc b/nind_denoise_amd/csrc/conv_qp.inc
--- a/nind_denoise_amd/csrc/conv_qp.inc
+++ b/nind_denoise_amd/csrc/conv_qp.inc
@@ -81,6 +81,7 @@
     long add_plane;
     const int *origin_add;
     int W_add;
+    const float *head_w, *head_b;
 };
 
 static inline void nd_conv_fastdivs(ConvParams &p) {
diff --git a/nind_denoise_amd/csrc/conv_w2d.hip b/nind_denoise_amd/csrc/conv_w2d.hip
--- a/nind_denoise_amd/csrc/conv_w2d.hip
+++ b/nind_denoise_amd/csrc/conv_w2d.hip
@@ -17,6 +17,7 @@
 constexpr int kStages = 2;
 constexpr int kScratch = 2048;
 constexpr int kLds = kStages * kStage + 8 * kScratch;
+constexpr int kHeadLds = 1024;
 constexpr int kDmaAt = 4;
 constexpr int kXfAt = 12;
 constexpr int kSlots = 4 * 32 * 4;
@@ -57,7 +58,7 @@
 #endif
 struct Strip { int img, y0, x0; bool ok; };
 
-template <int DBG, bool SRC2 = false, bool ADD = false>
+template <int DBG, bool SRC2 = false, bool ADD = false, bool HEAD = false>
 __global__ __launch_bounds__(512) void conv_w2d(ConvParams p) {
     extern __shared__ __attribute__((aligned(16))) char smem[];
     const int lane = threadIdx.x & 63;
@@ -95,6 +96,12 @@
             nsteps += it.c1 - it.c0;
         }
     if (nsteps == 0) return;
+
+    if constexpr (HEAD) {
+        float *const hw = (float *)(smem + kLds);
+        const int nw = 3 * p.cout;
+        for (int i = threadIdx.x; i < nw + 3; i += 512) hw[i] = i < nw ? p.head_w[i] : p.head_b[i - nw];
+    }
 
     const unsigned tot = (unsigned)p.nimg * (unsigned)p.PV;
     auto strip_of = [&](int nb, int s) -> Strip {
@@ -293,8 +300,16 @@
             add_loads(1);
             __builtin_amdgcn_sched_barrier(0);
         }
-        const bool okP = !SRC2 && !ADD && p.pool && !(lane & 2) && st.ok && 2 * pxp + 1 < p.wpx && 2 * pyp + 1 < p.Hv;
+        const bool okP = !SRC2 && !ADD && !HEAD && p.pool && !(lane & 2) && st.ok && 2 * pxp + 1 < p.wpx && 2 * pyp + 1 < p.Hv;
         const unsigned offP = (unsigned)((st.img * p.pool_P + (pyp + p.pool_pad) * p.pool_W + pxp + p.pool_pad) * 16);
+        float ha[3] = {0.f, 0.f, 0.f}, hb[3] = {0.f, 0.f, 0.f};
+        if constexpr (HEAD) {
+            if (wm == 0) {
+                const float *hbias = (const float *)(smem + kLds) + 3 * p.cout;
+#pragma unroll
+                for (int o = 0; o < 3; ++o) ha[o] = hb[o] = hbias[o];
+            }
+        }
 #pragma unroll
         for (int g = 0; g < 4; ++g) {
             f32x4 yy[4], ypre[4];
@@ -334,7 +349,7 @@
                     yy[i][2 * pr + 1] = y[i][1];
                 }
             }
-            if (!SRC2 && !ADD && p.pre) {
+            if (!SRC2 && !ADD && !HEAD && p.pre) {
                 const Strip so = strip_of(nb, sl);
                 const int yo = so.y0 + rr, m4 = (q0 + 2 * g + h) * 4, left = p.wpx - so.x0;
                 if (so.ok && yo < p.Hv && m4 < p.M) {
@@ -387,7 +402,7 @@
                     }
                 }
                 f32x4 vp = va;
-                if (!SRC2 && !ADD && p.pool) {
+                if (!SRC2 && !ADD && !HEAD && p.pool) {
                     const f32x4 *blk = (const f32x4 *)scratch + (2 * e_row) * 16 + pp_i;
                     const f32x4 p00 = blk[0], p01 = blk[1], p10 = blk[16], p11 = blk[17];
 #pragma unroll
@@ -397,12 +412,46 @@
                 __builtin_amdgcn_wave_barrier();
                 __builtin_amdgcn_fence(__ATOMIC_ACQUIRE, "wavefront");
                 const int quad = q0 + 2 * g + hq;
-                if (quad * 4 < p.M && !(DBG & 1)) {
+                if constexpr (HEAD) {
+                    if (quad * 4 < p.M) {
+                        const float *hw = (const float *)(smem + kLds) + 4 * quad;
+#pragma unroll
+                        for (int o = 0; o < 3; ++o) {
+                            const f32x4 w = *(const f32x4 *)(hw + o * p.cout);
+#pragma unroll
+                            for (int e = 0; e < 4; ++e) {
+                                ha[o] = fmaf(va[e], w[e], ha[o]);
+                                hb[o] = fmaf(vb2[e], w[e], hb[o]);
+                            }
+                        }
+                    }
+                } else if (quad * 4 < p.M && !(DBG & 1)) {
                     char *pb = (char *)(p.out + (size_t)(p.out_plane0 + quad) * p.out_plane);
                     if (okA) *(f32x4 *)(pb + offA) = va;
                     if (okB) *(f32x4 *)(pb + offB) = vb2;
                     if (okP) *(f32x4 *)((char *)(p.pool + (size_t)quad * p.pool_plane) + offP) = vp;
                 }
+            }
+        }
+        if constexpr (HEAD) {
+            float *const hs = (float *)scratch;
+            if (wm == 1) {
+#pragma unroll
+                for (int o = 0; o < 3; ++o) {
+                    hs[o * 64 + lane] = ha[o];
+                    hs[(3 + o) * 64 + lane] = hb[o];
+                }
+            }
+            __builtin_amdgcn_fence(__ATOMIC_RELEASE, "workgroup");
+            __builtin_amdgcn_s_barrier();
+            __builtin_amdgcn_fence(__ATOMIC_ACQUIRE, "workgroup");
+            if (wm == 0) {
+                const float *ps = (const float *)(scratch + 4 * kScratch);
+                const f32x4 ra = {ha[0] + ps[lane], ha[1] + ps[64 + lane], ha[2] + ps[128 + lane], 0.f};
+                const f32x4 rb = {hb[0] + ps[192 + lane], hb[1] + ps[256 + lane], hb[2] + ps[320 + lane], 0.f};
+                char *pb = (char *)(p.out + (size_t)p.out_plane0 * p.out_plane);
+                if (okA) *(f32x4 *)(pb + offA) = ra;
+                if (okB) *(f32x4 *)(pb + offB) = rb;
             }
         }
     };
@@ -551,7 +600,10 @@
     if (d.pre && (roi || d.pool)) ND_FAIL(ND_EINVAL, "w2d: a pre-activation copy goes with whole, unpooled layers only");
     if (d.cout % 4) ND_FAIL(ND_EINVAL, "w2d: cout must be a multiple of 4");
     ND_TRY(nd_check_in_planes("w2d", d, KB, true, true));
-    const bool src2 = d.in2.base != nullptr, add = d.add.base != nullptr;
+    const bool src2 = d.in2.base != nullptr, add = d.add.base != nullptr, head = d.head_w != nullptr;
+    if (head && (d.pool || d.pre || src2 || add || !d.head_b || d.cout > kMTB * 32))
+        ND_FAIL(ND_EINVAL, "w2d: a layer with a fused 1x1 head is neither pooled nor keeps a pre-activation copy, has one input source, no addend "
+                           "and at most %d output channels", kMTB * 32);
     if (add && (d.pool || d.pre || src2))
         ND_FAIL(ND_EINVAL, "w2d: a layer with an addend source is neither pooled nor keeps a pre-activation copy nor has a second input source");
     if (add) ND_TRY(nd_check_add("w2d", d, (long)(d.roi_r0 + Hv - 1 + d.add.pad) * d.add.Wb + d.roi_c0 + Wpx - 1 + d.add.pad + 1));
@@ -563,10 +615,11 @@
 
     int dev = 0, ncus = 0;
     ND_TRY(nd_device(&dev, &ncus));
-    void (*fn)(ConvParams) = add ? conv_w2d<0, false, true> : src2 ? conv_w2d<0, true> : conv_w2d<0>;
+    void (*fn)(ConvParams) = head ? conv_w2d<0, false, false, true> : add ? conv_w2d<0, false, true> : src2 ? conv_w2d<0, true> : conv_w2d<0>;
+    const size_t lds = head ? kLds + kHeadLds : kLds;
 #ifdef ND_QP_STAMPS
     static const int dbg_all = getenv("ND_W2D_DBG") ? atoi(getenv("ND_W2D_DBG")) : 0;
-    const int dbg_env = src2 ? 0 : add ? (dbg_all == 128 ? 128 : 0) : dbg_all;
+    const int dbg_env = src2 || head ? 0 : add ? (dbg_all == 128 ? 128 : 0) : dbg_all;
     switch (dbg_env) {
         case 1: fn = conv_w2d<1>; break;
         case 2: fn = conv_w2d<2>; break;
@@ -583,7 +636,7 @@
         default: break;
     }
 #endif
-    ND_TRY(nd_raise_lds(dev, (const void *)fn, kLds));
+    ND_TRY(nd_raise_lds(dev, (const void *)fn, lds));
 
     ConvParams p = nd_conv_params(d, KB, d.cout);
     if (roi) {
@@ -601,6 +654,8 @@
         p.KBw = d.w_kb;
         p.wpk += (size_t)d.w_kb0 * kTaps * 256;
     }
+    p.head_w = d.head_w;
+    p.head_b = d.head_b;
     if (add) {
         p.add = (const f32x4 *)d.add.base + (long)d.add_plane0 * d.add.np() + (long)((roi ? d.roi_r0 : 0) + d.add.pad) * d.add.Wb +
                 (roi ? d.roi_c0 : 0) + d.add.pad;
@@ -619,7 +674,7 @@
     nd_conv_tiles(p, true, kS, kMTB * 32);
     nd_conv_fastdivs(p);
     const long ntiles = p.tiles_per_problem;
-    const long cap = d.part && !d.nosplit && !d.pool && !d.pre ? (long)(d.part_bytes / ((size_t)kMTB * 32 * kSlots * 4)) : 0;
+    const long cap = d.part && !d.nosplit && !d.pool && !d.pre && !head ? (long)(d.part_bytes / ((size_t)kMTB * 32 * kSlots * 4)) : 0;
     const long grid = nd_conv_schedule(p, ntiles, KB, ncus, cap);
     p.part = (f32x4 *)d.part;
 #ifdef ND_QP_STAMPS
@@ -635,7 +690,7 @@
         return nd_stamped_launch(fn, 512, kLds, p, ntiles, KB, ncus, stream, printed++ < 2, nullptr, "[w2d stamps] wave", kStampNames, 6, {0, 1, 4});
     }
 #endif
-    hipLaunchKernelGGL(fn, dim3((unsigned)grid), dim3(512), kLds, stream, p);
+    hipLaunchKernelGGL(fn, dim3((unsigned)grid), dim3(512), lds, stream, p);
     if (p.split_first < ntiles) hipLaunchKernelGGL(k_w2d_split_finish, dim3((unsigned)(ntiles - p.split_first), kMTB * 8), dim3(256), 0, stream, p);
     ND_HIP(hipGetLastError());
     return ND_OK;
diff --git a/nind_denoise_amd/csrc/nd_common.h b/nind_denoise_amd/csrc/nd_common.h
--- a/nind_denoise_amd/csrc/nd_common.h
+++ b/nind_denoise_amd/csrc/nd_common.h
@@ -119,6 +119,7 @@
     int add_plane0 = 0;
     const int *add_origin = nullptr;
     long add_origin_max = 0;
+    const float *head_w = nullptr, *head_b = nullptr;
 };
 int nd_check_in2(const char *who, const ConvDesc &d, int KB, long reach);
 int nd_check_add(const char *who, const ConvDesc &d, long reach);
@@ -153,7 +154,8 @@
 int nd_check_roi(const char *who, const ConvDesc &d, int Hv, int Wv, bool refused, const char *why);
 static inline int nd_check_flags(int flags, bool frame_loop = false, bool unet_frame = false) {
     const int known = ND_FLAG_NO_SPLITK | ND_FLAG_DIRECT_CONV | ND_FLAG_W1D_REGS | ND_FLAG_FULL_TILES | ND_FLAG_UNFUSED_POOL |
-                      ND_FLAG_TILE_ENCODER | ND_FLAG_TILE_WINO | (frame_loop ? ND_FLAG_TILE_LEVEL2 | ND_FLAG_TILE_SKIPS : 0) | (unet_frame ? ND_FLAG_FIND_NOISE : 0);
+                      ND_FLAG_TILE_ENCODER | ND_FLAG_TILE_WINO | (frame_loop ? ND_FLAG_TILE_LEVEL2 | ND_FLAG_TILE_SKIPS | ND_FLAG_TILE_HEAD : 0) |
+                      (unet_frame ? ND_FLAG_FIND_NOISE : 0);
     if (flags & ~known) ND_FAIL(ND_EINVAL, "unknown flag bits 0x%x", flags);
     return ND_OK;
 }
@@ -209,9 +211,11 @@
     ND_TRY(nd_launch_tile_verdict(src, cin, w, bias, 2, width, height, cs, ucs, ol, tile_begin, tile_count, tile_ok, s));
     return nd_launch_final1x1_stitch_ok(src, cin, w, bias, 2, canvas, width, height, cs, ucs, ol, tile_begin, tile_count, tile_ok, s);
 }
+int nd_launch_head_stitch(const QpBuf &src, int crop, float *canvas, int width, int height, int cs, int ucs, int ol, int tile_begin,
+                          int tile_count, unsigned char *tile_ok, hipStream_t s);
 int nd_utnet_denoise_tiles_ok(int funit, int act, int dtype, int flags, const void *packed, const float *img, float *canvas, int width,
                               int height, int cs, int ucs, int ol, int tile_begin, int tile_count, int batch, void *ws, size_t ws_bytes,
-                              void *stream, unsigned char *tile_ok);
+                              void *stream, unsigned char *tile_ok, bool head = true);
 int nd_launch_gather_pack(const float *img, int width, int height, int cs, int ucs, int ol, int tile_begin,
                           int tile_count, const QpBuf &dst, hipStream_t s, int border = 2, bool reflect = true);
 int nd_launch_gather_band(const float *img, int width, int height, int cs, int ucs, int ol, int band_row0, const QpBuf &dst,
diff --git a/nind_denoise_amd/csrc/pack.hip b/nind_denoise_amd/csrc/pack.hip
--- a/nind_denoise_amd/csrc/pack.hip
+++ b/nind_denoise_amd/csrc/pack.hip
@@ -12,7 +12,7 @@
 }
 
 extern "C" const char *nd_last_error(void) { return g_err; }
-extern "C" int nd_version(void) { return 119; }
+extern "C" int nd_version(void) { return 120; }
 
 static inline uint16_t f32_to_bf16_rne(float f) {
     uint32_t u;
diff --git a/nind_denoise_amd/csrc/utnet.hip b/nind_denoise_amd/csrc/utnet.hip
--- a/nind_denoise_amd/csrc/utnet.hip
+++ b/nind_denoise_amd/csrc/utnet.hip
@@ -96,6 +96,17 @@
     return make_plan(funit, h, w, batch, batch, nullptr, dtype).bytes;
 }
 
+extern "C" int nd_utnet_last_buffer(int funit, int cs, int batch, int dtype, size_t *offset, size_t *plane_bytes, int *planes, int *side) {
+    ND_TRY(check_net(funit, cs, cs, batch, dtype));
+    if (!offset || !plane_bytes || !planes || !side) ND_FAIL(ND_EINVAL, "nd_utnet_last_buffer: null output");
+    const QpBuf q = make_plan(funit, cs, cs, batch, batch, nullptr, dtype).buf[T4B];
+    *offset = (size_t)(uintptr_t)q.base;
+    *plane_bytes = (size_t)q.np() * 16;
+    *planes = q.planes;
+    *side = q.Hb;
+    return ND_OK;
+}
+
 extern "C" int nd_utnet_workspace_init_hw(void *ws, size_t ws_bytes, int funit, int h, int w, int batch, int dtype,
                                           void *stream) {
     ND_TRY(check_net(funit, h, w, batch, dtype));
@@ -127,12 +138,12 @@
                                       float *canvas, int width, int height, int cs, int ucs, int ol, int tile_begin,
                                       int tile_count, int batch, void *ws, size_t ws_bytes, void *stream) {
     return nd_utnet_denoise_tiles_ok(funit, act, dtype, flags, packed, img, canvas, width, height, cs, ucs, ol, tile_begin, tile_count, batch,
-                                     ws, ws_bytes, stream, nullptr);
+                                     ws, ws_bytes, stream, nullptr, true);
 }
 
 int nd_utnet_denoise_tiles_ok(int funit, int act, int dtype, int flags, const void *packed, const float *img, float *canvas, int width,
                               int height, int cs, int ucs, int ol, int tile_begin, int tile_count, int batch, void *ws, size_t ws_bytes,
-                              void *stream, unsigned char *tile_ok) {
+                              void *stream, unsigned char *tile_ok, bool head) {
     ND_TRY(nd_check_flags(flags));
     Plan pl;
     ND_TRY(forward_common(funit, act, dtype, packed, batch, tile_count, cs, cs, ws, ws_bytes, &pl));
@@ -146,8 +157,10 @@
     o.flags = flags;
     const int crop = (cs - ucs) / 2;
     if (!(flags & ND_FLAG_FULL_TILES) && plan_rois(pl, crop, crop, rois) && rois_supported(funit, dtype, flags, pl, bl, rois)) o.rois = rois;
+    const float *fw = blob + bl.off[kNumLayers - 1];
+    if (head && head_fused(funit, dtype, flags, pl, bl)) o.head = fw;
     ND_TRY(run_stack(funit, act, dtype, blob, pl, s, o));
-    const float *fw = blob + bl.off[kNumLayers - 1];
+    if (o.head) return nd_launch_head_stitch(pl.buf[T4B], 2, canvas, width, height, cs, ucs, ol, tile_begin, tile_count, tile_ok, s);
     return nd_launch_utnet_stitch(pl.buf[T4B], funit, fw, fw + 3 * funit, canvas, width, height, cs, ucs, ol, tile_begin, tile_count,
                                   tile_ok, s);
 }
@@ -457,6 +470,40 @@
                          (hipStream_t)stream);
 }
 
+extern "C" int nd_layer_head_forward(int fused, int act, float slope, const void *packed, const float *head, const float *x, int batch,
+                                     int cin, int h, int w, int cout, const int *roi, float *raw, float *y3, void *ws, size_t ws_bytes,
+                                     void *stream) {
+    const size_t need = nd_layer_workspace_bytes(ND_CONVT3, batch, cin, cout, h, w, ND_F32);
+    if (!need || cout % 4) ND_FAIL(ND_EINVAL, "nd_layer_head_forward: bad shape");
+    if (!packed || !head || !x || !raw) ND_FAIL(ND_EINVAL, "nd_layer_head_forward: null pointer");
+    if (!ws || ws_bytes < need) ND_FAIL(ND_ENOMEM, "nd_layer_head_forward: workspace %zu B given, %zu B needed", ws_bytes, need);
+    hipStream_t s = (hipStream_t)stream;
+    const LayerForm fm = wino_form(5);
+    const LayerPlan pl = layer_plan(ND_CONVT3, batch, cin, cout, h, w, (char *)ws, ND_F32);
+    const size_t out_bytes = (size_t)pl.out.planes * pl.out.pstride * 16;
+    ND_HIP(hipMemsetAsync(ws, 0, pl.bytes, s));
+    ND_HIP(hipMemsetAsync(pl.out.base, 0xff, out_bytes, s));
+    ND_TRY(nd_launch_nchw_to_qp(x, cin, pl.in, 0, s));
+    ConvDesc d = layer_desc(fm, ND_CONVT3, cin, cout, ND_F32, (const float *)packed, pl);
+    d.act = act;
+    d.slope = slope;
+    d.nosplit = true;
+    if (roi) {
+        d.roi_r0 = roi[0];
+        d.roi_c0 = roi[1];
+        d.roi_rows = roi[2];
+        d.roi_cols = roi[3];
+    }
+    if (fused) {
+        d.head_w = head;
+        d.head_b = head + 3 * cout;
+    }
+    ND_TRY(nd_launch_conv_w2d(d, s));
+    if (!fused && y3) ND_TRY(nd_launch_final1x1(pl.out, cout, head, head + 3 * cout, 0, y3, h + 2, w + 2, s));
+    ND_HIP(hipMemcpyAsync(raw, pl.out.base, out_bytes, hipMemcpyDeviceToDevice, s));
+    return ND_OK;
+}
+
 extern "C" int nd_maxpool2_forward(const float *x, int batch, int c, int h, int w, float *y, void *ws, size_t ws_bytes,
                                    void *stream) {
     if (batch <= 0 || c <= 0 || h < 2 || w < 2) ND_FAIL(ND_EINVAL, "nd_maxpool2_forward: bad shape");
diff --git a/nind_denoise_amd/csrc/utnet_frame.hip b/nind_denoise_amd/csrc/utnet_frame.hip
--- a/nind_denoise_amd/csrc/utnet_frame.hip
+++ b/nind_denoise_amd/csrc/utnet_frame.hip
@@ -498,6 +498,15 @@
     return ND_OK;
 }
 
+extern "C" int nd_utnet_frame_head(int funit, int dtype, int flags, int width, int height, int cs, int ucs, int ol, int *fused) {
+    ND_TRY(nd_check_flags(flags, true));
+    if (!fused) ND_FAIL(ND_EINVAL, "nd_utnet_frame_head: null output");
+    FramePlan fp;
+    ND_TRY(frame_plan(funit, dtype, flags, width, height, cs, ucs, ol, 1, &fp));
+    *fused = head_fused(funit, dtype, flags, make_plan(funit, cs, cs, 1, 1, nullptr, dtype), blob_layout(funit, dtype)) ? 1 : 0;
+    return ND_OK;
+}
+
 static int denoise_frame(int funit, int act, int dtype, int flags, const void *packed, const float *img, float *canvas, int width,
                          int height, int cs, int ucs, int ol, int tile_begin, int tile_count, int batch, void *ws, size_t ws_bytes, void *fws,
                          size_t fws_bytes, void *stream, nd_progress_fn progress, void *progress_ctx, unsigned char *tile_ok) {
@@ -517,8 +526,9 @@
         for (int t0 = tile_begin; t0 < end; t0 += batch, ++n) {
             const int cnt = end - t0 < batch ? end - t0 : batch;
             if (progress) progress(progress_ctx, n, t0, cnt);
-            ND_TRY(nd_utnet_denoise_tiles_ok(funit, act, dtype, flags & ~(ND_FLAG_TILE_LEVEL2 | ND_FLAG_TILE_SKIPS), packed, img, canvas, width, height, cs, ucs, ol, t0, cnt, batch, ws,
-                                             ws_bytes, stream, tile_ok));
+            ND_TRY(nd_utnet_denoise_tiles_ok(funit, act, dtype, flags & ~(ND_FLAG_TILE_LEVEL2 | ND_FLAG_TILE_SKIPS | ND_FLAG_TILE_HEAD), packed, img,
+                                             canvas, width, height, cs, ucs, ol, t0, cnt, batch, ws, ws_bytes, stream, tile_ok,
+                                             !(flags & ND_FLAG_TILE_HEAD)));
         }
         return ND_OK;
     }
@@ -544,6 +554,7 @@
     dec.step_begin = kLevels[c.nlev - 1].end;
     dec.rois = c.rois;
     dec.src2 = src2;
+    if (head_fused(funit, dtype, flags, c.pl, c.bl)) dec.head = fw;
     const int per_band = fp.R * fp.cols;
     int band_done = tile_begin / per_band - 1;
     for (int t0 = tile_begin, n = 0; t0 < end; ++n) {
@@ -562,7 +573,10 @@
             ND_TRY(assemble_output(c, l, tp, cp, t0, cnt));
         }
         ND_TRY(run_stack(funit, act, dtype, c.blob, tp, c.s, dec));
-        ND_TRY(nd_launch_utnet_stitch(tp.buf[T4B], funit, fw, fw + 3 * funit, canvas, width, height, cs, ucs, ol, t0, cnt, tile_ok, c.s));
+        if (dec.head)
+            ND_TRY(nd_launch_head_stitch(tp.buf[T4B], 2, canvas, width, height, cs, ucs, ol, t0, cnt, tile_ok, c.s));
+        else
+            ND_TRY(nd_launch_utnet_stitch(tp.buf[T4B], funit, fw, fw + 3 * funit, canvas, width, height, cs, ucs, ol, t0, cnt, tile_ok, c.s));
         t0 += cnt;
     }
     return ND_OK;
diff --git a/nind_denoise_amd/csrc/utnet_net.h b/nind_denoise_amd/csrc/utnet_net.h
--- a/nind_denoise_amd/csrc/utnet_net.h
+++ b/nind_denoise_amd/csrc/utnet_net.h
@@ -347,12 +347,20 @@
     return form == FORM_W1D4 && nd_f43_w2d(pl.buf[st.src], lcout(kLayers[st.layer], f), false, flags);
 }
 
+inline bool head_fused(int f, int dt, int flags, const Plan &pl, const BlobLayout &bl) {
+    const Step &st = kSteps[kNumSteps - 1];
+    const int cout = lcout(kLayers[st.layer], f);
+    return dt == ND_F32 && !(flags & ND_FLAG_TILE_HEAD) && cout <= 64 && step_form(st, f, dt, flags, pl, bl) == FORM_W1D4 &&
+           nd_f43_w2d(pl.buf[st.src], cout, false, flags);
+}
+
 struct StackOpts {
     int flags = 0;
     const Roi *rois = nullptr;
     int step_begin = 0, step_end = kNumSteps;
     const StepSrc2 *src2 = nullptr;
     int nsrc2 = 0;
+    const float *head = nullptr;
     hipEvent_t *ev = nullptr;
     hipEvent_t *ev_x = nullptr;
     long *wino_tiles = nullptr;
@@ -425,6 +433,11 @@
             }
         const bool next_is_pool = this_step + 1 < step_end && kSteps[this_step + 1].layer < 0;
         const bool w2d = form == FORM_W1D4 && nd_f43_w2d(d.in, d.cout, pre != nullptr, flags);
+        if (o.head && k == kNumSteps - 1) {
+            if (!w2d) ND_FAIL(ND_EINVAL, "UtNet: a fused head needs the last layer in conv_w2d");
+            d.head_w = o.head;
+            d.head_b = o.head + 3 * f;
+        }
         if (next_is_pool && !pre && !(flags & ND_FLAG_UNFUSED_POOL)) {
             pool_view = pl.buf[kSteps[this_step + 1].dst];
             d.pool = &pool_view;
diff --git a/nind_denoise_amd/networks/UtNet.py b/nind_denoise_amd/networks/UtNet.py
--- a/nind_denoise_amd/networks/UtNet.py
+++ b/nind_denoise_amd/networks/UtNet.py
@@ -53,6 +53,7 @@
     share_encoder = True
     share_level2 = True
     fold_skips = True
+    fuse_head = True
 
     def __init__(self, funit=64, activation='PReLU', compute_dtype='f32', fallback_dtype=None):
         super().__init__()
@@ -117,7 +118,8 @@
 
     @property
     def frame_flags(self):
-        return self.flags | (0 if self.share_level2 else _lib.FLAG_TILE_LEVEL2) | (0 if self.fold_skips else _lib.FLAG_TILE_SKIPS)
+        return (self.flags | (0 if self.share_level2 else _lib.FLAG_TILE_LEVEL2) | (0 if self.fold_skips else _lib.FLAG_TILE_SKIPS) |
+                (0 if self.fuse_head else _lib.FLAG_TILE_HEAD))
 
     def _weights_key(self, device):
         return (str(device), self.weights_generation) + tuple((p.data_ptr(), p._version) for p in self.parameters())
```

Measured after the change: 91.26 MP/s (median of 6 runs). Within noise of the previous version (+0.9%).
